# fx-erick/uncertainty-vit

Hardware: AMD Instinct MI355X
Metric: pretrain images/sec (ViT-B/16 224, bs=128/GPU) (higher is better)
Workload: dtype bf16

## Files before the change

### include/uvit.h

```cpp
#ifndef UVIT_H
#define UVIT_H
#include <stddef.h>
#include <stdint.h>

#ifdef __cplusplus
extern "C" {
#endif

#define UVIT_VERSION 100
#define UVIT_MAX_DEPTH 64

typedef struct uvit_engine uvit_engine;
typedef void* uvit_stream;

typedef struct uvit_config {
    int32_t img_size, patch_size, in_chans, embed_dim, depth, num_heads, mlp_hidden;
    int32_t use_shared_rel_pos_bias;
    int32_t use_abs_pos_emb;
    int32_t batch;
    float ln_eps;
    float attn_drop_rate;
    float drop_path_rate;
    int32_t bias_chunk;
    int32_t two_stream;
} uvit_config;

typedef struct uvit_layout_entry {
    char name[96];
    int64_t offset;
    int64_t numel;
    int32_t ndim;
    int32_t decay;
    int64_t shape[4];
} uvit_layout_entry;

typedef struct uvit_buffers {
    float* params;
    float* grads;
    float* adam_m;
    float* adam_v;
    float* ema;
    void* params_bf16;
    void* params_bf16_t;
    void* ema_bf16;
    const int32_t* rel_index;
    void* workspace;
    int64_t workspace_bytes;
} uvit_buffers;

typedef struct uvit_step_params {
    int32_t target_layers[UVIT_MAX_DEPTH];
    int32_t n_target_layers;
    int32_t target_layer_norm_last;
    int32_t post_target_layer_norm;
    int32_t l2_loss;
    float l1_beta;
    float loss_scale;
    float clip_grad;
    float lr, weight_decay, beta1, beta2, eps;
    int32_t opt_step;
    float ema_decay;
    int32_t do_ema;
    float grad_scale;
    uint32_t seed;
    uint32_t it;
    int32_t train_dropout;
    float lambda_pretraining;
    const float* sched_dev;
    int32_t sched_len, sched_index;
    int32_t layer_results_fc;
    float var_w0, var_margin0;
    int32_t target_batch_norm, target_instance_norm, post_target_instance_norm;
    int32_t n_rows_hint;
} uvit_step_params;

int uvit_version(void);
const char* uvit_source_hash(void);

int uvit_layout_count(const uvit_config* cfg);
int uvit_layout_get(const uvit_config* cfg, int index, uvit_layout_entry* out);
int64_t uvit_arena_numel(const uvit_config* cfg, int64_t* n_decay_out);
int64_t uvit_workspace_bytes(const uvit_config* cfg);

uvit_engine* uvit_engine_create(const uvit_config* cfg, const uvit_buffers* bufs, uvit_stream stream, int* err_out);
void uvit_engine_destroy(uvit_engine* e);

int uvit_engine_sync_shadows(uvit_engine* e, int which, uvit_stream stream);

int uvit_engine_forward_features(uvit_engine* e, int which, const float* images, const int64_t* mask, int batch,
                                 int train_dropout, uint32_t seed, uint32_t it, uvit_stream stream);
int uvit_engine_head(uvit_engine* e, int which, int all_tokens, float* out, int32_t* count_dev, uvit_stream stream);

void* uvit_engine_ws_ptr(uvit_engine* e, const char* name, int layer);
int uvit_engine_compact_rows(uvit_engine* e);

int uvit_step_begin(uvit_engine* e, const float* images, const int64_t* mask, const uvit_step_params* hp,
                    uvit_stream stream);
int uvit_step_backward_layer(uvit_engine* e, int layer, const uvit_step_params* hp, uvit_stream stream);
int uvit_step_wait_layer_grads(uvit_engine* e, int layer, uvit_stream stream);
int uvit_step_backward_embed(uvit_engine* e, uvit_stream stream);
int uvit_step_update(uvit_engine* e, const uvit_step_params* hp, uvit_stream stream);
int uvit_train_step(uvit_engine* e, const float* images, const int64_t* mask, const uvit_step_params* hp,
                    uvit_stream stream);
typedef struct uvit_tuning { int32_t nt_variant, tn_variant, tn_split_target, wgrad_group_chunks, nt_group, nt_persist; } uvit_tuning;
void uvit_tuning_default(uvit_tuning* out);
int uvit_engine_set_tuning(uvit_engine* e, const uvit_tuning* t);
int uvit_engine_set_streams(uvit_engine* e, int dual);
int uvit_engine_set_drop_path_rows(uvit_engine* e, int on);
int uvit_drop_path_kept_counts(int depth, float drop_path_rate, int draws_per_block, int batch, uint32_t seed, uint32_t it, int32_t* out);
int uvit_engine_profile(uvit_engine* e, int enable, int max_launches);
int uvit_engine_profile_read(uvit_engine* e, double* total_ms, int* launches, double* flops_per_launch);
int uvit_engine_profile_read_kind(uvit_engine* e, int kind, double* total_ms, int* launches, double* flops_per_launch,
                                  double* bytes_per_launch);
int uvit_engine_read_stats_async(uvit_engine* e, float* host_out2, uvit_stream stream);
int uvit_engine_read_stats(uvit_engine* e, float* host_out2, uvit_stream stream);

typedef struct uvit_gemm_epilogue {
    void* out; void* out2; const float* bias; const float* bias2; const float* gamma; const float* resid;
    const float* rowscale; const void* aux; const int64_t* mask; const float* mask_token;
    int32_t ldo, tokens, patches;
    int32_t row0;
} uvit_gemm_epilogue;
enum { UVIT_EPI_BF16 = 0, UVIT_EPI_QKV = 1, UVIT_EPI_GELU = 2, UVIT_EPI_RESID = 3, UVIT_EPI_F32 = 4,
       UVIT_EPI_PATCH = 5, UVIT_EPI_DGELU = 6, UVIT_EPI_QKV_ELU = 7,
       UVIT_EPI_GELU_DG = 8,
       UVIT_EPI_MULAUX = 9 };

int uvit_op_gemm_nt(int mode, const void* A_bf16, const void* W_bf16, int M, int N, int K, int lda, int ldw,
                    const uvit_gemm_epilogue* epi, uvit_stream stream);
int uvit_op_gemm_nt_tuned(int mode, const void* A_bf16, const void* W_bf16, int M, int N, int K, int lda, int ldw,
                          const uvit_gemm_epilogue* epi, const uvit_tuning* tune, int* tail_rows, uvit_stream stream);
int uvit_op_gemm_nt_sched(int mode, const void* A_bf16, const void* W_bf16, int M, int N, int K, int lda, int ldw,
                          const uvit_gemm_epilogue* epi, const uvit_tuning* tune, uint32_t* tile_counters, uvit_stream stream);
int uvit_op_gemm_tn(const void* Y_bf16, const void* X_bf16, int M, int N, int K, int ldy, int ldx, float* C, int ldc,
                    const uvit_tuning* tune, uvit_stream stream);
typedef struct uvit_wgrad_problem {
    const void* Y_bf16; const void* X_bf16; float* C; float* bias; float* bias2;
    int32_t bias_end, bias2_begin, M, N, K, ldy, ldx, ldc;
} uvit_wgrad_problem;
int uvit_op_wgrad_group(const uvit_wgrad_problem* problems, int count, const uvit_tuning* tune, uvit_stream stream);
int uvit_op_attn_fwd(const void* qkv, const float* biasP, void* out, float* lse, int B, int H, int N, int NP,
                     float scale, float p_drop, uint32_t seed, uint32_t layer, uvit_stream stream);
int64_t uvit_op_attn_bwd_ws_bytes(int B, int H, int N);
int uvit_op_attn_bwd(const void* qkv, const void* o_fwd, const void* d_o, const float* biasP, const float* lse,
                           float* delta, void* dqkv, float* dbias_slab, int accumulate_slab, void* ds_workspace, int B, int H,
                           int N, int NP, float scale, float p_drop, uint32_t seed, uint32_t layer, uvit_stream stream);
int uvit_op_attn_fwd_hd(const void* qkv, const float* biasP, void* out, float* lse, int B, int H, int N, int NP, int head_dim,
                        float scale, float p_drop, uint32_t seed, uint32_t layer, uvit_stream stream);
int uvit_op_attn_bwd_hd(const void* qkv, const void* o_fwd, const void* d_o, const float* biasP, const float* lse,
                        float* delta, void* dqkv, float* dbias_slab, int accumulate_slab, void* ds_workspace, int B, int H,
                        int N, int NP, int head_dim, float scale, float p_drop, uint32_t seed, uint32_t layer, uvit_stream stream);
int uvit_op_attn2_fwd(const void* qkv_m, const void* qkv_c, const float* biasP, void* out_m, void* out_c, float* lse, int B, int H,
                      int N, int NP, float scale, float p_drop, uint32_t seed, uint32_t layer, uvit_stream stream);
int64_t uvit_op_attn2_bwd_ws_bytes(int B, int H, int N);
int uvit_op_attn2_bwd(const void* qkv_m, const void* qkv_c, const void* o_m, const void* o_c, const void* d_m, const void* d_c,
                      const float* biasP, const float* lse, float* delta, void* dqkv_m, void* dqkv_c, float* dbias_slab,
                      int accumulate_slab, void* ds_workspace, int B, int H, int N, int NP, float scale, float p_drop, uint32_t seed,
                      uint32_t layer, uvit_stream stream);
int uvit_op_relpos_gather(const float* table, const int32_t* index, float* biasP, int H, int N, int NP, uvit_stream stream);
int uvit_op_relpos_scatter(const float* slab, int nslab, const int32_t* index, float* dtable, int H, int N, int NP,
                           uvit_stream stream);
int uvit_op_ln_fwd(const float* x, const float* w, const float* b, void* y_bf16, float* mean, float* rstd, int M, int C,
                   float eps, uvit_stream stream);
int uvit_op_ln_bwd(const void* dy_bf16, const float* x, const float* mean, const float* rstd, const float* w,
                   const float* dres, float* dx, float* dw, float* db, int M, int C, uvit_stream stream);
int uvit_op_ema(float* ema, const float* params, void* ema_bf16, int64_t n, float decay, uvit_stream stream);
int uvit_op_sumsq(const float* g, int64_t n, double* out, uvit_stream stream);
int uvit_op_adamw(float* p, const float* g, float* m, float* v, void* p_bf16, int64_t n, int64_t n_decay, float lr,
                  float wd, float b1, float b2, float eps, int step, const double* sumsq, float max_norm,
                  float grad_scale, float* gnorm_out, uvit_stream stream);
int uvit_op_smooth_l1(const float* out, const float* target, const int32_t* count_dev, float beta, int l2,
                      float loss_scale, float* loss, void* dout_bf16, int Mmax, int C, uvit_stream stream);
int uvit_op_wasserstein_loss(const float* out_m, const float* out_c, const float* tgt_m, const float* tgt_c,
                             const int32_t* count_dev, float lam, float loss_scale, float* scratch, float* loss,
                             void* dout_m_bf16, void* dout_c_bf16, int Mmax, int C, uvit_stream stream);
int uvit_op_target_accum(const float* x, const int32_t* rowidx, const int32_t* count, float* acc, int first, int Mmax,
                         int C, float eps, uvit_stream stream);
int uvit_op_variance_loss(const float* out, const int32_t* count_dev, float w, float margin, float loss_scale, float* scratch,
                          float* loss, float* std_loss0_out, void* dout_bf16, int Mmax, int C, uvit_stream stream);
int uvit_op_target_finalize(float* acc, const int32_t* count, int n_layers, int post_ln, int Mmax, int C, float eps,
                            uvit_stream stream);
int uvit_op_mask_compact(const int64_t* mask, int32_t* rowidx, int32_t* count, int B, int P, uvit_stream stream);
int uvit_op_synth_batch(float* images, int64_t* mask, int B, int chans, int img_size, int patches, int n_mask, uint32_t seed,
                        uint32_t it, uvit_stream stream);
int uvit_op_im2col(const float* img, void* cols_bf16, int B, int Cin, int img_size, int patch, uvit_stream stream);
int uvit_op_droppath(float* scales, const float* rates_dev, int depth, int B, uint32_t seed, uint32_t step,
                     uvit_stream stream);
int uvit_op_cast_bf16(const float* src, void* dst_bf16, int64_t n, uvit_stream stream);

#define UVIT_AUG_LANCZOS 1
#define UVIT_AUG_BILINEAR 2
#define UVIT_AUG_BICUBIC 3
#define UVIT_AUG_HAMMING 5
#define UVIT_AUG_BRIGHTNESS 0
#define UVIT_AUG_CONTRAST 1
#define UVIT_AUG_SATURATION 2
typedef struct uvit_augment_desc {
    int64_t offset;
    int32_t h, w;
    int32_t flip;
    int32_t crop_x, crop_y, crop_w, crop_h;
    int32_t resize_w, resize_h;
    int32_t win_x, win_y;
    int32_t filter;
    int32_t n_jitter;
    int32_t jitter_op[3];
    float jitter_factor[3];
    int32_t reserved;
} uvit_augment_desc;
int64_t uvit_op_augment_ws_bytes(const uvit_augment_desc* desc, int B, int S);
int uvit_op_augment_batch(const uint8_t* pixels, int64_t pixel_bytes, const uvit_augment_desc* desc, int B, int S, const float* mean,
                          const float* std, float* out, void* workspace, int64_t ws_bytes, uvit_stream stream);

#ifdef __cplusplus
}
#endif
#endif
```

### uncertainty-vit_amd/csrc/elementwise.hip

```cpp
#include "common.h"
#include "uvit_internal.h"
#include "rowwise.h"

__global__ void im2col_kernel(const float* __restrict__ img, bf16* __restrict__ cols, int B, int Cin, int S, int p) {
    const int g = S / p, P = g * g, K = Cin * p * p, kc_per_row = K / 8;
    const size_t total = (size_t)B * P * kc_per_row;
    for (size_t idx = blockIdx.x * (size_t)blockDim.x + threadIdx.x; idx < total; idx += (size_t)gridDim.x * blockDim.x) {
        const int kc = idx % kc_per_row;
        const size_t row = idx / kc_per_row;
        const int b = row / P, pp = row % P, py = pp / g, px = pp % g;
        const int k = kc * 8, c = k / (p * p), i = (k % (p * p)) / p, j = k % p;
        const float* src = img + (((size_t)b * Cin + c) * S + py * p + i) * S + px * p + j;
        const float4 a = *(const float4*)src, d = *(const float4*)(src + 4);
        bf16x8 o = {f2bf(a.x), f2bf(a.y), f2bf(a.z), f2bf(a.w), f2bf(d.x), f2bf(d.y), f2bf(d.z), f2bf(d.w)};
        *(bf16x8*)(cols + row * K + k) = o;
    }
}

__global__ __launch_bounds__(1024)
void mask_compact_kernel(const int64_t* __restrict__ mask, int* __restrict__ rowidx, int* __restrict__ count, int B, int P) {
    __shared__ int s_w[16];
    const int n = B * P, tid = threadIdx.x, lane = tid & 63, wave = tid >> 6;
    int base = 0;
    for (int sc = 0; sc < n; sc += 32 * 1024) {
        unsigned bits = 0;
#pragma unroll
        for (int k = 0; k < 32; ++k) {
            const int i = sc + k * 1024 + tid;
            if (i < n && mask[i] != 0) bits |= 1u << k;
        }
        for (int k = 0; k < 32 && sc + k * 1024 < n; ++k) {
            const bool keep = (bits >> k) & 1u;
            const unsigned long long bal = __ballot(keep);
            if (lane == 0) s_w[wave] = __popcll(bal);
            __syncthreads();
            int before = base, tot = 0;
#pragma unroll
            for (int q = 0; q < 16; ++q) { const int v = s_w[q]; tot += v; if (q < wave) before += v; }
            if (keep) {
                const int i = sc + k * 1024 + tid, b = i / P;
                rowidx[before + __popcll(bal & ((1ull << lane) - 1ull))] = b * (P + 1) + 1 + (i - b * P);
            }
            base += tot;
            __syncthreads();
        }
    }
    if (tid == 0) *count = base;
    for (int i = base + tid; i < n; i += 1024) rowidx[i] = 0;
}

__global__ void set_cls_kernel(float* __restrict__ x, const float* __restrict__ cls, int B, int N, int C) {
    const int i = blockIdx.x * blockDim.x + threadIdx.x;
    if (i < B * C) { const int b = i / C, c = i - b * C; x[(size_t)b * N * C + c] = cls[c]; }
}

__global__ void relpos_gather_kernel(const float* __restrict__ table, const int* __restrict__ index,
                                     float* __restrict__ biasP, int H, int N, int NP) {
    const size_t total = (size_t)H * NP * NP;
    for (size_t i = blockIdx.x * (size_t)blockDim.x + threadIdx.x; i < total; i += (size_t)gridDim.x * blockDim.x) {
        const int k = i % NP, q = (i / NP) % NP, h = i / ((size_t)NP * NP);
        float v = 0.f;
        if (k >= N) v = -1e30f;
        else if (q < N && table) v = table[(size_t)index[q * N + k] * H + h] * 1.4426950408889634f;
        biasP[i] = v;
    }
}

__global__ void relpos_scatter_kernel(const float* __restrict__ slab, int nslab, const int* __restrict__ index,
                                      float* __restrict__ dtable, int H, int N, int NP, int ntable) {
    extern __shared__ float tsum[];
    const int h = blockIdx.x;
    for (int i = threadIdx.x; i < ntable; i += blockDim.x) tsum[i] = 0.f;
    __syncthreads();
    const int total = N * N;
    for (int i = blockIdx.y * blockDim.x + threadIdx.x; i < total; i += gridDim.y * blockDim.x) {
        const int k = i / N, q = i - k * N;
        float s = 0.f;
        for (int sl = 0; sl < nslab; ++sl) s += slab[(((size_t)sl * H + h) * NP + k) * NP + q];
        atomicAdd(&tsum[index[q * N + k]], s);
    }
    __syncthreads();
    for (int i = threadIdx.x; i < ntable; i += blockDim.x)
        if (tsum[i] != 0.f) atomicAdd(dtable + (size_t)i * H + h, tsum[i]);
}

#define CP_ROWS 32

template <int NV, int WAVES = 4>
__device__ __forceinline__ void block_col_atomic(float4 (&acc)[NV], float* out, int nv, float (*red)[64 * 4]) {
    const int lane = threadIdx.x & 63, wave = threadIdx.x >> 6;
#pragma unroll
    for (int k = 0; k < NV; ++k) {
        if (64 * k < nv) {
            __syncthreads();
            ((float4*)red[wave])[lane] = acc[k];
            __syncthreads();
            if (wave == 0) {
                float4 s = ((float4*)red[0])[lane];
#pragma unroll
                for (int q = 1; q < WAVES; ++q) { const float4 a = ((float4*)red[q])[lane]; s.x += a.x; s.y += a.y; s.z += a.z; s.w += a.w; }
                const int i = lane + 64 * k;
                if (i < nv) { atomicAdd(out + 4 * i, s.x); atomicAdd(out + 4 * i + 1, s.y); atomicAdd(out + 4 * i + 2, s.z); atomicAdd(out + 4 * i + 3, s.w); }
            }
        }
    }
}

template <int NV>
__global__ __launch_bounds__(256)
void ls_bwd_kernel(const float* __restrict__ dx, const bf16* __restrict__ y, const float* __restrict__ gamma,
                   const float* __restrict__ rowscale, bf16* __restrict__ dy, float* __restrict__ dgamma,
                   float* __restrict__ dbias, int M, int C, int tokens, int nrep, size_t rep_stride,
                   const int* __restrict__ rowidx, const int* __restrict__ count) {
    __shared__ float red[4][64 * 4];
    dgamma += (size_t)(blockIdx.x % nrep) * rep_stride; dbias += (size_t)(blockIdx.x % nrep) * rep_stride;
    const int lane = threadIdx.x & 63, wave = threadIdx.x >> 6, nv = C >> 2;
    float4 ag[NV], ab[NV];
#pragma unroll
    for (int k = 0; k < NV; ++k) { ag[k] = make_float4(0.f, 0.f, 0.f, 0.f); ab[k] = ag[k]; }
    const int row_end = min((int)(blockIdx.x + 1) * CP_ROWS, M);
    const int n_valid = rowidx ? min(*count, M) : M;
    for (int row = blockIdx.x * CP_ROWS + wave; row < row_end; row += 4) {
        if (row >= n_valid) { store_zero_row<NV>(dy + (size_t)row * C, nv, lane); continue; }
        const int xr = rowidx ? rowidx[row] : row;
        const float dp = rowscale ? rowscale[xr / tokens] : 1.0f;
#pragma unroll
        for (int k = 0; k < NV; ++k) {
            const int i = lane + 64 * k;
            if (i < nv) {
                const float4 d = ((const float4*)(dx + (size_t)xr * C))[i];
                const float4 g = ((const float4*)gamma)[i];
                const bf16x4 yy = ((const bf16x4*)(y + (size_t)xr * C))[i];
                ls_apply(d, dp, yy, g, (bf16x4*)(dy + (size_t)row * C) + i, ag[k], ab[k]);
            }
        }
    }
    block_col_atomic(ag, dgamma, nv, red);
    block_col_atomic(ab, dbias, nv, red);
}

#define CS_ROWS 256
__global__ __launch_bounds__(256)
void colsum_kernel(const bf16* __restrict__ y, int ld, int col0, int ncols, int M, float* __restrict__ out, int nrep, size_t rep_stride) {
    __shared__ float red[4][64 * 8];
    out += (size_t)(blockIdx.y % nrep) * rep_stride;
    const int lane = threadIdx.x & 63, wave = threadIdx.x >> 6;
    const int c = blockIdx.x * 512 + lane * 8;
    float acc[8];
#pragma unroll
    for (int j = 0; j < 8; ++j) acc[j] = 0.f;
    const int row_end = min((int)(blockIdx.y + 1) * CS_ROWS, M);
    if (c < ncols) {
        const bf16* base = y + col0 + c;
        int row = blockIdx.y * CS_ROWS + wave;
        for (; row + 12 < row_end; row += 16) {
            const bf16x8 v0 = *(const bf16x8*)(base + (size_t)row * ld), v1 = *(const bf16x8*)(base + (size_t)(row + 4) * ld);
            const bf16x8 v2 = *(const bf16x8*)(base + (size_t)(row + 8) * ld), v3 = *(const bf16x8*)(base + (size_t)(row + 12) * ld);
#pragma unroll
            for (int j = 0; j < 8; ++j) acc[j] += (bf2f(v0[j]) + bf2f(v1[j])) + (bf2f(v2[j]) + bf2f(v3[j]));
        }
        for (; row < row_end; row += 4) {
            const bf16x8 v = *(const bf16x8*)(base + (size_t)row * ld);
#pragma unroll
            for (int j = 0; j < 8; ++j) acc[j] += bf2f(v[j]);
        }
    }
#pragma unroll
    for (int j = 0; j < 8; ++j) red[wave][lane * 8 + j] = acc[j];
    __syncthreads();
    for (int i = threadIdx.x; i < 512; i += 256) {
        const int cc = blockIdx.x * 512 + i;
        if (cc < ncols) atomicAdd(out + cc, red[0][i] + red[1][i] + red[2][i] + red[3][i]);
    }
}

__global__ __launch_bounds__(256)
void smooth_l1_kernel(const float* __restrict__ out, const float* __restrict__ target, const int* __restrict__ count,
                      float beta, int l2, float loss_scale, float* __restrict__ loss, bf16* __restrict__ dout,
                      int Mmax, int C) {
    __shared__ float red[4];
    const int n_valid = min(*count, Mmax);
    const size_t nv = (size_t)Mmax * C / 4, valid = (size_t)n_valid * C / 4;
    const float inv = loss_scale / ((float)n_valid * (float)C);
    float part = 0.f;
    for (size_t i = blockIdx.x * (size_t)blockDim.x + threadIdx.x; i < nv; i += (size_t)gridDim.x * blockDim.x) {
        bf16x4 g = bf16x4_zero();
        if (i < valid) {
            const float4 o = ((const float4*)out)[i], t = ((const float4*)target)[i];
            const float d[4] = {o.x - t.x, o.y - t.y, o.z - t.z, o.w - t.w};
#pragma unroll
            for (int j = 0; j < 4; ++j) {
                const float a = fabsf(d[j]);
                float l, gr;
                if (l2) { l = d[j] * d[j]; gr = 2.0f * d[j]; }
                else if (a < beta) { l = 0.5f * d[j] * d[j] / beta; gr = d[j] / beta; }
                else { l = a - 0.5f * beta; gr = d[j] > 0.f ? 1.0f : (d[j] < 0.f ? -1.0f : 0.f); }
                part += l;
                g[j] = f2bf(gr * inv);
            }
        }
        ((bf16x4*)dout)[i] = g;
    }
    part = wave_sum(part);
    if ((threadIdx.x & 63) == 0) red[threadIdx.x >> 6] = part;
    __syncthreads();
    if (threadIdx.x == 0) atomicAdd(loss, (red[0] + red[1] + red[2] + red[3]) * inv);
}

template <int NV, int TKB_WAVES>
__global__ __launch_bounds__(TKB_WAVES * 64)
void token_bwd_kernel(const float* __restrict__ dx, const int64_t* __restrict__ mask, bf16* __restrict__ dpatch,
                      float* __restrict__ dcls, float* __restrict__ dmask, int B, int P, int C, int rows_per_block) {
    __shared__ float red[TKB_WAVES][64 * 4];
    const int lane = threadIdx.x & 63, wave = threadIdx.x >> 6, nv = C >> 2, N = P + 1;
    float4 ac[NV], am[NV];
#pragma unroll
    for (int k = 0; k < NV; ++k) { ac[k] = make_float4(0.f, 0.f, 0.f, 0.f); am[k] = ac[k]; }
    const int M = B * N;
    const int row_end = min((int)(blockIdx.x + 1) * rows_per_block, M);
    for (int row = blockIdx.x * rows_per_block + wave; row < row_end; row += TKB_WAVES) {
        const int b = row / N, t = row - b * N;
        const bool is_cls = t == 0;
        const bool masked = !is_cls && mask[b * P + t - 1] != 0;
#pragma unroll
        for (int k = 0; k < NV; ++k) {
            const int i = lane + 64 * k;
            if (i < nv) {
                const float4 d = ((const float4*)(dx + (size_t)row * C))[i];
                if (is_cls) { ac[k].x += d.x; ac[k].y += d.y; ac[k].z += d.z; ac[k].w += d.w; }
                else {
                    if (masked) { am[k].x += d.x; am[k].y += d.y; am[k].z += d.z; am[k].w += d.w; }
                    const float m = masked ? 0.f : 1.f;
                    bf16x4 o = {f2bf(d.x * m), f2bf(d.y * m), f2bf(d.z * m), f2bf(d.w * m)};
                    ((bf16x4*)(dpatch + ((size_t)b * P + t - 1) * C))[i] = o;
                }
            }
        }
    }
    const int row0 = blockIdx.x * rows_per_block;
    if ((row0 + N - 1) / N * N < row_end) block_col_atomic<NV, TKB_WAVES>(ac, dcls, nv, red);
    block_col_atomic<NV, TKB_WAVES>(am, dmask, nv, red);
}

__global__ __launch_bounds__(256)
void transpose_batch_kernel(const TransposeDesc* __restrict__ descs, int ndesc) {
    __shared__ bf16 tile[64][66];
    int lo = 0, hi = ndesc - 1;
    const int t = blockIdx.x;
    while (lo < hi) { const int mid = (lo + hi + 1) >> 1; if (descs[mid].tile0 <= t) lo = mid; else hi = mid - 1; }
    const TransposeDesc d = descs[lo];
    const int local = t - d.tile0, tc = (d.cols + 63) / 64;
    const int tr0 = (local / tc) * 64, tc0 = (local % tc) * 64;
    if (tr0 >= d.rows) return;
    const bf16* src = (const bf16*)d.src; bf16* dst = (bf16*)d.dst;
    if (tr0 + 64 <= d.rows && tc0 + 64 <= d.cols && !(d.rows & 7) && !(d.cols & 7)) {
#pragma unroll
        for (int k = 0; k < 2; ++k) {
            const int idx = threadIdx.x + 256 * k, r = idx >> 3, c8 = (idx & 7) * 8;
            const bf16x8 v = *(const bf16x8*)(src + (size_t)(tr0 + r) * d.cols + tc0 + c8);
#pragma unroll
            for (int j = 0; j < 8; ++j) tile[r][c8 + j] = v[j];
        }
        __syncthreads();
#pragma unroll
        for (int k = 0; k < 2; ++k) {
            const int idx = threadIdx.x + 256 * k, oc = idx >> 3, r8 = (idx & 7) * 8;
            bf16x8 o;
#pragma unroll
            for (int j = 0; j < 8; ++j) o[j] = tile[r8 + j][oc];
            *(bf16x8*)(dst + (size_t)(tc0 + oc) * d.rows + tr0 + r8) = o;
        }
        return;
    }
    for (int i = threadIdx.x; i < 64 * 64; i += 256) {
        const int r = i >> 6, c = i & 63;
        tile[r][c] = (tr0 + r < d.rows && tc0 + c < d.cols) ? src[(size_t)(tr0 + r) * d.cols + tc0 + c] : f2bf(0.f);
    }
    __syncthreads();
    for (int i = threadIdx.x; i < 64 * 64; i += 256) {
        const int c = i >> 6, r = i & 63;
        if (tr0 + r < d.rows && tc0 + c < d.cols) dst[(size_t)(tc0 + c) * d.rows + tr0 + r] = tile[r][c];
    }
}

__global__ void droppath_kernel(float* __restrict__ scales, const float* __restrict__ rates, int depth, int nbr, int B,
                                uint32_t seed, uint32_t step) {
    const int i = blockIdx.x * blockDim.x + threadIdx.x;
    if (i >= depth * nbr * B) return;
    const int b = i % B, lb = i / B, layer = lb / nbr, br = lb - layer * nbr;
    const float r = rates[layer];
    float v = 1.0f;
    if (r > 0.f) {
        const uint32_t key = uvit_hash32(seed ^ ((step * (uint32_t)nbr * depth + (uint32_t)nbr * layer + br + 1u) * 0x9E3779B9u));
        v = uvit_hash32((uint32_t)b ^ key) >= uvit_drop_threshold(r) ? 1.0f / (1.0f - r) : 0.f;
    }
    scales[i] = v;
}

#define DP_MAX_LISTS 128
struct DpHostCounts { int k[DP_MAX_LISTS]; };
#define DPL_CHUNKS 8
__global__ __launch_bounds__(256)
void droppath_lists_kernel(const float* __restrict__ scales, int* __restrict__ pos, int* __restrict__ bmap, int* __restrict__ rows,
                           int* __restrict__ cnt, int B, int tokens, int rows_stride, DpHostCounts host) {
    extern __shared__ int s_m[];
    const int lb = blockIdx.x;
    const float* sc = scales + (size_t)lb * B;
    int* p = pos + (size_t)lb * B; int* m = bmap + (size_t)lb * B; int* r = rows + (size_t)lb * rows_stride;
    const bool pub = blockIdx.y == 0;
    __shared__ int s_w[4];
    const int lane = threadIdx.x & 63, wave = threadIdx.x >> 6;
    int base = 0;
    for (int b0 = 0; b0 < B; b0 += 256) {
        const int b = b0 + threadIdx.x;
        const bool keep = b < B && sc[b] != 0.f;
        const unsigned long long bal = __ballot(keep);
        if (lane == 0) s_w[wave] = __popcll(bal);
        __syncthreads();
        int before = base;
        for (int q = 0; q < wave; ++q) before += s_w[q];
        const int slot = before + __popcll(bal & ((1ull << lane) - 1ull));
        if (pub && b < B) p[b] = keep ? slot : -1;
        if (keep) { s_m[slot] = b; if (pub) m[slot] = b; }
        base += s_w[0] + s_w[1] + s_w[2] + s_w[3];
        __syncthreads();
    }
    if (pub) {
        for (int b = base + threadIdx.x; b < B; b += 256) m[b] = 0;
        if (threadIdx.x == 0) {
            cnt[lb] = base * tokens;
            cnt[gridDim.x + lb] = base != host.k[lb];
        }
    }
    const int n = base * tokens, npad = (n + 63) & ~63;
    const int per = (npad + DPL_CHUNKS - 1) / DPL_CHUNKS, lo = blockIdx.y * per, hi = min(lo + per, npad);
    for (int i = lo + threadIdx.x; i < hi; i += blockDim.x) {
        const int slot = i / tokens;
        r[i] = i < n ? s_m[slot] * tokens + (i - slot * tokens) : -1;
    }
}

static inline int grid_for(size_t n, int block, int cap = 256 * 8) {
    size_t g = (n + block - 1) / block;
    return (int)(g < 1 ? 1 : (g > (size_t)cap ? cap : g));
}

int uvit_im2col_launch(const float* img, void* cols, int B, int Cin, int S, int p, hipStream_t s) {
    if (B <= 0 || p % 8 || S % p || S % 4) return UVIT_ERR_SHAPE;
    const size_t total = (size_t)B * (S / p) * (S / p) * (Cin * p * p / 8);
    hipLaunchKernelGGL(im2col_kernel, dim3(grid_for(total, 256, 256 * 16)), dim3(256), 0, s, img, (bf16*)cols, B, Cin, S, p);
    return uvit_check_launch();
}
int uvit_mask_compact_launch(const int64_t* mask, int* rowidx, int* count, int B, int P, hipStream_t s) {
    hipLaunchKernelGGL(mask_compact_kernel, dim3(1), dim3(1024), 0, s, mask, rowidx, count, B, P);
    return uvit_check_launch();
}
int uvit_set_cls_launch(float* x, const float* cls, const float* pos, int B, int N, int C, hipStream_t s) {
    if (pos) return UVIT_ERR_ARG;
    hipLaunchKernelGGL(set_cls_kernel, dim3((B * C + 255) / 256), dim3(256), 0, s, x, cls, B, N, C);
    return uvit_check_launch();
}
int uvit_relpos_gather_launch(const float* table, const int* index, float* biasP, int H, int N, int NP, hipStream_t s) {
    hipLaunchKernelGGL(relpos_gather_kernel, dim3(grid_for((size_t)H * NP * NP, 256)), dim3(256), 0, s, table, index, biasP, H, N, NP);
    return uvit_check_launch();
}
int uvit_relpos_scatter_launch(const float* slab, int nslab, const int* index, float* dtable, int H, int N, int NP,
                               hipStream_t s) {
    const int g = (int)(sqrtf((float)(N - 1)) + 0.5f);
    const int ntable = (2 * g - 1) * (2 * g - 1) + 3;
    hipLaunchKernelGGL(relpos_scatter_kernel, dim3(H, 24), dim3(256), ntable * sizeof(float), s, slab, nslab, index, dtable, H, N, NP, ntable);
    return uvit_check_launch();
}
int uvit_ls_bwd_launch(const float* dx, const LsNext& ls, int M, int C, int nrep, size_t rep_stride, hipStream_t s,
                       const int* rowidx, const int* count) {
    if (C % 4 || C > ROW_MAXV * 256 || (rowidx && !count)) return UVIT_ERR_SHAPE;
    dispatch_nv(C, [&](auto nv) {
        hipLaunchKernelGGL(ls_bwd_kernel<decltype(nv)::value>, dim3((M + CP_ROWS - 1) / CP_ROWS), dim3(256), 0, s, dx, ls.y, ls.gamma, ls.rowscale,
                           ls.dy, ls.dgamma, ls.dbias, M, C, ls.tokens, nrep > 0 ? nrep : 1, rep_stride, rowidx, count);
    });
    return uvit_check_launch();
}
__global__ void rows_guard_kernel(const int* __restrict__ count, int limit, float* __restrict__ loss) {
    if (*count > limit) loss[0] = __builtin_nanf("");
}
int uvit_rows_guard_launch(const int* count, int limit, float* loss, hipStream_t s) {
    hipLaunchKernelGGL(rows_guard_kernel, dim3(1), dim3(1), 0, s, count, limit, loss);
    return uvit_check_launch();
}
int uvit_colsum_launch(const void* y, int ld, int col0, int ncols, int M, float* out, int nrep, size_t rep_stride, hipStream_t s) {
    if (ncols % 8 || col0 % 8 || ld % 8) return UVIT_ERR_SHAPE;
    hipLaunchKernelGGL(colsum_kernel, dim3((ncols + 511) / 512, (M + CS_ROWS - 1) / CS_ROWS), dim3(256), 0, s, (const bf16*)y, ld, col0, ncols, M, out, nrep > 0 ? nrep : 1, rep_stride);
    return uvit_check_launch();
}
int uvit_smooth_l1_launch(const float* out, const float* target, const int* count, float beta, int l2, float loss_scale,
                          float* loss, void* dout, int Mmax, int C, hipStream_t s) {
    if (C % 4) return UVIT_ERR_SHAPE;
    hipLaunchKernelGGL(smooth_l1_kernel, dim3(grid_for((size_t)Mmax * C / 4, 256, 512)), dim3(256), 0, s, out, target, count, beta, l2,
                       loss_scale, loss, (bf16*)dout, Mmax, C);
    return uvit_check_launch();
}
int uvit_token_bwd_launch(const float* dx, const int64_t* mask, void* dpatch, float* dcls, float* dmask_token, int B,
                          int P, int C, hipStream_t s) {
    if (C % 4 || C > ROW_MAXV * 256) return UVIT_ERR_SHAPE;
    const int M = B * (P + 1);
    int rpb = (M + 127) / 128;
    rpb = ((rpb + 15) / 16) * 16;
    if (rpb < 32) rpb = 32;
    dispatch_nv(C, [&](auto nv) {
        hipLaunchKernelGGL((token_bwd_kernel<decltype(nv)::value, 16>), dim3((M + rpb - 1) / rpb), dim3(16 * 64), 0, s, dx, mask, (bf16*)dpatch,
                           dcls, dmask_token, B, P, C, rpb);
    });
    return uvit_check_launch();
}
int uvit_transpose_batch_launch(const void* descs_dev, int ndesc, int total_tiles, hipStream_t s) {
    if (ndesc <= 0 || total_tiles <= 0) return UVIT_OK;
    hipLaunchKernelGGL(transpose_batch_kernel, dim3(total_tiles), dim3(256), 0, s, (const TransposeDesc*)descs_dev, ndesc);
    return uvit_check_launch();
}
int uvit_droppath_launch(float* scales, const float* rates_dev, int depth, int nbr, int B, uint32_t seed, uint32_t step, hipStream_t s) {
    hipLaunchKernelGGL(droppath_kernel, dim3((depth * nbr * B + 255) / 256), dim3(256), 0, s, scales, rates_dev, depth, nbr, B, seed, step);
    return uvit_check_launch();
}

__global__ void droppath_lists_guard_kernel(const int* __restrict__ flags, int n, float* __restrict__ loss) {
    int bad = 0;
    for (int i = 0; i < n; ++i) bad |= flags[i];
    if (bad) loss[0] = __builtin_nanf("");
}
int uvit_droppath_lists_guard_launch(const int* cnt, int nlists, float* loss, hipStream_t s) {
    hipLaunchKernelGGL(droppath_lists_guard_kernel, dim3(1), dim3(1), 0, s, cnt + nlists, nlists, loss);
    return uvit_check_launch();
}
int uvit_droppath_lists_launch(const float* scales, int* pos, int* bmap, int* rows, int* cnt, int nlists, int B, int tokens,
                               int rows_stride, const int* host_counts, hipStream_t s) {
    if (nlists < 1 || nlists > DP_MAX_LISTS || rows_stride < ((B * tokens + 63) & ~63)) return UVIT_ERR_ARG;
    DpHostCounts h;
    for (int i = 0; i < DP_MAX_LISTS; ++i) h.k[i] = i < nlists ? host_counts[i] : 0;
    hipLaunchKernelGGL(droppath_lists_kernel, dim3(nlists, DPL_CHUNKS), dim3(256), (size_t)B * sizeof(int), s, scales, pos, bmap, rows, cnt, B, tokens, rows_stride, h);
    return uvit_check_launch();
}

__global__ void poison_kernel(const float* __restrict__ loss, float* __restrict__ dst, int* __restrict__ sticky) {
    if ((__float_as_uint(*loss) & 0x7F800000u) == 0x7F800000u) { *dst = __int_as_float(0x7FC00000); if (sticky) *sticky = 1; }
}
int uvit_poison_if_nonfinite_launch(const float* loss, float* dst, int* sticky, hipStream_t s) {
    hipLaunchKernelGGL(poison_kernel, dim3(1), dim3(1), 0, s, loss, dst, sticky);
    return uvit_check_launch();
}

__device__ __forceinline__ float sig_(float x) { return 1.0f / (1.0f + __expf(-x)); }

__global__ __launch_bounds__(256)
void wl_pos_kernel(const float* __restrict__ om, const float* __restrict__ oc, const float* __restrict__ tm,
                   const float* __restrict__ tc, const int* __restrict__ count, float* __restrict__ scratch, int Mmax, int C) {
    const int lane = threadIdx.x & 63, row = blockIdx.x * 4 + (threadIdx.x >> 6);
    if (row >= min(*count, Mmax)) return;
    float acc = 0.f;
    for (int i = lane; i < C; i += 64) {
        const size_t o = (size_t)row * C + i;
        const float d = sig_(om[o]) - sig_(tm[o]);
        const float e = sqrtf(fmaxf(sig_(oc[o]), 1e-24f)) - sqrtf(fmaxf(sig_(tc[o]), 1e-24f));
        acc += d * d + e * e;
    }
    acc = wave_sum(acc);
    if (lane == 0) { scratch[16 + row] = acc; atomicMax((int*)scratch, __float_as_int(acc)); }
}

__global__ __launch_bounds__(256)
void wl_sum_kernel(const int* __restrict__ count, float* __restrict__ scratch, int Mmax) {
    const int n = min(*count, Mmax);
    const float m = scratch[0];
    float s1 = 0.f, s2 = 0.f;
    for (int r = blockIdx.x * blockDim.x + threadIdx.x; r < n; r += gridDim.x * blockDim.x) {
        const float pos = scratch[16 + r], u = pos / m;
        s1 += log1pf(__expf(u));
        s2 += sig_(u) * u;
        if (pos == m) atomicMin((int*)scratch + 3, r);
    }
    s1 = wave_sum(s1); s2 = wave_sum(s2);
    if ((threadIdx.x & 63) == 0) { atomicAdd(scratch + 1, s1); atomicAdd(scratch + 2, s2); }
}

__global__ __launch_bounds__(256)
void wl_grad_kernel(const float* __restrict__ om, const float* __restrict__ oc, const float* __restrict__ tm,
                    const float* __restrict__ tc, const int* __restrict__ count, const float* __restrict__ scratch,
                    float lam, float* __restrict__ loss, bf16* __restrict__ dout_m, bf16* __restrict__ dout_c, int Mmax, int C) {
    const int lane = threadIdx.x & 63, row = blockIdx.x * 4 + (threadIdx.x >> 6);
    const int n = min(*count, Mmax);
    const float F = 1.3132616875182228f;
    if (blockIdx.x == 0 && threadIdx.x == 0) atomicAdd(loss, lam * scratch[1] / F);
    if (row >= Mmax) return;
    if (row >= n) {
        for (int i = lane; i < C; i += 64) dout_c[(size_t)row * C + i] = f2bf(0.f);
        return;
    }
    const float m = scratch[0], u = scratch[16 + row] / m;
    float coef = sig_(u);
    if (row == ((const int*)scratch)[3]) coef -= scratch[2];
    coef *= lam / (F * m);
    for (int i = lane; i < C; i += 64) {
        const size_t o = (size_t)row * C + i;
        const float a = sig_(om[o]), c1 = sig_(oc[o]), c2 = sig_(tc[o]);
        const float gm = coef * 2.0f * (a - sig_(tm[o])) * a * (1.0f - a);
        const float s1 = sqrtf(fmaxf(c1, 1e-24f)), s2 = sqrtf(fmaxf(c2, 1e-24f));
        const float gc = coef * (s1 - s2) / s1 * c1 * (1.0f - c1);
        dout_m[o] = f2bf(bf2f(dout_m[o]) + gm);
        dout_c[o] = f2bf(gc);
    }
}

int uvit_wasserstein_loss_launch(const float* out_m, const float* out_c, const float* tgt_m, const float* tgt_c, const int* count,
                                 float lam, float loss_scale, float* scratch, float* loss, void* dout_m, void* dout_c,
                                 int Mmax, int C, hipStream_t s) {
    if (hipMemsetAsync(scratch, 0, 16 * sizeof(float), s) != hipSuccess) return UVIT_ERR_LAUNCH;
    const int big = 0x7FFFFFFF;
    (void)big;
    hipLaunchKernelGGL(wl_pos_kernel, dim3((Mmax + 3) / 4), dim3(256), 0, s, out_m, out_c, tgt_m, tgt_c, count, scratch, Mmax, C);
    if (hipMemsetD32Async((hipDeviceptr_t)((int*)scratch + 3), 0x7FFFFFFF, 1, s) != hipSuccess) return UVIT_ERR_LAUNCH;
    hipLaunchKernelGGL(wl_sum_kernel, dim3(64), dim3(256), 0, s, count, scratch, Mmax);
    hipLaunchKernelGGL(wl_grad_kernel, dim3((Mmax + 3) / 4), dim3(256), 0, s, out_m, out_c, tgt_m, tgt_c, count, scratch,
                       lam * loss_scale, loss, (bf16*)dout_m, (bf16*)dout_c, Mmax, C);
    return uvit_check_launch();
}

__global__ __launch_bounds__(256)
void synth_images_kernel(float* __restrict__ img, size_t n2, uint32_t key) {
    for (size_t i = blockIdx.x * (size_t)blockDim.x + threadIdx.x; i < n2; i += (size_t)gridDim.x * blockDim.x) {
        const uint32_t a = uvit_hash32((uint32_t)(2 * i) ^ key), b = uvit_hash32((uint32_t)(2 * i + 1) ^ key ^ (uint32_t)(i >> 31));
        const float u1 = ((float)(a >> 8) + 0.5f) * (1.0f / 16777216.0f);
        const float u2 = ((float)(b >> 8) + 0.5f) * (1.0f / 16777216.0f);
        const float r = sqrtf(-2.0f * __logf(u1));
        float sn, cs;
        __sincosf(6.283185307179586f * u2, &sn, &cs);
        ((float2*)img)[i] = make_float2(r * cs, r * sn);
    }
}

__global__ __launch_bounds__(256)
void synth_mask_kernel(int64_t* __restrict__ mask, int P, int n_mask, uint32_t key) {
    extern __shared__ uint32_t keys[];
    const int b = blockIdx.x;
    for (int i = threadIdx.x; i < P; i += blockDim.x) keys[i] = uvit_hash32((uint32_t)(b * P + i) ^ key);
    __syncthreads();
    for (int i = threadIdx.x; i < P; i += blockDim.x) {
        const uint32_t k = keys[i];
        int rank = 0;
        for (int j = 0; j < P; ++j) rank += (keys[j] < k) || (keys[j] == k && j < i);
        mask[(size_t)b * P + i] = rank < n_mask ? 1 : 0;
    }
}

int uvit_synth_batch_launch(float* images, int64_t* mask, int B, int chans, int img_size, int patches, int n_mask, uint32_t seed,
                            uint32_t it, hipStream_t s) {
    if (B < 1 || chans < 1 || img_size < 1 || patches < 1 || n_mask < 0 || n_mask > patches) return UVIT_ERR_SHAPE;
    const size_t n = (size_t)B * chans * img_size * img_size;
    if (n % 2) return UVIT_ERR_SHAPE;
    const uint32_t key = uvit_hash32(seed ^ (it * 0x9E3779B9u + 0x51ED270Bu));
    if (images) {
        size_t g = (n / 2 + 255) / 256;
        hipLaunchKernelGGL(synth_images_kernel, dim3((unsigned)(g > 4096 ? 4096 : g)), dim3(256), 0, s, images, n / 2, key);
    }
    if (mask) hipLaunchKernelGGL(synth_mask_kernel, dim3(B), dim3(256), patches * sizeof(uint32_t), s, mask, patches, n_mask, key ^ 0xA5A5A5A5u);
    return uvit_check_launch();
}

#define VL_ROWS 64
template <int PASS>
__global__ __launch_bounds__(256)
void varloss_colstat_kernel(const float* __restrict__ out, const int* __restrict__ count, float* __restrict__ scratch, int Mmax, int C) {
    const int n = min(*count, Mmax);
    const int c = blockIdx.x * 256 + threadIdx.x;
    if (c >= C) return;
    const int r0 = blockIdx.y * VL_ROWS, r1 = min(r0 + VL_ROWS, n);
    const float mean = PASS == 1 ? scratch[c] / (float)max(n, 1) : 0.f;
    float acc = 0.f;
    for (int r = r0; r < r1; ++r) {
        const float v = out[(size_t)r * C + c];
        acc += PASS == 0 ? v : (v - mean) * (v - mean);
    }
    if (r0 < r1) atomicAdd(scratch + PASS * C + c, acc);
}

__global__ __launch_bounds__(256)
void varloss_sum_kernel(const int* __restrict__ count, float* __restrict__ scratch, float w, float margin, float* __restrict__ loss,
                        float* __restrict__ std_out, int Mmax, int C) {
    __shared__ float red[4];
    const int n = min(*count, Mmax);
    float acc = 0.f;
    for (int c = threadIdx.x; c < C; c += 256) {
        const float z0 = sqrtf(scratch[C + c] / (float)max(n - 1, 1) + 1e-6f);
        acc += fmaxf(margin - z0, 0.f);
    }
    acc = wave_sum(acc);
    if ((threadIdx.x & 63) == 0) red[threadIdx.x >> 6] = acc;
    __syncthreads();
    if (threadIdx.x == 0) {
        const float s = (red[0] + red[1] + red[2] + red[3]) / (float)C;
        scratch[2 * C] = s;
        if (std_out) *std_out = s;
        atomicAdd(loss, w * s);
    }
}

__global__ __launch_bounds__(256)
void varloss_grad_kernel(const float* __restrict__ out, const int* __restrict__ count, const float* __restrict__ scratch, float w,
                         float margin, bf16* __restrict__ dout, int Mmax, int C) {
    const int n = min(*count, Mmax);
    const int c = blockIdx.x * 256 + threadIdx.x;
    if (c >= C || n < 2) return;
    const float mean = scratch[c] / (float)n;
    const float z0 = sqrtf(scratch[C + c] / (float)(n - 1) + 1e-6f);
    if (!(z0 < margin)) return;
    const float k = -w / ((float)C * (float)(n - 1) * z0);
    const int r0 = blockIdx.y * VL_ROWS, r1 = min(r0 + VL_ROWS, n);
    for (int r = r0; r < r1; ++r) {
        const size_t o = (size_t)r * C + c;
        dout[o] = f2bf(bf2f(dout[o]) + k * (out[o] - mean));
    }
}

int uvit_variance_loss_launch(const float* out, const int* count, float w, float margin, float loss_scale, float* scratch, float* loss,
                              float* std_loss0_out, void* dout, int Mmax, int C, hipStream_t s) {
    if (Mmax < 1 || C < 1) return UVIT_ERR_SHAPE;
    if (hipMemsetAsync(scratch, 0, (2 * (size_t)C + 16) * sizeof(float), s) != hipSuccess) return UVIT_ERR_LAUNCH;
    const dim3 grid((C + 255) / 256, (Mmax + VL_ROWS - 1) / VL_ROWS);
    hipLaunchKernelGGL(varloss_colstat_kernel<0>, grid, dim3(256), 0, s, out, count, scratch, Mmax, C);
    hipLaunchKernelGGL(varloss_colstat_kernel<1>, grid, dim3(256), 0, s, out, count, scratch, Mmax, C);
    hipLaunchKernelGGL(varloss_sum_kernel, dim3(1), dim3(256), 0, s, count, scratch, w * loss_scale, margin, loss, std_loss0_out, Mmax, C);
    hipLaunchKernelGGL(varloss_grad_kernel, grid, dim3(256), 0, s, out, count, scratch, w * loss_scale, margin, (bf16*)dout, Mmax, C);
    return uvit_check_launch();
}

__global__ __launch_bounds__(256)
void add_pos_kernel(float* __restrict__ x, const float* __restrict__ pos, size_t n4, size_t per_sample4) {
    for (size_t i = blockIdx.x * (size_t)blockDim.x + threadIdx.x; i < n4; i += (size_t)gridDim.x * blockDim.x) {
        float4 a = ((float4*)x)[i];
        const float4 p = ((const float4*)pos)[i % per_sample4];
        a.x += p.x; a.y += p.y; a.z += p.z; a.w += p.w;
        ((float4*)x)[i] = a;
    }
}
__global__ __launch_bounds__(256)
void pos_bwd_kernel(const float* __restrict__ dx, float* __restrict__ dpos, int B, size_t per_sample4) {
    const size_t i = blockIdx.x * (size_t)blockDim.x + threadIdx.x;
    if (i >= per_sample4) return;
    float4 acc = make_float4(0.f, 0.f, 0.f, 0.f);
    for (int b = 0; b < B; ++b) {
        const float4 d = ((const float4*)dx)[(size_t)b * per_sample4 + i];
        acc.x += d.x; acc.y += d.y; acc.z += d.z; acc.w += d.w;
    }
    ((float4*)dpos)[i] = acc;
}
int uvit_add_pos_launch(float* x, const float* pos, int B, int N, int C, hipStream_t s) {
    if (C % 4) return UVIT_ERR_SHAPE;
    const size_t per = (size_t)N * C / 4, n4 = per * B;
    hipLaunchKernelGGL(add_pos_kernel, dim3(grid_for(n4, 256)), dim3(256), 0, s, x, pos, n4, per);
    return uvit_check_launch();
}
int uvit_pos_bwd_launch(const float* dx, float* dpos, int B, int N, int C, hipStream_t s) {
    if (C % 4) return UVIT_ERR_SHAPE;
    const size_t per = (size_t)N * C / 4;
    hipLaunchKernelGGL(pos_bwd_kernel, dim3((unsigned)((per + 255) / 256)), dim3(256), 0, s, dx, dpos, B, per);
    return uvit_check_launch();
}
```

### uncertainty-vit_amd/csrc/engine.hip

```cpp
#include <hip/hip_runtime.h>
#include <math.h>
#include <stdio.h>
#include <stdlib.h>
#include <string.h>

#include <string>
#include <vector>

#include "../../include/uvit.h"
#include "common.h"
#include "uvit_internal.h"

#define CHECK(x) do { int _rc = (x); if (_rc) return _rc; } while (0)
#define NREP 32
#define RP(off) (e->grep + ((off) - e->lo.n_decay))
#define HIPCHECK(x) do { if ((x) != hipSuccess) return UVIT_ERR_LAUNCH; } while (0)
#define GEMM_NT(...) uvit_gemm_nt_launch(__VA_ARGS__, &e->tune)
#define GEMM_TN(...) uvit_gemm_tn_launch(__VA_ARGS__, &e->tune)
#define GEMM_TN_GROUP(...) uvit_gemm_tn_group_launch(__VA_ARGS__, &e->tune)

struct LayerOff { size_t n1w, n1b, qkvw, qb, vb, projw, projb, g1, n2w, n2b, fc1w, fc1b, fc2w, fc2b, g2;
                  size_t cqkvw, cqb, cvb, cprojw, cprojb; };
struct Layout {
    size_t cls, mask_tok, pew, peb, relt, normw, normb, lmw, lmb, pos;
    size_t ccls, cmask_tok, cpew, cpeb, clmw, clmb;
    LayerOff L[UVIT_MAX_DEPTH];
    size_t n_total, n_decay, n_live;
    std::vector<uvit_layout_entry> entries;
};

static size_t align64(size_t x) { return (x + 63) & ~(size_t)63; }

static int cfg_ok(const uvit_config* c) {
    if (!c) return UVIT_ERR_ARG;
    if (c->depth < 1 || c->depth > UVIT_MAX_DEPTH || c->num_heads < 1) return UVIT_ERR_SHAPE;
    if (c->embed_dim != c->num_heads * 64 && (c->two_stream || c->embed_dim != c->num_heads * 80)) return UVIT_ERR_SHAPE;
    if (c->embed_dim % 64 || c->mlp_hidden % 64 || c->patch_size % 8 || c->img_size % c->patch_size) return UVIT_ERR_SHAPE;
    if ((c->in_chans * c->patch_size * c->patch_size) % 64) return UVIT_ERR_SHAPE;
    const int g = c->img_size / c->patch_size;
    if (g * g + 1 > 208 || c->batch < 1) return UVIT_ERR_SHAPE;
    if (c->use_abs_pos_emb && c->two_stream) return UVIT_ERR_SHAPE;
    return UVIT_OK;
}

static void build_layout(const uvit_config* c, Layout& lo) {
    const int64_t C = c->embed_dim, Hd = c->mlp_hidden, g = c->img_size / c->patch_size;
    const int64_t Kpe = (int64_t)c->in_chans * c->patch_size * c->patch_size;
    size_t off = 0;
    auto add = [&](const std::string& name, std::vector<int64_t> shape, int decay) -> size_t {
        uvit_layout_entry e;
        memset(&e, 0, sizeof(e));
        snprintf(e.name, sizeof(e.name), "%s", name.c_str());
        e.offset = (int64_t)off; e.ndim = (int)shape.size(); e.decay = decay; e.numel = 1;
        for (size_t i = 0; i < shape.size(); ++i) { e.shape[i] = shape[i]; e.numel *= shape[i]; }
        lo.entries.push_back(e);
        const size_t at = off;
        off = align64(off + (size_t)e.numel);
        return at;
    };
    auto blk = [](int i, const char* s) { return "blocks." + std::to_string(i) + "." + s; };
    const bool two = c->two_stream != 0;
    lo.mask_tok = add("mask_token", {1, 1, C}, 1);
    if (two) lo.cmask_tok = add("cov_mask_token", {1, 1, C}, 1);
    if (two) lo.ccls = add("cov_cls_token", {1, 1, C}, 1);
    if (c->use_shared_rel_pos_bias) lo.relt = add("rel_pos_bias.relative_position_bias_table", {(2 * g - 1) * (2 * g - 1) + 3, c->num_heads}, 1);
    else lo.relt = (size_t)-1;
    lo.pew = add("patch_embed.proj.weight", {C, c->in_chans, c->patch_size, c->patch_size}, 1);
    if (two) lo.cpew = add("cov_patch_embed.proj.weight", {C, c->in_chans, c->patch_size, c->patch_size}, 1);
    (void)Kpe;
    for (int i = 0; i < c->depth; ++i) {
        lo.L[i].qkvw = add(blk(i, "attn.qkv.weight"), {3 * C, C}, 1);
        lo.L[i].projw = add(blk(i, "attn.proj.weight"), {C, C}, 1);
        if (two) lo.L[i].cprojw = add(blk(i, "attn.cov_proj.weight"), {C, C}, 1);
        lo.L[i].fc1w = add(blk(i, "mlp.fc1.weight"), {Hd, C}, 1);
        lo.L[i].fc2w = add(blk(i, "mlp.fc2.weight"), {C, Hd}, 1);
    }
    lo.lmw = add("lm_head.weight", {C, C}, 1);
    if (two) lo.clmw = add("cov_lm_head.weight", {C, C}, 1);
    lo.n_decay = off;
    lo.cls = add("cls_token", {1, 1, C}, 0);
    lo.pos = c->use_abs_pos_emb ? add("pos_embed", {1, g * g + 1, C}, 0) : (size_t)-1;
    lo.peb = add("patch_embed.proj.bias", {C}, 0);
    if (two) lo.cpeb = add("cov_patch_embed.proj.bias", {C}, 0);
    for (int i = 0; i < c->depth; ++i) {
        lo.L[i].g1 = add(blk(i, "gamma_1"), {C}, 0);
        lo.L[i].g2 = add(blk(i, "gamma_2"), {C}, 0);
        lo.L[i].n1w = add(blk(i, "norm1.weight"), {C}, 0);
        lo.L[i].n1b = add(blk(i, "norm1.bias"), {C}, 0);
        lo.L[i].qb = add(blk(i, "attn.q_bias"), {C}, 0);
        lo.L[i].vb = add(blk(i, "attn.v_bias"), {C}, 0);
        if (two) { lo.L[i].cqb = add(blk(i, "attn.cov_q_bias"), {C}, 0); lo.L[i].cvb = add(blk(i, "attn.cov_v_bias"), {C}, 0); }
        lo.L[i].projb = add(blk(i, "attn.proj.bias"), {C}, 0);
        if (two) lo.L[i].cprojb = add(blk(i, "attn.cov_proj.bias"), {C}, 0);
        lo.L[i].n2w = add(blk(i, "norm2.weight"), {C}, 0);
        lo.L[i].n2b = add(blk(i, "norm2.bias"), {C}, 0);
        lo.L[i].fc1b = add(blk(i, "mlp.fc1.bias"), {Hd}, 0);
        lo.L[i].fc2b = add(blk(i, "mlp.fc2.bias"), {C}, 0);
    }
    lo.normw = add("norm.weight", {C}, 0);
    lo.normb = add("norm.bias", {C}, 0);
    lo.lmb = add("lm_head.bias", {C}, 0);
    if (two) lo.clmb = add("cov_lm_head.bias", {C}, 0);
    lo.n_live = off;
    if (two)
        for (int i = 0; i < c->depth; ++i) lo.L[i].cqkvw = add(blk(i, "attn.cov_qkv.weight"), {3 * C, C}, 2);
    lo.n_total = off;
}

struct LayerActs {
    bf16 *ln1, *qkv, *attn, *projout, *ln2, *h, *a, *mlpout;
    float *mean1, *rstd1, *mean2, *rstd2, *lse;
};

struct uvit_engine {
    uvit_config cfg;
    uvit_buffers buf;
    Layout lo;
    int B, P, N, NP, C, Hd, H, Kpe, M, Mpad, BP, BPpad, chunk, nchunk;
    int head_dim;
    float attn_scale;
    int S;
    GemmTune tune;
    int cur_B;
    bf16* cols;
    float* X[UVIT_MAX_DEPTH + 1];
    float* XM[UVIT_MAX_DEPTH];
    LayerActs acts[UVIT_MAX_DEPTH];
    LayerActs tacts;
    float *tX[2], *tXM;
    int *rowidx, *count;
    bf16 *normed[2], *dout[2], *dnormed[2], *dpatch[2];
    float *meanF[2], *rstdF[2], *outputs[2], *targets[2];
    float *biasP_s, *biasP_t, *slabs, *delta;
    void* ds_ws[2] = {nullptr, nullptr};
    float *dXa, *dXb;
    bf16 *dY1[2], *dY2[2], *dH[2], *dLN, *dAttn, *dqkv[2];
    float *dp_scales, *dp_rates;
    int *dpl_pos = nullptr, *dpl_bmap = nullptr, *dpl_rows = nullptr, *dpl_cnt = nullptr;
    size_t dpl_stride = 0;
    int dpl_K[128] = {};
    bool dpl_enable = true;
    bool dpl_on = false;
    std::vector<float> dp_rates_host;
    float *loss, *gnorm; double* sumsq;
    float* wl_scratch;
    float *dense_v, *dense_acc; int *idrows, *idcount;
    float* var_scratch;
    int* poisoned;
    TransposeDesc* tdesc; int n_tdesc, n_ttiles;
    int64_t* mask_copy;
    unsigned* tile_cnt = nullptr;
    float* grep;
    size_t n_nd;
    bool slab_started;
    bool last_dropout; uint32_t last_seed, last_it;
    int bwd_next = -1;
    int compact_R = 0;
    bool dual = true;
    hipStream_t aux = nullptr, aux_eq = nullptr, aux_lo = nullptr;
    hipEvent_t ev_fork = nullptr, ev_teacher = nullptr, ev_x = nullptr;
    hipEvent_t ev_wdone[UVIT_MAX_DEPTH] = {};
    hipEvent_t ev_ds = nullptr;
    bool prof_on = false;
    std::vector<hipEvent_t> prof_ev;
    std::vector<int> prof_kind;
    std::vector<int> prof_rows;
    size_t prof_used = 0;
    size_t rows_all() const { return (size_t)(S - 1) * Mpad + M; }
    size_t rows_alloc() const { return (size_t)S * Mpad; }
};

struct Bump {
    char* base; size_t off, cap;
    template <typename T> T* take(size_t n) {
        off = (off + 255) & ~(size_t)255;
        T* p = base ? (T*)(base + off) : nullptr;
        off += n * sizeof(T);
        return p;
    }
};

static size_t roundup(size_t x, size_t m) { return (x + m - 1) / m * m; }
static std::vector<float> dp_rates_linspace(int depth, float rate);

static void plan_workspace(uvit_engine* e, Bump& b) {
    const uvit_config& c = e->cfg;
    const size_t Mp = e->rows_alloc(), C = e->C, Hd = e->Hd, BPp = e->BPpad;
    auto acts = [&](LayerActs& a) {
        a.ln1 = b.take<bf16>(Mp * C); a.qkv = b.take<bf16>(Mp * 3 * C); a.attn = b.take<bf16>(Mp * C);
        a.projout = b.take<bf16>(Mp * C); a.ln2 = b.take<bf16>(Mp * C); a.h = b.take<bf16>(Mp * Hd);
        a.a = b.take<bf16>(Mp * Hd); a.mlpout = b.take<bf16>(Mp * C);
        a.mean1 = b.take<float>(Mp); a.rstd1 = b.take<float>(Mp); a.mean2 = b.take<float>(Mp); a.rstd2 = b.take<float>(Mp);
        a.lse = b.take<float>((size_t)e->B * e->H * e->N);
    };
    e->cols = b.take<bf16>(BPp * e->Kpe);
    for (int i = 0; i <= c.depth; ++i) e->X[i] = b.take<float>(Mp * C);
    for (int i = 0; i < c.depth; ++i) { e->XM[i] = b.take<float>(Mp * C); acts(e->acts[i]); }
    acts(e->tacts);
    e->tX[0] = b.take<float>(Mp * C); e->tX[1] = b.take<float>(Mp * C); e->tXM = b.take<float>(Mp * C);
    e->rowidx = b.take<int>(e->BP + 64); e->count = b.take<int>(64);
    for (int st = 0; st < e->S; ++st) {
        e->normed[st] = b.take<bf16>(BPp * C); e->dout[st] = b.take<bf16>(BPp * C); e->dnormed[st] = b.take<bf16>(BPp * C);
        e->dpatch[st] = b.take<bf16>(BPp * C);
        e->meanF[st] = b.take<float>(BPp); e->rstdF[st] = b.take<float>(BPp);
        e->outputs[st] = b.take<float>(BPp * C); e->targets[st] = b.take<float>(BPp * C);
    }
    const size_t bias_n = (size_t)e->H * e->NP * e->NP;
    e->biasP_s = b.take<float>(bias_n); e->biasP_t = b.take<float>(bias_n);
    e->slabs = b.take<float>(bias_n);
    e->delta = b.take<float>((size_t)e->B * e->H * e->N);
    if (e->cfg.use_shared_rel_pos_bias)
        for (int k = 0; k < 2; ++k)
            e->ds_ws[k] = b.take<char>(e->S == 1 ? uvit_attn_bwd_fused_ws_bytes(e->B, e->H, e->N) : uvit_attn2_bwd_ws_bytes(e->B, e->H, e->N));
    e->dXa = b.take<float>(Mp * C); e->dXb = b.take<float>(Mp * C);
    for (int k = 0; k < 2; ++k) {
        e->dY1[k] = b.take<bf16>(Mp * C); e->dY2[k] = b.take<bf16>(Mp * C); e->dH[k] = b.take<bf16>(Mp * Hd);
        e->dqkv[k] = b.take<bf16>(Mp * 3 * C);
    }
    e->dLN = b.take<bf16>(Mp * C); e->dAttn = b.take<bf16>(Mp * C);
    e->dp_scales = b.take<float>((size_t)c.depth * 2 * e->S * e->B); e->dp_rates = b.take<float>(c.depth);
    if ((size_t)c.depth * 2 * e->S <= 128) {
        const size_t nl = (size_t)c.depth * 2 * e->S;
        e->dpl_stride = roundup((size_t)e->B * e->N, 64);
        e->dpl_pos = b.take<int>(nl * e->B); e->dpl_bmap = b.take<int>(nl * e->B);
        e->dpl_rows = b.take<int>(nl * e->dpl_stride); e->dpl_cnt = b.take<int>(2 * nl + 64);
    }
    e->loss = b.take<float>(64); e->gnorm = e->loss + 1; e->sumsq = (double*)(e->loss + 2);
    e->wl_scratch = b.take<float>(16 + BPp);
    e->poisoned = b.take<int>(64);
    e->var_scratch = b.take<float>(2 * C + 16);
    e->dense_v = b.take<float>(BPp * C); e->dense_acc = b.take<float>(BPp * C);
    e->idrows = b.take<int>(e->BP + 64); e->idcount = b.take<int>(64);
    e->tdesc = b.take<TransposeDesc>(7 * c.depth + 4);
    e->mask_copy = b.take<int64_t>(e->BP + 64);
    e->grep = b.take<float>((size_t)NREP * e->n_nd);
    e->tile_cnt = b.take<unsigned>(64);
}

static void fill_dims(uvit_engine* e) {
    const uvit_config& c = e->cfg;
    const int g = c.img_size / c.patch_size;
    e->B = c.batch; e->P = g * g; e->N = e->P + 1; e->NP = 208; e->C = c.embed_dim; e->Hd = c.mlp_hidden;
    e->H = c.num_heads; e->Kpe = c.in_chans * c.patch_size * c.patch_size;
    e->head_dim = c.embed_dim / c.num_heads;
    e->attn_scale = e->head_dim == 64 ? 0.125f : (float)(1.0 / std::sqrt((double)e->head_dim));
    e->S = c.two_stream ? 2 : 1;
    e->M = e->B * e->N; e->Mpad = (int)roundup(e->M, 128); e->BP = e->B * e->P; e->BPpad = (int)roundup(e->BP, 128);
    if (c.bias_chunk > 0) {
        e->chunk = c.bias_chunk;
    } else {
        int ncu = 256, dev = 0; hipDeviceProp_t prop;
        if (hipGetDevice(&dev) == hipSuccess && hipGetDeviceProperties(&prop, dev) == hipSuccess && prop.multiProcessorCount > 0)
            ncu = prop.multiProcessorCount;
        const int nhalf = (e->N + 15) / 16 > 7 ? 2 : 1;
        const int resident = 1;
        int max_chunks = (resident * ncu) / (e->H * nhalf);
        if (max_chunks < 1) max_chunks = 1;
        e->chunk = (e->B + max_chunks - 1) / max_chunks;
        if (e->chunk < 1) e->chunk = 1;
    }
    e->nchunk = (e->B + e->chunk - 1) / e->chunk;
    e->cur_B = e->B;
    Layout tmp_lo; build_layout(&e->cfg, tmp_lo);
    e->n_nd = tmp_lo.n_live - tmp_lo.n_decay;
}


extern "C" void uvit_engine_destroy(uvit_engine* e);
extern "C" int uvit_version(void) { return UVIT_VERSION; }
#ifndef UVIT_SRC_HASH
#define UVIT_SRC_HASH "unknown"
#endif
extern "C" const char* uvit_source_hash(void) { return UVIT_SRC_HASH; }

extern "C" int uvit_layout_count(const uvit_config* cfg) {
    if (cfg_ok(cfg)) return UVIT_ERR_SHAPE;
    Layout lo; build_layout(cfg, lo);
    return (int)lo.entries.size();
}
extern "C" int uvit_layout_get(const uvit_config* cfg, int index, uvit_layout_entry* out) {
    if (cfg_ok(cfg) || !out) return UVIT_ERR_SHAPE;
    Layout lo; build_layout(cfg, lo);
    if (index < 0 || index >= (int)lo.entries.size()) return UVIT_ERR_ARG;
    *out = lo.entries[index];
    return UVIT_OK;
}
extern "C" int64_t uvit_arena_numel(const uvit_config* cfg, int64_t* n_decay_out) {
    if (cfg_ok(cfg)) return UVIT_ERR_SHAPE;
    Layout lo; build_layout(cfg, lo);
    if (n_decay_out) *n_decay_out = (int64_t)lo.n_decay;
    return (int64_t)lo.n_total;
}
extern "C" int64_t uvit_workspace_bytes(const uvit_config* cfg) {
    if (cfg_ok(cfg)) return UVIT_ERR_SHAPE;
    uvit_engine tmp;
    tmp.cfg = *cfg;
    fill_dims(&tmp);
    Bump b{nullptr, 0, 0};
    plan_workspace(&tmp, b);
    return (int64_t)roundup(b.off, 4096) + 4096;
}

extern "C" uvit_engine* uvit_engine_create(const uvit_config* cfg, const uvit_buffers* bufs, uvit_stream stream, int* err_out) {
    auto fail = [&](int rc) -> uvit_engine* { if (err_out) *err_out = rc; return nullptr; };
    if (cfg_ok(cfg) || !bufs) return fail(UVIT_ERR_SHAPE);
    if (!bufs->params || !bufs->grads || !bufs->adam_m || !bufs->adam_v || !bufs->ema || !bufs->params_bf16 ||
        !bufs->params_bf16_t || !bufs->ema_bf16 || !bufs->workspace) return fail(UVIT_ERR_ARG);
    if (cfg->use_shared_rel_pos_bias && !bufs->rel_index) return fail(UVIT_ERR_ARG);
    if (bufs->workspace_bytes < uvit_workspace_bytes(cfg)) return fail(UVIT_ERR_WORKSPACE);
    uvit_engine* e = new uvit_engine();
    e->cfg = *cfg; e->buf = *bufs;
    fill_dims(e);
    build_layout(cfg, e->lo);
    Bump b{(char*)bufs->workspace, 0, (size_t)bufs->workspace_bytes};
    plan_workspace(e, b);
    hipStream_t s = (hipStream_t)stream;
    if (hipMemsetAsync(bufs->workspace, 0, b.off, s) != hipSuccess) { delete e; return fail(UVIT_ERR_LAUNCH); }
    std::vector<float> rates = dp_rates_linspace(cfg->depth, cfg->drop_path_rate);
    e->dp_rates_host = rates;
    if (const char* v = getenv("UVIT_DP_ROWS")) e->dpl_enable = v[0] != '0';
    std::vector<TransposeDesc> td;
    int tiles = 0;
    const char* src = (const char*)bufs->params_bf16; char* dst = (char*)bufs->params_bf16_t;
    auto addT = [&](size_t off, int rows, int cols) {
        TransposeDesc d; d.src = src + off * 2; d.dst = dst + off * 2; d.rows = rows; d.cols = cols; d.tile0 = tiles; d.pad = 0;
        tiles += ((rows + 63) / 64) * ((cols + 63) / 64);
        td.push_back(d);
    };
    for (int i = 0; i < cfg->depth; ++i) {
        addT(e->lo.L[i].qkvw, 3 * e->C, e->C); addT(e->lo.L[i].projw, e->C, e->C);
        addT(e->lo.L[i].fc1w, e->Hd, e->C); addT(e->lo.L[i].fc2w, e->C, e->Hd);
        if (e->S == 2) addT(e->lo.L[i].cprojw, e->C, e->C);
    }
    addT(e->lo.lmw, e->C, e->C);
    if (e->S == 2) addT(e->lo.clmw, e->C, e->C);
    e->n_tdesc = (int)td.size(); e->n_ttiles = tiles;
    {
        std::vector<int> idr(e->BP);
        for (int i = 0; i < e->BP; ++i) idr[i] = i;
        const int cnt = e->BP;
        if (hipMemcpyAsync(e->idrows, idr.data(), idr.size() * sizeof(int), hipMemcpyHostToDevice, s) != hipSuccess ||
            hipMemcpyAsync(e->idcount, &cnt, sizeof(int), hipMemcpyHostToDevice, s) != hipSuccess ||
            hipStreamSynchronize(s) != hipSuccess) { delete e; return fail(UVIT_ERR_LAUNCH); }
    }
    if (hipMemcpyAsync(e->dp_rates, rates.data(), rates.size() * sizeof(float), hipMemcpyHostToDevice, s) != hipSuccess ||
        hipMemcpyAsync(e->tdesc, td.data(), td.size() * sizeof(TransposeDesc), hipMemcpyHostToDevice, s) != hipSuccess ||
        hipStreamSynchronize(s) != hipSuccess) { delete e; return fail(UVIT_ERR_LAUNCH); }
    e->slab_started = false; e->last_dropout = false; e->last_seed = 0; e->last_it = 0;
    {
        const char* env = getenv("UVIT_SINGLE_STREAM");
        e->dual = !(env && env[0] == '1');
        int lo = 0, hi = 0; (void)hipDeviceGetStreamPriorityRange(&lo, &hi);
        bool ok = hipStreamCreateWithFlags(&e->aux_eq, hipStreamNonBlocking) == hipSuccess &&
                  hipStreamCreateWithPriority(&e->aux_lo, hipStreamNonBlocking, lo) == hipSuccess;
        e->aux = e->aux_eq;
        auto mk = [&](hipEvent_t* ev) { ok = ok && hipEventCreateWithFlags(ev, hipEventDisableTiming) == hipSuccess; };
        mk(&e->ev_fork); mk(&e->ev_teacher); mk(&e->ev_ds); mk(&e->ev_x);
        for (int i = 0; i < cfg->depth; ++i) mk(&e->ev_wdone[i]);
        if (!ok) { uvit_engine_destroy(e); return fail(UVIT_ERR_LAUNCH); }
    }
    if (err_out) *err_out = UVIT_OK;
    return e;
}

extern "C" void uvit_engine_destroy(uvit_engine* e) {
    if (!e) return;
    for (hipEvent_t ev : e->prof_ev) (void)hipEventDestroy(ev);
    if (e->aux_eq) { (void)hipStreamSynchronize(e->aux_eq); (void)hipStreamDestroy(e->aux_eq); }
    if (e->aux_lo) { (void)hipStreamSynchronize(e->aux_lo); (void)hipStreamDestroy(e->aux_lo); }
    if (e->ev_fork) (void)hipEventDestroy(e->ev_fork);
    if (e->ev_teacher) (void)hipEventDestroy(e->ev_teacher);
    if (e->ev_ds) (void)hipEventDestroy(e->ev_ds);
    if (e->ev_x) (void)hipEventDestroy(e->ev_x);
    for (int i = 0; i < UVIT_MAX_DEPTH; ++i) if (e->ev_wdone[i]) (void)hipEventDestroy(e->ev_wdone[i]);
    delete e;
}

static int tune_from_abi(const uvit_tuning* t, GemmTune& g) {
    if (!t) { g = GemmTune(); return UVIT_OK; }
    if ((t->nt_variant != 0 && t->nt_variant != 1 && t->nt_variant != 3 && t->nt_variant != 5 && t->nt_variant != 6 && t->nt_variant != 7) ||
        (t->tn_variant != 0 && t->tn_variant != 1 && t->tn_variant != 3) || t->tn_split_target < 0 || t->wgrad_group_chunks < 0 || t->nt_group < 0 || t->nt_group > 64 || (t->nt_persist != 0 && t->nt_persist != 1))
        return UVIT_ERR_ARG;
    g.nt_variant = t->nt_variant; g.tn_variant = t->tn_variant;
    g.tn_target = t->tn_split_target > 0 ? t->tn_split_target : 512; g.group_chunks = t->wgrad_group_chunks; g.nt_group = t->nt_group; g.nt_persist = t->nt_persist;
    return UVIT_OK;
}

extern "C" void uvit_tuning_default(uvit_tuning* out) {
    if (!out) return;
    const GemmTune d;
    out->nt_variant = d.nt_variant; out->tn_variant = d.tn_variant; out->tn_split_target = d.tn_target; out->wgrad_group_chunks = d.group_chunks; out->nt_group = d.nt_group; out->nt_persist = d.nt_persist;
}

extern "C" int uvit_engine_set_tuning(uvit_engine* e, const uvit_tuning* t) {
    if (!e) return UVIT_ERR_ARG;
    return tune_from_abi(t, e->tune);
}

extern "C" int uvit_engine_set_streams(uvit_engine* e, int dual) {
    if (!e || dual < 0 || dual > 2) return UVIT_ERR_ARG;
    hipStream_t next = dual == 2 ? e->aux_lo : e->aux_eq;
    if (next != e->aux && e->aux) HIPCHECK(hipStreamSynchronize(e->aux));
    e->aux = next;
    e->dual = dual != 0;
    return UVIT_OK;
}

extern "C" int uvit_engine_set_drop_path_rows(uvit_engine* e, int on) {
    if (!e) return UVIT_ERR_ARG;
    e->dpl_enable = on != 0;
    return UVIT_OK;
}

extern "C" int uvit_engine_profile(uvit_engine* e, int enable, int max_launches) {
    if (!e) return UVIT_ERR_ARG;
    if (enable && e->prof_ev.empty()) {
        e->prof_ev.resize((size_t)(max_launches > 0 ? max_launches : 4096) * 2);
        e->prof_kind.assign(e->prof_ev.size() / 2, -1);
        e->prof_rows.assign(e->prof_ev.size() / 2, 0);
        for (auto& ev : e->prof_ev) if (hipEventCreate(&ev) != hipSuccess) return UVIT_ERR_LAUNCH;
    }
    e->prof_on = enable != 0;
    if (enable) e->prof_used = 0;
    return UVIT_OK;
}

enum { UVIT_PROF_FC1_T = 0, UVIT_PROF_FC1_S = 1, UVIT_PROF_PROJ = 2, UVIT_PROF_FC2 = 3, UVIT_PROF_KINDS = 4 };

extern "C" int uvit_engine_profile_read_kind(uvit_engine* e, int kind, double* total_ms, int* launches, double* flops_per_launch,
                                             double* bytes_per_launch) {
    if (!e || !total_ms || !launches || kind >= UVIT_PROF_KINDS) return UVIT_ERR_ARG;
    double t = 0.0, rows = 0.0; int n = 0;
    for (size_t i = 0; i + 1 < e->prof_used; i += 2) {
        const int k = e->prof_kind[i / 2];
        if (kind < 0 ? (k != UVIT_PROF_FC1_T && k != UVIT_PROF_FC1_S) : k != kind) continue;
        float ms = 0.f;
        if (hipEventElapsedTime(&ms, e->prof_ev[i], e->prof_ev[i + 1]) != hipSuccess) return UVIT_ERR_LAUNCH;
        t += ms; ++n; rows += e->prof_rows[i / 2];
    }
    *total_ms = t; *launches = n;
    const double M1 = n ? rows / n : (double)e->cur_B * e->N, Mall = M1, C = e->C, Hd = e->Hd;
    double fl = 0.0, by = 0.0;
    if (kind < 0 || kind == UVIT_PROF_FC1_T || kind == UVIT_PROF_FC1_S) {
        fl = 2.0 * Mall * Hd * C;
        by = 2.0 * (Mall * C + Hd * C + Mall * Hd * (kind == UVIT_PROF_FC1_T ? 1.0 : kind == UVIT_PROF_FC1_S ? 2.0 : 1.5));
    } else if (kind == UVIT_PROF_PROJ) {
        fl = 2.0 * M1 * C * C;
        by = 2.0 * (M1 * C + C * C) + 8.0 * M1 * C;
    } else {
        fl = 2.0 * M1 * C * Hd;
        by = 2.0 * (M1 * Hd + C * Hd) + 8.0 * M1 * C;
    }
    if (flops_per_launch) *flops_per_launch = fl;
    if (bytes_per_launch) *bytes_per_launch = by;
    return UVIT_OK;
}
extern "C" int uvit_engine_profile_read(uvit_engine* e, double* total_ms, int* launches, double* flops_per_launch) {
    return uvit_engine_profile_read_kind(e, -1, total_ms, launches, flops_per_launch, nullptr);
}

extern "C" int uvit_engine_sync_shadows(uvit_engine* e, int which, uvit_stream stream) {
    if (!e) return UVIT_ERR_ARG;
    hipStream_t s = (hipStream_t)stream;
    if (which & 1) {
        CHECK(uvit_cast_bf16_launch(e->buf.params, e->buf.params_bf16, e->lo.n_total, s));
        CHECK(uvit_transpose_batch_launch(e->tdesc, e->n_tdesc, e->n_ttiles, s));
    }
    if (which & 2) CHECK(uvit_cast_bf16_launch(e->buf.ema, e->buf.ema_bf16, e->lo.n_total, s));
    return UVIT_OK;
}

struct Weights { const float* f; const bf16* b; };

static size_t off_projw(const LayerOff& o, int st) { return st ? o.cprojw : o.projw; }
static size_t off_projb(const LayerOff& o, int st) { return st ? o.cprojb : o.projb; }
static size_t off_qb(const LayerOff& o, int st) { return st ? o.cqb : o.qb; }
static size_t off_vb(const LayerOff& o, int st) { return st ? o.cvb : o.vb; }

static const float* dp_ptr(uvit_engine* e, bool on, int l, int st, int branch, int Bc) {
    if (!on) return nullptr;
    const int nbr = 2 * e->S, k = e->S == 2 ? 2 * st + branch : branch;
    return e->dp_scales + (size_t)(nbr * l + k) * Bc;
}

struct DpList { const int *pos, *bmap, *rows, *cnt; int K; };
static void dp_list_get(const uvit_engine* e, int l, int st, int branch, DpList& d) {
    const int lb = 2 * e->S * l + (e->S == 2 ? 2 * st + branch : branch);
    d.pos = e->dpl_pos + (size_t)lb * e->B; d.bmap = e->dpl_bmap + (size_t)lb * e->B;
    d.rows = e->dpl_rows + (size_t)lb * e->dpl_stride; d.cnt = e->dpl_cnt + lb; d.K = e->dpl_K[lb];
}
static void dp_kept_counts(const float* rates, int depth, int nbr, int B, uint32_t seed, uint32_t it, int* out) {
    for (int l = 0; l < depth; ++l)
        for (int br = 0; br < nbr; ++br) {
            const float r = rates[l];
            int K = B;
            if (r > 0.f) {
                const uint32_t key = uvit_hash32(seed ^ ((it * (uint32_t)nbr * depth + (uint32_t)nbr * l + br + 1u) * 0x9E3779B9u));
                const uint32_t thr = uvit_drop_threshold(r);
                K = 0;
                for (int b = 0; b < B; ++b) K += uvit_hash32((uint32_t)b ^ key) >= thr ? 1 : 0;
            }
            out[nbr * l + br] = K;
        }
}
static std::vector<float> dp_rates_linspace(int depth, float rate) {
    std::vector<float> rates(depth);
    for (int i = 0; i < depth; ++i) rates[i] = depth > 1 ? (float)((double)rate * i / (depth - 1)) : 0.f;
    return rates;
}
extern "C" int uvit_drop_path_kept_counts(int depth, float drop_path_rate, int draws_per_block, int B, uint32_t seed, uint32_t it,
                                          int32_t* out) {
    if (depth < 1 || depth > UVIT_MAX_DEPTH || (draws_per_block != 2 && draws_per_block != 4) || B < 1 || !out) return UVIT_ERR_ARG;
    const std::vector<float> rates = dp_rates_linspace(depth, drop_path_rate);
    dp_kept_counts(rates.data(), depth, draws_per_block, B, seed, it, out);
    return UVIT_OK;
}
static int dp_lists_begin(uvit_engine* e, uint32_t seed, uint32_t it, int Bc, hipStream_t s) {
    const int depth = e->cfg.depth, nbr = 2 * e->S;
    e->dpl_on = false;
    if (!e->dpl_pos) return UVIT_OK;
    dp_kept_counts(e->dp_rates_host.data(), depth, nbr, Bc, seed, it, e->dpl_K);
    bool any = false;
    for (int i = 0; i < nbr * depth; ++i) {
        const int K = e->dpl_K[i], br = i % nbr;
        any = any || (K > 0 && K < Bc && (e->S == 1 || (br & 1)));
    }
    e->dpl_on = any;
    if (!any) return UVIT_OK;
    return uvit_droppath_lists_launch(e->dp_scales, e->dpl_pos, e->dpl_bmap, e->dpl_rows, e->dpl_cnt, nbr * depth, Bc, e->N,
                                      (int)e->dpl_stride, e->dpl_K, s);
}

enum RowMode { ROWS_ALL, ROWS_LIST, ROWS_LIST2, ROWS_MASKED };
enum Pass { PASS_DENSE, PASS_TEACHER, PASS_STUDENT };
struct BranchRows {
    RowMode mode = ROWS_ALL;
    int K = 0;
    int n[2] = {0, 0};
    size_t off[2] = {0, 0};
    int rows = 0;
    int red = 0;
    DpList d[2] = {};
    const int* rowmap[2] = {nullptr, nullptr};
    const int* rowcnt[2] = {nullptr, nullptr};
};
static BranchRows branch_rows(const uvit_engine* e, int l, int branch, Pass pass, int Bc) {
    const int S = e->S;
    BranchRows r;
    r.K = Bc; r.n[0] = r.n[1] = Bc * e->N; r.off[1] = e->Mpad;
    if (pass != PASS_DENSE && branch == 1 && l == e->cfg.depth - 1 && e->compact_R > 0) {
        r.mode = ROWS_MASKED; r.n[0] = e->compact_R; r.rowmap[0] = e->rowidx; r.rowcnt[0] = e->count;
    } else if (pass == PASS_STUDENT && e->dpl_on && (S == 1 || branch == 1)) {
        DpList d[2] = {};
        bool none = false, some = false;
        for (int st = 0; st < S; ++st) {
            dp_list_get(e, l, st, branch, d[st]);
            none = none || d[st].K == 0; some = some || d[st].K < e->B;
        }
        if (!none && some) {
            r.mode = S == 1 ? ROWS_LIST : ROWS_LIST2;
            r.K = d[0].K;
            for (int st = 0; st < S; ++st) { r.d[st] = d[st]; r.n[st] = d[st].K * e->N; r.rowmap[st] = d[st].rows; r.rowcnt[st] = d[st].cnt; }
            r.off[1] = r.n[0];
        }
    }
    r.rows = (int)(r.off[S - 1] + r.n[S - 1]);
    r.red = (int)roundup(r.rows, 64);
    return r;
}

static int forward_layer(uvit_engine* e, const Weights& w, int l, const float* x_in, float* x_mid, float* x_out,
                         LayerActs& a, const float* biasP, bool dp_on, float pdrop, uint32_t seed, int Bc, Pass pass, hipStream_t s) {
    const LayerOff& o = e->lo.L[l];
    const int M = Bc * e->N, C = e->C, Hd = e->Hd, S = e->S;
    const size_t Mp = e->Mpad;
    const bool save = pass == PASS_STUDENT;
    const BranchRows at = branch_rows(e, l, 0, pass, Bc), ml = branch_rows(e, l, 1, pass, Bc);
    unsigned* const tcnt = e->tile_cnt + ((e->dual && s == e->aux) ? 16 : 0);
    LnFwd n1; n1.x = x_in; n1.w = w.f + o.n1w; n1.b = w.f + o.n1b; n1.y = a.ln1; n1.mean = a.mean1; n1.rstd = a.rstd1; n1.M = at.rows; n1.C = C;
    n1.eps = e->cfg.ln_eps;
    if (at.mode == ROWS_LIST) { n1.pos = at.d[0].pos; n1.xcopy = x_mid; n1.tokens = e->N; n1.M = M; }
    CHECK(uvit_ln_fwd_launch(n1, s));
    for (int st = 0; st < S; ++st) {
        GemmEpi q; q.out = a.qkv + at.off[st] * 3 * C; q.bias = w.f + off_qb(o, st); q.bias2 = w.f + off_vb(o, st); q.ldo = 3 * C;
        q.tile_counter = tcnt;
        CHECK(GEMM_NT(st ? EPI_QKV_ELU : EPI_QKV, a.ln1 + at.off[st] * C, w.b + o.qkvw, at.n[st], 3 * C, C, C, C, &q, s));
    }
    if (S == 1) {
        CHECK(uvit_attn_fwd_launch(a.qkv, biasP, a.attn, a.lse, at.K, e->H, e->N, e->NP, e->attn_scale, pdrop, seed, (uint32_t)l, s, at.d[0].bmap,
                                   e->head_dim));
    } else {
        CHECK(uvit_attn2_fwd_launch(a.qkv, a.qkv + Mp * 3 * C, biasP, a.attn, a.attn + Mp * C, a.lse, Bc, e->H, e->N, e->NP, 0.125f,
                                    pdrop, seed, (uint32_t)l, s));
    }
    auto prof_begin = [&](int kind, int rows) -> bool {
        if (!(e->prof_on && e->prof_used + 2 <= e->prof_ev.size())) return false;
        e->prof_kind[e->prof_used / 2] = kind; e->prof_rows[e->prof_used / 2] = rows;
        (void)hipEventRecord(e->prof_ev[e->prof_used], s);
        return true;
    };
    auto prof_end = [&](bool on) { if (on) { (void)hipEventRecord(e->prof_ev[e->prof_used + 1], s); e->prof_used += 2; } };
    for (int st = 0; st < S; ++st) {
        GemmEpi p; p.out = x_mid + st * Mp * C; p.out2 = save ? a.projout + st * Mp * C : nullptr; p.bias = w.f + off_projb(o, st);
        p.gamma = w.f + o.g1; p.resid = x_in + st * Mp * C; p.rowscale = dp_ptr(e, dp_on, l, st, 0, Bc); p.ldo = C; p.tokens = e->N;
        p.rowmap = at.rowmap[st]; p.rowcount = at.rowcnt[st];
        const bool pp = prof_begin(UVIT_PROF_PROJ, at.n[st]);
        CHECK(GEMM_NT(EPI_RESID, a.attn + at.off[st] * C, w.b + off_projw(o, st), at.n[st], C, C, C, C, &p, s));
        prof_end(pp);
    }
    LnFwd n2; n2.x = x_mid; n2.w = w.f + o.n2w; n2.b = w.f + o.n2b; n2.y = a.ln2; n2.mean = a.mean2; n2.rstd = a.rstd2; n2.M = ml.rows; n2.C = C;
    n2.eps = e->cfg.ln_eps;
    if (ml.mode == ROWS_LIST || ml.mode == ROWS_LIST2) {
        n2.tokens = e->N; n2.M = M;
        for (int st = 0; st < S; ++st) {
            n2.x = x_mid + st * Mp * C; n2.pos = ml.d[st].pos; n2.xcopy = x_out + st * Mp * C;
            n2.y = a.ln2 + ml.off[st] * C; n2.mean = a.mean2 + ml.off[st]; n2.rstd = a.rstd2 + ml.off[st];
            CHECK(uvit_ln_fwd_launch(n2, s));
        }
    } else {
        n2.rowidx = ml.rowmap[0]; n2.count = ml.rowcnt[0];
        CHECK(uvit_ln_fwd_launch(n2, s));
    }
    GemmEpi f1; f1.out = a.a; f1.out2 = save ? a.h : nullptr; f1.bias = w.f + o.fc1b; f1.ldo = Hd; f1.tile_counter = tcnt;
    const bool prof = prof_begin(save ? UVIT_PROF_FC1_S : UVIT_PROF_FC1_T, ml.rows);
    CHECK(GEMM_NT(save ? EPI_GELU_DG : EPI_GELU, a.ln2, w.b + o.fc1w, ml.rows, Hd, C, C, C, &f1, s));
    prof_end(prof);
    for (int st = 0; st < S; ++st) {
        GemmEpi f2; f2.out = x_out + st * Mp * C; f2.out2 = save ? a.mlpout + st * Mp * C : nullptr; f2.bias = w.f + o.fc2b;
        f2.gamma = w.f + o.g2; f2.resid = x_mid + st * Mp * C; f2.rowscale = dp_ptr(e, dp_on, l, st, 1, Bc); f2.ldo = C; f2.tokens = e->N;
        f2.rowmap = ml.rowmap[st]; f2.rowcount = ml.rowcnt[st];
        const bool pf2 = prof_begin(UVIT_PROF_FC2, ml.n[st]);
        CHECK(GEMM_NT(EPI_RESID, a.a + ml.off[st] * Hd, w.b + o.fc2w, ml.n[st], C, Hd, Hd, Hd, &f2, s));
        prof_end(pf2);
    }
    return UVIT_OK;
}

static int embed(uvit_engine* e, const Weights& w, const int64_t* mask, float* x0, int Bc, hipStream_t s) {
    for (int st = 0; st < e->S; ++st) {
        float* x = x0 + (size_t)st * e->Mpad * e->C;
        GemmEpi pe; pe.out = x; pe.bias = w.f + (st ? e->lo.cpeb : e->lo.peb); pe.mask = mask;
        pe.mask_token = w.f + (st ? e->lo.cmask_tok : e->lo.mask_tok); pe.ldo = e->C; pe.patches = e->P;
        CHECK(GEMM_NT(EPI_PATCH, e->cols, w.b + (st ? e->lo.cpew : e->lo.pew), Bc * e->P, e->C, e->Kpe, e->Kpe, e->Kpe, &pe, s));
        CHECK(uvit_set_cls_launch(x, w.f + (st ? e->lo.ccls : e->lo.cls), nullptr, Bc, e->N, e->C, s));
        if (e->cfg.use_abs_pos_emb) CHECK(uvit_add_pos_launch(x, w.f + e->lo.pos, Bc, e->N, e->C, s));
    }
    return UVIT_OK;
}

static int run_forward(uvit_engine* e, int which, const float* images, const int64_t* mask, int Bc, bool save_student,
                       bool dropout, uint32_t seed, uint32_t it, const uvit_step_params* hp_targets, bool cols_ready,
                       hipStream_t s) {
    if (Bc < 1 || Bc > e->B) return UVIT_ERR_SHAPE;
    const bool teacher = which == 1;
    Weights w{teacher ? e->buf.ema : e->buf.params, (const bf16*)(teacher ? e->buf.ema_bf16 : e->buf.params_bf16)};
    if (!cols_ready) CHECK(uvit_im2col_launch(images, e->cols, Bc, e->cfg.in_chans, e->cfg.img_size, e->cfg.patch_size, s));
    float* biasP = teacher ? e->biasP_t : e->biasP_s;
    CHECK(uvit_relpos_gather_launch(e->cfg.use_shared_rel_pos_bias ? w.f + e->lo.relt : nullptr, e->buf.rel_index, biasP,
                                    e->H, e->N, e->NP, s));
    const bool dp_on = dropout && !teacher && e->cfg.drop_path_rate > 0.f;
    const float pdrop = (dropout && !teacher) ? e->cfg.attn_drop_rate : 0.f;
    if (dp_on) CHECK(uvit_droppath_launch(e->dp_scales, e->dp_rates, e->cfg.depth, 2 * e->S, Bc, seed, it, s));
    if (!teacher) {
        e->dpl_on = false;
        if (dp_on && save_student && e->dpl_enable && Bc == e->B) CHECK(dp_lists_begin(e, seed, it, Bc, s));
    }
    const uint32_t aseed = uvit_hash32(seed ^ (it * 0x85EBCA6Bu + 0x1234567u));
    if (!teacher) { e->last_dropout = dropout; e->last_seed = aseed; e->last_it = it; }
    const bool use_saved = !teacher || !hp_targets;
    float* x0 = use_saved ? e->X[0] : e->tX[0];
    CHECK(embed(e, w, mask, x0, Bc, s));
    int n_t = 0;
    for (int l = 0; l < e->cfg.depth; ++l) {
        if (use_saved) {
            CHECK(forward_layer(e, w, l, e->X[l], e->XM[l], e->X[l + 1], e->acts[l], biasP, dp_on, pdrop, aseed, Bc,
                                save_student && !teacher ? PASS_STUDENT : PASS_DENSE, s));
        } else {
            float* xin = e->tX[l & 1]; float* xout = e->tX[(l + 1) & 1];
            const bool dense = hp_targets->target_batch_norm || hp_targets->target_instance_norm ||
                               hp_targets->post_target_instance_norm || !hp_targets->target_layer_norm_last;
            CHECK(forward_layer(e, w, l, xin, e->tXM, xout, e->tacts, biasP, false, 0.f, 0, Bc, dense ? PASS_DENSE : PASS_TEACHER, s));
            if (dense && Bc != e->B) return UVIT_ERR_ARG;
            for (int k = 0; k < hp_targets->n_target_layers; ++k) {
                if (hp_targets->target_layers[k] != l) continue;
                const float* sub = hp_targets->layer_results_fc ? e->tXM : nullptr;
                for (int st = dense ? 1 : 0; st < e->S; ++st)
                    CHECK(uvit_target_accum_launch(xout + (size_t)st * e->Mpad * e->C, e->rowidx, e->count, e->targets[st], n_t == 0,
                                                   Bc * e->P, e->C, 1e-5f, s, sub ? sub + (size_t)st * e->Mpad * e->C : nullptr,
                                                   hp_targets->target_layer_norm_last ? 1 : 0));
                if (dense) {
                    CHECK(uvit_gather_patch_rows_launch(xout, sub, e->dense_v, Bc, e->P, e->C, s));
                    if (hp_targets->target_batch_norm) CHECK(uvit_colnorm_launch(e->dense_v, 1, Bc * e->P, e->C, 1e-5f, s));
                    if (hp_targets->target_instance_norm) CHECK(uvit_colnorm_launch(e->dense_v, Bc, e->P, e->C, 1e-5f, s));
                    if (hp_targets->target_layer_norm_last)
                        CHECK(uvit_target_accum_launch(e->dense_v, e->idrows, e->idcount, e->dense_acc, n_t == 0, Bc * e->P, e->C, 1e-5f, s));
                    else CHECK(uvit_axpy_rows_launch(e->dense_acc, e->dense_v, n_t == 0, (size_t)Bc * e->P * e->C, s));
                }
                ++n_t;
            }
        }
    }
    if (teacher && hp_targets) {
        if (n_t != hp_targets->n_target_layers) return UVIT_ERR_ARG;
        const bool dense = hp_targets->target_batch_norm || hp_targets->target_instance_norm ||
                           hp_targets->post_target_instance_norm || !hp_targets->target_layer_norm_last;
        for (int st = dense ? 1 : 0; st < e->S; ++st)
            CHECK(uvit_target_finalize_launch(e->targets[st], e->count, n_t, hp_targets->post_target_layer_norm, Bc * e->P, e->C, 1e-5f, s));
        if (dense) {
            const bool pin = hp_targets->post_target_instance_norm != 0;
            CHECK(uvit_target_finalize_launch(e->dense_acc, e->idcount, n_t, hp_targets->post_target_layer_norm && !pin, Bc * e->P, e->C, 1e-5f, s));
            if (pin) {
                CHECK(uvit_colnorm_launch(e->dense_acc, Bc, e->P, e->C, 1e-5f, s));
                if (hp_targets->post_target_layer_norm)
                    CHECK(uvit_target_finalize_launch(e->dense_acc, e->idcount, 1, 1, Bc * e->P, e->C, 1e-5f, s));
            }
            CHECK(uvit_gather_masked_rows_launch(e->dense_acc, e->rowidx, e->count, e->targets[0], Bc * e->P, e->P, e->C, s));
        }
    }
    e->cur_B = Bc;
    return UVIT_OK;
}

extern "C" int uvit_engine_forward_features(uvit_engine* e, int which, const float* images, const int64_t* mask, int batch,
                                            int train_dropout, uint32_t seed, uint32_t it, uvit_stream stream) {
    if (!e || !images || (which != 0 && which != 1)) return UVIT_ERR_ARG;
    hipStream_t s = (hipStream_t)stream;
    if (mask) CHECK(uvit_mask_compact_launch(mask, e->rowidx, e->count, batch, e->P, s));
    return run_forward(e, which, images, mask, batch, false, train_dropout != 0, seed, it, nullptr, false, s);
}

static int head_forward(uvit_engine* e, const Weights& w, int Bc, int st, bool all_tokens, float* out, hipStream_t s, int rows = 0) {
    const int BP = rows > 0 ? rows : Bc * e->P;
    const float* x = e->X[e->cfg.depth] + (size_t)st * e->Mpad * e->C;
    const size_t lmw = st ? e->lo.clmw : e->lo.lmw, lmb = st ? e->lo.clmb : e->lo.lmb;
    LnFwd fn; fn.x = x; fn.w = w.f + e->lo.normw; fn.b = w.f + e->lo.normb; fn.C = e->C; fn.eps = e->cfg.ln_eps;
    if (all_tokens) {
        fn.y = e->acts[0].ln1; fn.mean = e->acts[0].mean1; fn.rstd = e->acts[0].rstd1; fn.M = Bc * e->N;
        CHECK(uvit_ln_fwd_launch(fn, s));
        for (int b = 0; b < Bc; ++b) {
            GemmEpi h; h.out = out + (size_t)b * e->P * e->C; h.bias = w.f + lmb; h.ldo = e->C;
            CHECK(GEMM_NT(EPI_F32, e->acts[0].ln1 + ((size_t)b * e->N + 1) * e->C, w.b + lmw, e->P, e->C, e->C,
                                      e->C, e->C, &h, s));
        }
        return UVIT_OK;
    }
    fn.rowidx = e->rowidx; fn.count = e->count; fn.y = e->normed[st]; fn.mean = e->meanF[st]; fn.rstd = e->rstdF[st]; fn.M = BP;
    CHECK(uvit_ln_fwd_launch(fn, s));
    GemmEpi h; h.out = out; h.bias = w.f + lmb; h.ldo = e->C;
    CHECK(GEMM_NT(EPI_F32, e->normed[st], w.b + lmw, BP, e->C, e->C, e->C, e->C, &h, s));
    return UVIT_OK;
}

extern "C" int uvit_engine_head(uvit_engine* e, int which, int all_tokens, float* out, int32_t* count_dev, uvit_stream stream) {
    if (!e || !out) return UVIT_ERR_ARG;
    hipStream_t s = (hipStream_t)stream;
    const bool teacher = (which & 1) != 0;
    const int st = (which >> 1) & 1;
    if (st >= e->S) return UVIT_ERR_ARG;
    Weights w{teacher ? e->buf.ema : e->buf.params, (const bf16*)(teacher ? e->buf.ema_bf16 : e->buf.params_bf16)};
    CHECK(head_forward(e, w, e->cur_B, st, all_tokens != 0, out, s));
    if (count_dev && !all_tokens) HIPCHECK(hipMemcpyAsync(count_dev, e->count, sizeof(int), hipMemcpyDeviceToDevice, s));
    return UVIT_OK;
}

extern "C" int uvit_engine_compact_rows(uvit_engine* e) { return e ? e->compact_R : 0; }

extern "C" void* uvit_engine_ws_ptr(uvit_engine* e, const char* name, int layer) {
    if (!e || !name) return nullptr;
    const std::string n(name);
    const size_t cov = (size_t)e->Mpad * e->C;
    if (n == "x" && layer >= 0 && layer <= e->cfg.depth) return e->X[layer];
    if (n == "xm" && layer >= 0 && layer < e->cfg.depth) return e->XM[layer];
    if (n == "x_cov" && e->S == 2 && layer >= 0 && layer <= e->cfg.depth) return e->X[layer] + cov;
    if (n == "xm_cov" && e->S == 2 && layer >= 0 && layer < e->cfg.depth) return e->XM[layer] + cov;
    if (n == "loss") return e->loss;
    if (n == "grad_norm") return e->gnorm;
    if (n == "targets") return e->targets[0];
    if (n == "outputs") return e->outputs[0];
    if (n == "targets_cov" && e->S == 2) return e->targets[1];
    if (n == "outputs_cov" && e->S == 2) return e->outputs[1];
    if (n == "count") return e->count;
    if (n == "dx") return e->dXa;
    return nullptr;
}

static int wgrad(uvit_engine* e, const TnProb* p, int n, hipStream_t s) {
    if (uvit_gemm_tn_group_ok(p, n, &e->tune)) return GEMM_TN_GROUP(p, n, s);
    for (int i = 0; i < n; ++i) {
        const TnProb& q = p[i];
        const int r0 = q.s1_row ? q.s1_row : q.M;
        const bf16* y1 = (const bf16*)q.Y + (size_t)r0 * q.ldy;
        if (q.bias) CHECK(uvit_colsum_launch(q.Y, q.ldy, 0, q.bias_end, r0, q.bias, NREP, e->n_nd, s));
        if (q.bias2) CHECK(uvit_colsum_launch(q.Y, q.ldy, q.bias2_begin, q.Nn - q.bias2_begin, r0, q.bias2, NREP, e->n_nd, s));
        if (q.s1_row && q.bias_s1) CHECK(uvit_colsum_launch(y1, q.ldy, 0, q.bias_end, q.M - r0, q.bias_s1, NREP, e->n_nd, s));
        if (q.s1_row && q.bias2_s1) CHECK(uvit_colsum_launch(y1, q.ldy, q.bias2_begin, q.Nn - q.bias2_begin, q.M - r0, q.bias2_s1, NREP, e->n_nd, s));
        CHECK(GEMM_TN(q.Y, q.X, q.M, q.Nn, q.Kk, q.ldy, q.ldx, q.C, q.ldc, 1, s));
    }
    return UVIT_OK;
}

extern "C" int uvit_step_begin(uvit_engine* e, const float* images, const int64_t* mask, const uvit_step_params* hp,
                               uvit_stream stream) {
    if (!e || !images || !mask || !hp || hp->n_target_layers < 1 || hp->n_target_layers > UVIT_MAX_DEPTH) return UVIT_ERR_ARG;
    hipStream_t s = (hipStream_t)stream;
    const int Bc = e->B, BP = e->BP, C = e->C;
    Layout& lo = e->lo;
    hipStream_t ts = e->dual ? e->aux : s;
    if (e->dual) { HIPCHECK(hipEventRecord(e->ev_fork, s)); HIPCHECK(hipStreamWaitEvent(ts, e->ev_fork, 0)); }
    CHECK(uvit_zero_launch(e->buf.grads, lo.n_live * sizeof(float), ts));
    CHECK(uvit_zero_launch(e->grep, (size_t)NREP * e->n_nd * sizeof(float), ts));
    CHECK(uvit_zero_launch(e->loss, 64 * sizeof(float), ts));
    CHECK(uvit_zero_launch(e->dXa, e->rows_alloc() * C * sizeof(float), ts));
    e->slab_started = false; e->bwd_next = e->cfg.depth - 1;
    e->compact_R = 0;
    if (e->S == 1 && hp->n_rows_hint > 0) {
        const int R = (int)roundup((size_t)(hp->n_rows_hint < BP ? hp->n_rows_hint : BP), 64);
        if (R >= 512 && R < e->M) {
            e->compact_R = R;
            CHECK(uvit_zero_launch(e->dXb, e->rows_alloc() * C * sizeof(float), ts));
            CHECK(uvit_zero_launch(e->dY2[(e->cfg.depth - 1) & 1], e->rows_alloc() * C * sizeof(bf16), ts));
        }
    }
    HIPCHECK(hipMemcpyAsync(e->mask_copy, mask, (size_t)BP * sizeof(int64_t), hipMemcpyDeviceToDevice, s));
    CHECK(uvit_mask_compact_launch(mask, e->rowidx, e->count, Bc, e->P, s));
    CHECK(uvit_im2col_launch(images, e->cols, Bc, e->cfg.in_chans, e->cfg.img_size, e->cfg.patch_size, s));
    if (e->dual) { HIPCHECK(hipEventRecord(e->ev_fork, s)); HIPCHECK(hipStreamWaitEvent(ts, e->ev_fork, 0)); }
    CHECK(run_forward(e, 1, images, nullptr, Bc, false, false, 0, 0, hp, true, ts));
    if (e->dual) HIPCHECK(hipEventRecord(e->ev_teacher, ts));
    CHECK(run_forward(e, 0, images, mask, Bc, true, hp->train_dropout != 0, hp->seed, hp->it, nullptr, true, s));
    Weights w{e->buf.params, (const bf16*)e->buf.params_bf16};
    const int Rh = e->compact_R > 0 ? e->compact_R : BP;
    for (int st = 0; st < e->S; ++st) CHECK(head_forward(e, w, Bc, st, false, e->outputs[st], s, e->compact_R));
    if (e->dual) HIPCHECK(hipStreamWaitEvent(s, e->ev_teacher, 0));
    const float ls = hp->loss_scale == -1.0f ? 1.0f : hp->loss_scale;
    CHECK(uvit_smooth_l1_launch(e->outputs[0], e->targets[0], e->count, hp->l1_beta, hp->l2_loss, ls, e->loss, e->dout[0], BP, C, s));
    if (hp->var_w0 > 0.f)
        CHECK(uvit_variance_loss_launch(e->outputs[0], e->count, hp->var_w0, hp->var_margin0, ls, e->var_scratch, e->loss, e->loss + 4,
                                        e->dout[0], BP, C, s));
    if (e->compact_R > 0) CHECK(uvit_rows_guard_launch(e->count, e->compact_R, e->loss, s));
    if (e->dpl_on) CHECK(uvit_droppath_lists_guard_launch(e->dpl_cnt, 2 * e->S * e->cfg.depth, e->loss, s));
    if (e->S == 2)
        CHECK(uvit_wasserstein_loss_launch(e->outputs[0], e->outputs[1], e->targets[0], e->targets[1], e->count, hp->lambda_pretraining,
                                           ls, e->wl_scratch, e->loss, e->dout[0], e->dout[1], BP, C, s));
    float* g = e->buf.grads;
    const bf16* wt = (const bf16*)e->buf.params_bf16_t;
    for (int st = 0; st < e->S; ++st) {
        const size_t lmw = st ? lo.clmw : lo.lmw, lmb = st ? lo.clmb : lo.lmb;
        TnProb hw; hw.Y = e->dout[st]; hw.X = e->normed[st]; hw.C = g + lmw; hw.M = e->compact_R > 0 ? e->compact_R : e->BPpad; hw.Nn = C; hw.Kk = C;
        hw.ldy = C; hw.ldx = C; hw.ldc = C; hw.bias = RP(lmb); hw.bias_end = C;
        CHECK(wgrad(e, &hw, 1, s));
        GemmEpi d; d.out = e->dnormed[st]; d.ldo = C;
        CHECK(GEMM_NT(EPI_BF16, e->dout[st], wt + lmw, Rh, C, C, C, C, &d, s));
        LnBwd fn; fn.dy = e->dnormed[st]; fn.x = e->X[e->cfg.depth] + (size_t)st * e->Mpad * C; fn.rowidx = e->rowidx; fn.count = e->count;
        fn.mean = e->meanF[st]; fn.rstd = e->rstdF[st]; fn.w = e->buf.params + lo.normw; fn.dx = e->dXa + (size_t)st * e->Mpad * C;
        fn.dw = RP(lo.normw); fn.db = RP(lo.normb); fn.M = Rh; fn.C = C; fn.nrep = NREP; fn.rep_stride = e->n_nd;
        CHECK(uvit_ln_bwd_launch(fn, s));
    }
    return UVIT_OK;
}

extern "C" int uvit_step_backward_layer(uvit_engine* e, int l, const uvit_step_params* hp, uvit_stream stream) {
    if (!e || l < 0 || l >= e->cfg.depth || l != e->bwd_next) return UVIT_ERR_ARG;
    (void)hp;
    e->bwd_next = l - 1;
    hipStream_t s = (hipStream_t)stream;
    const LayerOff& o = e->lo.L[l];
    LayerActs& a = e->acts[l];
    const int M = e->M, C = e->C, Hd = e->Hd, S = e->S;
    const size_t Mp = e->Mpad;
    float* g = e->buf.grads;
    const float* pf = e->buf.params;
    const bf16* wt = (const bf16*)e->buf.params_bf16_t;
    const bool dp_on = e->last_dropout && e->cfg.drop_path_rate > 0.f;
    const float pdrop = e->last_dropout ? e->cfg.attn_drop_rate : 0.f;
    const int par = l & 1;
    hipStream_t ws = e->dual ? e->aux : s;
    if (e->dual && l + 2 < e->cfg.depth) HIPCHECK(hipStreamWaitEvent(s, e->ev_wdone[l + 2], 0));
    bf16 *dY1 = e->dY1[par], *dY2 = e->dY2[par], *dH = e->dH[par], *dqkv = e->dqkv[par];
    const BranchRows at = branch_rows(e, l, 0, PASS_STUDENT, e->B), ml = branch_rows(e, l, 1, PASS_STUDENT, e->B);
    const BranchRows nx = l > 0 ? branch_rows(e, l - 1, 1, PASS_STUDENT, e->B) : BranchRows{};
    const int Mmlp = ml.mode == ROWS_ALL ? ml.rows : ml.red;
    if (S == 2 && ml.mode == ROWS_ALL && Mp > (size_t)M) CHECK(uvit_zero_launch(dY1 + (size_t)M * C, (Mp - M) * C * sizeof(bf16), s));
    TnProb wg[UVIT_TN_GROUP_MAX];
    int nwg = 0;
    {
        TnProb& f2 = wg[nwg++]; f2.Y = dY1; f2.X = a.a; f2.C = g + o.fc2w; f2.M = ml.red; f2.Nn = C; f2.Kk = Hd; f2.ldy = C; f2.ldx = Hd; f2.ldc = Hd;
        TnProb& f1 = wg[nwg++]; f1.Y = dH; f1.X = a.ln2; f1.C = g + o.fc1w; f1.M = ml.red; f1.Nn = Hd; f1.Kk = C; f1.ldy = Hd; f1.ldx = C; f1.ldc = C;
        f1.bias = RP(o.fc1b); f1.bias_end = Hd;
        for (int st = 0; st < S; ++st) {
            TnProb& pj = wg[nwg++]; pj.Y = dY2 + at.off[st] * C; pj.X = a.attn + at.off[st] * C; pj.C = g + off_projw(o, st);
            pj.M = (int)roundup(at.n[st], 64); pj.Nn = C; pj.Kk = C; pj.ldy = C; pj.ldx = C; pj.ldc = C;
        }
        TnProb& qk = wg[nwg++]; qk.Y = dqkv; qk.X = a.ln1; qk.C = g + o.qkvw; qk.M = at.red; qk.Nn = 3 * C; qk.Kk = C; qk.ldy = 3 * C; qk.ldx = C; qk.ldc = C;
        qk.bias = RP(off_qb(o, 0)); qk.bias_end = C; qk.bias2 = RP(off_vb(o, 0)); qk.bias2_begin = 2 * C;
        if (S == 2) { qk.bias_s1 = RP(off_qb(o, 1)); qk.bias2_s1 = RP(off_vb(o, 1)); qk.s1_row = (int)Mp; }
    }
    auto mlp_rider = [&](int layer, int st, const BranchRows& br, bf16* dY) {
        const LayerOff& L = e->lo.L[layer];
        LsNext n; n.y = e->acts[layer].mlpout + st * Mp * C; n.gamma = pf + L.g2; n.rowscale = dp_ptr(e, dp_on, layer, st, 1, e->B);
        n.dy = dY + br.off[st] * C; n.dgamma = RP(L.g2); n.dbias = RP(L.fc2b); n.tokens = e->N;
        return n;
    };
    if (l == e->cfg.depth - 1)
        for (int st = 0; st < S; ++st)
            CHECK(uvit_ls_bwd_launch(e->dXa + st * Mp * C, mlp_rider(l, st, ml, dY1), (ml.mode == ROWS_ALL || st + 1 < S) ? ml.n[st] : ml.red - (int)ml.off[st],
                                     C, NREP, e->n_nd, s, ml.rowmap[st], ml.rowcnt[st]));
    GemmEpi d1; d1.out = dH; d1.aux = a.h; d1.ldo = Hd;
    CHECK(GEMM_NT(EPI_MULAUX, dY1, wt + o.fc2w, Mmlp, Hd, C, C, C, &d1, s));
    GemmEpi d2; d2.out = e->dLN; d2.ldo = C;
    CHECK(GEMM_NT(EPI_BF16, dH, wt + o.fc1w, Mmlp, C, Hd, Hd, Hd, &d2, s));
    const bool ln2_samples = ml.mode != ROWS_MASKED && (ml.mode != ROWS_ALL || at.mode == ROWS_LIST);
    for (int st = 0; st < S; ++st) {
        const size_t eo = st * Mp * C;
        LnBwd b; b.dy = e->dLN + ml.off[st] * C; b.x = e->XM[l] + eo; b.mean = a.mean2 + ml.off[st]; b.rstd = a.rstd2 + ml.off[st]; b.w = pf + o.n2w;
        b.dres = e->dXa + eo; b.dx = e->dXb + eo; b.dw = RP(o.n2w); b.db = RP(o.n2b); b.C = C; b.nrep = NREP; b.rep_stride = e->n_nd;
        LsNext& n = b.next;
        n.y = a.projout + eo; n.gamma = pf + o.g1; n.rowscale = dp_ptr(e, dp_on, l, st, 0, e->B); n.dy = dY2 + at.off[st] * C;
        n.dgamma = RP(o.g1); n.dbias = RP(off_projb(o, st)); n.tokens = e->N; n.pos = at.d[st].pos;
        if (ln2_samples) { b.M = M; b.pos = ml.d[st].pos; n.cnt = at.d[st].cnt; if (at.mode == ROWS_LIST) { n.pad2 = dqkv; n.pad2_cols = 3 * C; } }
        else { b.M = ml.n[st]; b.rowidx = ml.rowmap[st]; b.count = ml.rowcnt[st]; }
        CHECK(uvit_ln_bwd_launch(b, s));
    }
    for (int st = 0; st < S; ++st) {
        GemmEpi d3; d3.out = e->dAttn + at.off[st] * C; d3.ldo = C;
        CHECK(GEMM_NT(EPI_BF16, dY2 + at.off[st] * C, wt + off_projw(o, st), at.n[st], C, C, C, C, &d3, s));
    }
    const float* biasP = e->biasP_s;
    float* slabs = e->cfg.use_shared_rel_pos_bias ? e->slabs : nullptr;
    {
        void* dsw = slabs ? e->ds_ws[par] : nullptr;
        if (S == 1) {
            if (at.mode == ROWS_LIST && ml.mode == ROWS_MASKED && at.red > at.rows)
                CHECK(uvit_zero_launch(dqkv + (size_t)at.rows * 3 * C, (size_t)(at.red - at.rows) * 3 * C * sizeof(bf16), s));
            CHECK(uvit_attn_bwd_fused_launch(a.qkv, a.attn, e->dAttn, biasP, a.lse, e->delta, dqkv, dsw, dsw != nullptr, at.K, e->H,
                                             e->N, e->NP, e->attn_scale, pdrop, e->last_seed, (uint32_t)l, s, at.d[0].bmap, e->head_dim));
        } else {
            CHECK(uvit_attn2_bwd_launch(a.qkv, a.qkv + Mp * 3 * C, a.attn, a.attn + Mp * C, e->dAttn, e->dAttn + Mp * C, biasP, a.lse,
                                        e->delta, dqkv, dqkv + Mp * 3 * C, dsw, dsw != nullptr, e->B, e->H, e->N, e->NP, 0.125f, pdrop,
                                        e->last_seed, (uint32_t)l, s));
        }
        if (dsw) {
            if (e->dual) { HIPCHECK(hipEventRecord(e->ev_ds, s)); HIPCHECK(hipStreamWaitEvent(ws, e->ev_ds, 0)); }
            if (S == 1) CHECK(uvit_attn_dbias_reduce_launch(dsw, slabs, e->slab_started ? 1 : 0, at.K, e->H, e->N, e->NP, ws));
            else CHECK(uvit_attn2_dbias_reduce_launch(dsw, slabs, e->slab_started ? 1 : 0, e->B, e->H, e->N, e->NP, ws));
        }
    }
    e->slab_started = true;
    if (e->dual) { HIPCHECK(hipEventRecord(e->ev_x, s)); HIPCHECK(hipStreamWaitEvent(ws, e->ev_x, 0)); }
    CHECK(wgrad(e, wg, nwg, ws));
    if (e->dual) HIPCHECK(hipEventRecord(e->ev_wdone[l], ws));
    GemmEpi d4; d4.out = e->dLN; d4.ldo = C;
    CHECK(GEMM_NT(EPI_BF16, dqkv, wt + o.qkvw, at.rows, C, 3 * C, 3 * C, 3 * C, &d4, s));
    if (l > 0 && e->dual && l + 1 < e->cfg.depth) HIPCHECK(hipStreamWaitEvent(s, e->ev_wdone[l + 1], 0));
    const bool ln1_samples = at.mode == ROWS_LIST || nx.mode != ROWS_ALL;
    for (int st = 0; st < (l > 0 ? S : 1); ++st) {
        const size_t ro = st * Mp, eo = ro * C;
        LnBwd b; b.dy = e->dLN + eo; b.x = e->X[l] + eo; b.mean = a.mean1 + ro; b.rstd = a.rstd1 + ro; b.w = pf + o.n1w; b.dres = e->dXb + eo;
        b.dx = e->dXa + eo; b.dw = RP(o.n1w); b.db = RP(o.n1b); b.M = l > 0 ? M : (int)e->rows_all(); b.C = C; b.nrep = NREP;
        b.rep_stride = e->n_nd;
        if (ln1_samples) { b.pos = at.d[st].pos; b.next.tokens = e->N; }
        if (l > 0) {
            b.next = mlp_rider(l - 1, st, nx, e->dY1[(l - 1) & 1]);
            b.next.pos = nx.d[st].pos;
            if (st + 1 == S && nx.d[st].cnt) { b.next.cnt = nx.d[st].cnt; b.next.pad_base = (int)nx.off[st]; }
        }
        CHECK(uvit_ln_bwd_launch(b, s));
    }
    return UVIT_OK;
}

extern "C" int uvit_step_backward_embed(uvit_engine* e, uvit_stream stream) {
    if (!e) return UVIT_ERR_ARG;
    hipStream_t s = (hipStream_t)stream;
    Layout& lo = e->lo;
    float* g = e->buf.grads;
    const int C = e->C, BP = e->BP;
    TnProb pe[2];
    for (int st = 0; st < e->S; ++st) {
        CHECK(uvit_token_bwd_launch(e->dXa + (size_t)st * e->Mpad * C, e->mask_copy, e->dpatch[st], g + (st ? lo.ccls : lo.cls),
                                    g + (st ? lo.cmask_tok : lo.mask_tok), e->B, e->P, C, s));
        TnProb& q = pe[st]; q.Y = e->dpatch[st]; q.X = e->cols; q.C = g + (st ? lo.cpew : lo.pew); q.M = (int)roundup(BP, 64); q.Nn = C; q.Kk = e->Kpe;
        q.ldy = C; q.ldx = e->Kpe; q.ldc = e->Kpe; q.bias = RP(st ? lo.cpeb : lo.peb); q.bias_end = C;
    }
    CHECK(wgrad(e, pe, e->S, s));
    if (e->cfg.use_abs_pos_emb) CHECK(uvit_pos_bwd_launch(e->dXa, g + lo.pos, e->B, e->N, C, s));
    if (e->dual) HIPCHECK(hipStreamWaitEvent(s, e->ev_wdone[0], 0));
    if (e->cfg.use_shared_rel_pos_bias && e->slab_started)
        CHECK(uvit_relpos_scatter_launch(e->slabs, 1, e->buf.rel_index, g + lo.relt, e->H, e->N, e->NP, s));
    CHECK(uvit_reduce_replicas_launch(e->grep, g + lo.n_decay, e->n_nd, NREP, e->n_nd, s));
    CHECK(uvit_poison_if_nonfinite_launch(e->loss, g + lo.n_decay, e->poisoned, s));
    return UVIT_OK;
}


extern "C" int uvit_step_wait_layer_grads(uvit_engine* e, int layer, uvit_stream stream) {
    if (!e || layer < 0 || layer >= e->cfg.depth) return UVIT_ERR_ARG;
    if (e->dual) HIPCHECK(hipStreamWaitEvent((hipStream_t)stream, e->ev_wdone[layer], 0));
    return UVIT_OK;
}

extern "C" int uvit_step_update(uvit_engine* e, const uvit_step_params* hp, uvit_stream stream) {
    if (!e || !hp) return UVIT_ERR_ARG;
    if (hp->sched_dev && (hp->sched_len < 1 || hp->sched_index < 0 || hp->sched_index >= hp->sched_len)) return UVIT_ERR_ARG;
    hipStream_t s = (hipStream_t)stream;
    Layout& lo = e->lo;
    HIPCHECK(hipMemsetAsync(e->sumsq, 0, sizeof(double), s));
    CHECK(uvit_sumsq_launch(e->buf.grads, lo.n_live, e->sumsq, s));
    const float gs = hp->grad_scale > 0.f ? hp->grad_scale : 1.0f;
    CHECK(uvit_adamw_launch(e->buf.params, e->buf.grads, e->buf.adam_m, e->buf.adam_v, e->buf.params_bf16, lo.n_live, lo.n_decay,
                            hp->lr, hp->weight_decay, hp->beta1, hp->beta2, hp->eps, hp->opt_step, e->sumsq, hp->clip_grad, gs,
                            e->gnorm, s, e->loss, (hp->do_ema || hp->sched_dev) ? e->buf.ema : nullptr, e->buf.ema_bf16, hp->ema_decay, e->poisoned,
                            hp->sched_dev, hp->sched_len, hp->sched_index));
    CHECK(uvit_transpose_batch_launch(e->tdesc, e->n_tdesc, e->n_ttiles, s));
    return UVIT_OK;
}

extern "C" int uvit_train_step(uvit_engine* e, const float* images, const int64_t* mask, const uvit_step_params* hp,
                               uvit_stream stream) {
    CHECK(uvit_step_begin(e, images, mask, hp, stream));
    for (int l = e->cfg.depth - 1; l >= 0; --l) CHECK(uvit_step_backward_layer(e, l, hp, stream));
    CHECK(uvit_step_backward_embed(e, stream));
    return uvit_step_update(e, hp, stream);
}

extern "C" int uvit_engine_read_stats_async(uvit_engine* e, float* host_out2, uvit_stream stream) {
    if (!e || !host_out2) return UVIT_ERR_ARG;
    HIPCHECK(hipMemcpyAsync(host_out2, e->loss, 8 * sizeof(float), hipMemcpyDeviceToHost, (hipStream_t)stream));
    return UVIT_OK;
}

extern "C" int uvit_engine_read_stats(uvit_engine* e, float* host_out2, uvit_stream stream) {
    if (!e || !host_out2) return UVIT_ERR_ARG;
    hipStream_t s = (hipStream_t)stream;
    HIPCHECK(hipMemcpyAsync(host_out2, e->loss, 2 * sizeof(float), hipMemcpyDeviceToHost, s));
    HIPCHECK(hipStreamSynchronize(s));
    return UVIT_OK;
}

#define S(x) ((hipStream_t)(x))
static GemmEpi epi_from_abi(const uvit_gemm_epilogue* ep) {
    GemmEpi g; g.out = ep->out; g.out2 = ep->out2; g.bias = ep->bias; g.bias2 = ep->bias2; g.gamma = ep->gamma;
    g.resid = ep->resid; g.rowscale = ep->rowscale; g.aux = ep->aux; g.mask = ep->mask; g.mask_token = ep->mask_token;
    g.ldo = ep->ldo; g.tokens = ep->tokens > 0 ? ep->tokens : 1; g.patches = ep->patches > 0 ? ep->patches : 1;
    g.row0 = ep->row0;
    return g;
}
extern "C" int uvit_op_gemm_nt_tuned(int mode, const void* A, const void* W, int M, int N, int K, int lda, int ldw,
                                     const uvit_gemm_epilogue* ep, const uvit_tuning* tune, int* tail_rows, uvit_stream st) {
    if (!A || !W || !ep || !ep->out) return UVIT_ERR_ARG;
    GemmTune tu;
    const int trc = tune_from_abi(tune, tu);
    if (trc) return trc;
    GemmEpi g = epi_from_abi(ep);
    return uvit_gemm_nt_launch(mode, A, W, M, N, K, lda, ldw, &g, S(st), &tu, tail_rows);
}
extern "C" int uvit_op_gemm_nt(int mode, const void* A, const void* W, int M, int N, int K, int lda, int ldw,
                               const uvit_gemm_epilogue* ep, uvit_stream st) {
    return uvit_op_gemm_nt_tuned(mode, A, W, M, N, K, lda, ldw, ep, nullptr, nullptr, st);
}
extern "C" int uvit_op_gemm_nt_sched(int mode, const void* A, const void* W, int M, int N, int K, int lda, int ldw,
                                     const uvit_gemm_epilogue* ep, const uvit_tuning* tune, uint32_t* tile_counters, uvit_stream st) {
    if (!ep || !A || !W || !ep->out) return UVIT_ERR_ARG;
    GemmTune tu;
    const int trc = tune_from_abi(tune, tu);
    if (trc) return trc;
    GemmEpi g = epi_from_abi(ep);
    g.tile_counter = tile_counters;
    return uvit_gemm_nt_launch(mode, A, W, M, N, K, lda, ldw, &g, S(st), &tu, nullptr);
}
extern "C" int uvit_op_wgrad_group(const uvit_wgrad_problem* problems, int count, const uvit_tuning* tune, uvit_stream st) {
    if (!problems || count < 1 || count > UVIT_TN_GROUP_MAX) return UVIT_ERR_ARG;
    GemmTune tu;
    const int trc = tune_from_abi(tune, tu);
    if (trc) return trc;
    TnProb pr[UVIT_TN_GROUP_MAX];
    for (int i = 0; i < count; ++i) {
        const uvit_wgrad_problem& q = problems[i];
        if (!q.Y_bf16 || !q.X_bf16 || !q.C) return UVIT_ERR_ARG;
        pr[i].Y = q.Y_bf16; pr[i].X = q.X_bf16; pr[i].C = q.C; pr[i].bias = q.bias; pr[i].bias2 = q.bias2;
        pr[i].bias_end = q.bias_end; pr[i].bias2_begin = q.bias2_begin;
        pr[i].M = q.M; pr[i].Nn = q.N; pr[i].Kk = q.K; pr[i].ldy = q.ldy; pr[i].ldx = q.ldx; pr[i].ldc = q.ldc;
    }
    return uvit_gemm_tn_group_launch(pr, count, S(st), &tu);
}

extern "C" int uvit_op_gemm_tn(const void* Y, const void* X, int M, int N, int K, int ldy, int ldx, float* C, int ldc,
                               const uvit_tuning* tune, uvit_stream st) {
    if (!Y || !X || !C) return UVIT_ERR_ARG;
    GemmTune tu;
    const int trc = tune_from_abi(tune, tu);
    if (trc) return trc;
    if (hipMemsetAsync(C, 0, (size_t)N * ldc * sizeof(float), S(st)) != hipSuccess) return UVIT_ERR_LAUNCH;
    return uvit_gemm_tn_launch(Y, X, M, N, K, ldy, ldx, C, ldc, 1, S(st), &tu);
}
extern "C" int uvit_op_attn_fwd(const void* qkv, const float* biasP, void* out, float* lse, int B, int H, int N, int NP,
                                float scale, float p_drop, uint32_t seed, uint32_t layer, uvit_stream st) {
    if (!qkv || !out || !lse) return UVIT_ERR_ARG;
    return uvit_attn_fwd_launch(qkv, biasP, out, lse, B, H, N, NP, scale, p_drop, seed, layer, S(st));
}
extern "C" int64_t uvit_op_attn_bwd_ws_bytes(int B, int H, int N) {
    if (B < 1 || H < 1 || N < 1 || N > 208) return UVIT_ERR_SHAPE;
    return (int64_t)uvit_attn_bwd_fused_ws_bytes(B, H, N);
}
extern "C" int uvit_op_attn_bwd(const void* qkv, const void* o_fwd, const void* d_o, const float* biasP, const float* lse,
                                      float* delta, void* dqkv, float* slab, int acc, void* ds_ws, int B, int H, int N, int NP,
                                      float scale, float p_drop, uint32_t seed, uint32_t layer, uvit_stream st) {
    if (!qkv || !o_fwd || !d_o || !lse || !delta || !dqkv || (slab && !ds_ws)) return UVIT_ERR_ARG;
    CHECK(uvit_attn_bwd_fused_launch(qkv, o_fwd, d_o, biasP, lse, delta, dqkv, ds_ws, slab != nullptr, B, H, N, NP, scale, p_drop, seed, layer, S(st)));
    if (slab) CHECK(uvit_attn_dbias_reduce_launch(ds_ws, slab, acc, B, H, N, NP, S(st)));
    return UVIT_OK;
}
extern "C" int uvit_op_attn_fwd_hd(const void* qkv, const float* biasP, void* out, float* lse, int B, int H, int N, int NP, int head_dim,
                                   float scale, float p_drop, uint32_t seed, uint32_t layer, uvit_stream st) {
    if (!qkv || !out || !lse) return UVIT_ERR_ARG;
    if (head_dim != 64 && head_dim != 80) return UVIT_ERR_SHAPE;
    return uvit_attn_fwd_launch(qkv, biasP, out, lse, B, H, N, NP, scale, p_drop, seed, layer, S(st), nullptr, head_dim);
}
extern "C" int uvit_op_attn_bwd_hd(const void* qkv, const void* o_fwd, const void* d_o, const float* biasP, const float* lse,
                                   float* delta, void* dqkv, float* slab, int acc, void* ds_ws, int B, int H, int N, int NP, int head_dim,
                                   float scale, float p_drop, uint32_t seed, uint32_t layer, uvit_stream st) {
    if (!qkv || !o_fwd || !d_o || !lse || !delta || !dqkv || (slab && !ds_ws)) return UVIT_ERR_ARG;
    if (head_dim != 64 && head_dim != 80) return UVIT_ERR_SHAPE;
    CHECK(uvit_attn_bwd_fused_launch(qkv, o_fwd, d_o, biasP, lse, delta, dqkv, ds_ws, slab != nullptr, B, H, N, NP, scale, p_drop, seed, layer,
                                     S(st), nullptr, head_dim));
    if (slab) CHECK(uvit_attn_dbias_reduce_launch(ds_ws, slab, acc, B, H, N, NP, S(st)));
    return UVIT_OK;
}
extern "C" int uvit_op_attn2_fwd(const void* qkv_m, const void* qkv_c, const float* biasP, void* out_m, void* out_c, float* lse, int B,
                                 int H, int N, int NP, float scale, float p_drop, uint32_t seed, uint32_t layer, uvit_stream st) {
    if (!qkv_m || !qkv_c || !out_m || !out_c || !lse) return UVIT_ERR_ARG;
    return uvit_attn2_fwd_launch(qkv_m, qkv_c, biasP, out_m, out_c, lse, B, H, N, NP, scale, p_drop, seed, layer, S(st));
}
extern "C" int64_t uvit_op_attn2_bwd_ws_bytes(int B, int H, int N) {
    if (B <= 0 || H <= 0 || N <= 0) return UVIT_ERR_SHAPE;
    return (int64_t)uvit_attn2_bwd_ws_bytes(B, H, N);
}
extern "C" int uvit_op_attn2_bwd(const void* qkv_m, const void* qkv_c, const void* o_m, const void* o_c, const void* d_m, const void* d_c,
                                 const float* biasP, const float* lse, float* delta, void* dqkv_m, void* dqkv_c, float* slab, int acc,
                                 void* ds_ws, int B, int H, int N, int NP, float scale, float p_drop, uint32_t seed, uint32_t layer,
                                 uvit_stream st) {
    if (!qkv_m || !qkv_c || !o_m || !o_c || !d_m || !d_c || !lse || !delta || !dqkv_m || !dqkv_c || (slab && !ds_ws)) return UVIT_ERR_ARG;
    CHECK(uvit_attn2_bwd_launch(qkv_m, qkv_c, o_m, o_c, d_m, d_c, biasP, lse, delta, dqkv_m, dqkv_c, ds_ws, slab != nullptr, B, H, N, NP,
                                scale, p_drop, seed, layer, S(st)));
    if (slab) CHECK(uvit_attn2_dbias_reduce_launch(ds_ws, slab, acc, B, H, N, NP, S(st)));
    return UVIT_OK;
}
extern "C" int uvit_op_relpos_gather(const float* t, const int32_t* idx, float* biasP, int H, int N, int NP, uvit_stream st) {
    return uvit_relpos_gather_launch(t, idx, biasP, H, N, NP, S(st));
}
extern "C" int uvit_op_relpos_scatter(const float* slab, int nslab, const int32_t* idx, float* dt, int H, int N, int NP, uvit_stream st) {
    return uvit_relpos_scatter_launch(slab, nslab, idx, dt, H, N, NP, S(st));
}
extern "C" int uvit_op_ln_fwd(const float* x, const float* w, const float* b, void* y, float* mean, float* rstd, int M, int C,
                              float eps, uvit_stream st) {
    LnFwd p; p.x = x; p.w = w; p.b = b; p.y = (bf16*)y; p.mean = mean; p.rstd = rstd; p.M = M; p.C = C; p.eps = eps;
    return uvit_ln_fwd_launch(p, S(st));
}
extern "C" int uvit_op_ln_bwd(const void* dy, const float* x, const float* mean, const float* rstd, const float* w,
                              const float* dres, float* dx, float* dw, float* db, int M, int C, uvit_stream st) {
    LnBwd p; p.dy = (const bf16*)dy; p.x = x; p.mean = mean; p.rstd = rstd; p.w = w; p.dres = dres; p.dx = dx; p.dw = dw; p.db = db; p.M = M; p.C = C;
    return uvit_ln_bwd_launch(p, S(st));
}
extern "C" int uvit_op_ema(float* ema, const float* p, void* eb, int64_t n, float d, uvit_stream st) {
    return uvit_ema_launch(ema, p, eb, (size_t)n, d, S(st));
}
extern "C" int uvit_op_sumsq(const float* g, int64_t n, double* out, uvit_stream st) { return uvit_sumsq_launch(g, (size_t)n, out, S(st)); }
extern "C" int uvit_op_adamw(float* p, const float* g, float* m, float* v, void* pb, int64_t n, int64_t nd, float lr, float wd,
                             float b1, float b2, float eps, int step, const double* sumsq, float max_norm, float gs,
                             float* gn, uvit_stream st) {
    return uvit_adamw_launch(p, g, m, v, pb, (size_t)n, (size_t)nd, lr, wd, b1, b2, eps, step, sumsq, max_norm, gs, gn, S(st));
}
extern "C" int uvit_op_smooth_l1(const float* out, const float* target, const int32_t* count, float beta, int l2, float ls,
                                 float* loss, void* dout, int Mmax, int C, uvit_stream st) {
    return uvit_smooth_l1_launch(out, target, count, beta, l2, ls, loss, dout, Mmax, C, S(st));
}
extern "C" int uvit_op_wasserstein_loss(const float* om, const float* oc, const float* tm, const float* tc, const int32_t* count, float lam,
                                        float ls, float* scratch, float* loss, void* dm, void* dc, int Mmax, int C, uvit_stream st) {
    if (!om || !oc || !tm || !tc || !count || !scratch || !loss || !dm || !dc || Mmax < 1 || C < 1) return UVIT_ERR_ARG;
    return uvit_wasserstein_loss_launch(om, oc, tm, tc, count, lam, ls, scratch, loss, dm, dc, Mmax, C, S(st));
}
extern "C" int uvit_op_variance_loss(const float* out, const int32_t* count, float w, float margin, float ls, float* scratch, float* loss,
                                     float* std_out, void* dout, int Mmax, int C, uvit_stream st) {
    if (!out || !count || !scratch || !loss || !dout) return UVIT_ERR_ARG;
    return uvit_variance_loss_launch(out, count, w, margin, ls, scratch, loss, std_out, dout, Mmax, C, S(st));
}
extern "C" int uvit_op_target_accum(const float* x, const int32_t* rowidx, const int32_t* count, float* acc, int first, int Mmax,
                                    int C, float eps, uvit_stream st) {
    return uvit_target_accum_launch(x, rowidx, count, acc, first, Mmax, C, eps, S(st));
}
extern "C" int uvit_op_target_finalize(float* acc, const int32_t* count, int nl, int post_ln, int Mmax, int C, float eps, uvit_stream st) {
    return uvit_target_finalize_launch(acc, count, nl, post_ln, Mmax, C, eps, S(st));
}
extern "C" int uvit_op_mask_compact(const int64_t* mask, int32_t* rowidx, int32_t* count, int B, int P, uvit_stream st) {
    return uvit_mask_compact_launch(mask, rowidx, count, B, P, S(st));
}
extern "C" int uvit_op_synth_batch(float* images, int64_t* mask, int B, int chans, int img_size, int patches, int n_mask, uint32_t seed,
                                   uint32_t it, uvit_stream st) {
    if (!images && !mask) return UVIT_ERR_ARG;
    return uvit_synth_batch_launch(images, mask, B, chans, img_size, patches, n_mask, seed, it, S(st));
}
extern "C" int uvit_op_im2col(const float* img, void* cols, int B, int Cin, int S_, int p, uvit_stream st) {
    return uvit_im2col_launch(img, cols, B, Cin, S_, p, S(st));
}
extern "C" int uvit_op_droppath(float* sc, const float* rates, int depth, int B, uint32_t seed, uint32_t step, uvit_stream st) {
    return uvit_droppath_launch(sc, rates, depth, 2, B, seed, step, S(st));
}
extern "C" int uvit_op_cast_bf16(const float* src, void* dst, int64_t n, uvit_stream st) { return uvit_cast_bf16_launch(src, dst, (size_t)n, S(st)); }
```

### uncertainty-vit_amd/csrc/norm.hip

```cpp
#include "common.h"
#include "uvit_internal.h"
#include "rowwise.h"

#define LN_WAVES 4

enum LnWalk { WALK_ROWS, WALK_SAMPLES };

template <int NV, LnWalk WALK>
__global__ __launch_bounds__(LN_WAVES * 64)
void ln_fwd_kernel(const float* __restrict__ x, const int* __restrict__ rowidx, const int* __restrict__ count,
                   const int* __restrict__ pos, const float* __restrict__ w, const float* __restrict__ b, bf16* __restrict__ y,
                   float* __restrict__ mean_o, float* __restrict__ rstd_o, float* __restrict__ xcopy, int M, int C, float eps, int tokens) {
    const int lane = threadIdx.x & 63;
    const int row = blockIdx.x * LN_WAVES + (threadIdx.x >> 6);
    if (row >= M) return;
    const int nv = C >> 2;
    int src = row;
    size_t dst = row;
    if constexpr (WALK == WALK_ROWS) {
        if (row >= (count ? *count : M)) { store_zero_row<NV>(y + (size_t)row * C, nv, lane); return; }
        if (rowidx) src = rowidx[row];
    }
    RowVec<NV> r;
    load_row(r, x + (size_t)src * C, C, lane);
    if constexpr (WALK == WALK_SAMPLES) {
        const int smp = row / tokens, slot = pos[smp];
        if (slot < 0) {
#pragma unroll
            for (int k = 0; k < NV; ++k) if (lane + 64 * k < nv) ((float4*)(xcopy + (size_t)row * C))[lane + 64 * k] = r.v[k];
            return;
        }
        dst = (size_t)slot * tokens + (row - smp * tokens);
    }
    float mean, rstd;
    row_stats(r, C, lane, eps, mean, rstd);
    if (lane == 0 && (WALK == WALK_SAMPLES || mean_o)) { mean_o[dst] = mean; rstd_o[dst] = rstd; }
    normalize_store(r, mean, rstd, w, b, y + dst * C, nv, lane);
}

#define LNB_WAVES 8

template <int NV, bool LS>
struct LnbRow {
    float4 x[NV], dres[NV];
    bf16x4 dy[NV], y[LS ? NV : 1];
    float mean, rstd, dp;
    int xr;
    int ar;
    int yr;
};

template <int NV, LnWalk WALK, bool LS>
__device__ __forceinline__ void lnb_load(LnbRow<NV, LS>& r, int row, const bf16* dy, const float* x, const int* map,
                                         const float* mean_i, const float* rstd_i, const float* dres, const LsNext& ls,
                                         int C, int nv, int lane) {
    const int tokens = ls.tokens;
    r.dp = 1.0f;
    if constexpr (WALK == WALK_ROWS) {
        const int xr = map ? map[row] : row;
        r.xr = xr; r.ar = row; r.yr = xr;
        r.mean = mean_i[row]; r.rstd = rstd_i[row];
        if constexpr (LS) {
            if (ls.rowscale) r.dp = ls.rowscale[xr / tokens];
            if (ls.pos) { const int smp = xr / tokens, sl = ls.pos[smp]; r.yr = sl < 0 ? -1 : sl * tokens + (xr - smp * tokens); }
        }
    } else {
        const int smp = row / tokens, t = row - smp * tokens;
        const int sa = map ? map[smp] : smp, sb = LS ? (ls.pos ? ls.pos[smp] : smp) : -1;
        r.xr = row;
        r.ar = sa < 0 ? -1 : sa * tokens + t;
        r.yr = sb < 0 ? -1 : sb * tokens + t;
        r.mean = 0.f; r.rstd = 0.f;
        if (r.ar >= 0) { r.mean = mean_i[r.ar]; r.rstd = rstd_i[r.ar]; }
        if (r.yr >= 0 && ls.rowscale) r.dp = ls.rowscale[smp];
    }
#pragma unroll
    for (int k = 0; k < NV; ++k) {
        const int i = lane + 64 * k;
        if (i < nv) {
            if (WALK == WALK_ROWS || r.ar >= 0) {
                r.x[k] = ((const float4*)(x + (size_t)r.xr * C))[i];
                r.dy[k] = ((const bf16x4*)(dy + (size_t)r.ar * C))[i];
            }
            r.dres[k] = WALK == WALK_SAMPLES || dres ? ((const float4*)(dres + (size_t)r.xr * C))[i] : make_float4(0.f, 0.f, 0.f, 0.f);
            if constexpr (LS) if (WALK == WALK_ROWS || r.yr >= 0) r.y[k] = ((const bf16x4*)(ls.y + (size_t)r.xr * C))[i];
        }
    }
}

template <int NV>
__device__ __forceinline__ void lnb_pad_fill(const LsNext& ls, int C, int nv, int lane, int wave) {
    const int n = *ls.cnt, npad = ((ls.pad_base + n + 63) & ~63) - ls.pad_base;
    for (int r = n + wave; r < npad; r += LNB_WAVES) {
        store_zero_row<NV>(ls.dy + (size_t)r * C, nv, lane);
        if (ls.pad2) for (int c = lane * 4; c < ls.pad2_cols; c += 256) *(bf16x4*)(ls.pad2 + (size_t)r * ls.pad2_cols + c) = bf16x4_zero();
    }
}

template <int NV, LnWalk WALK, bool LS>
__global__ __launch_bounds__(LNB_WAVES * 64)
void ln_bwd_kernel(const bf16* __restrict__ dy, const float* __restrict__ x, const int* __restrict__ map ,
                   const int* __restrict__ count, const float* __restrict__ mean_i, const float* __restrict__ rstd_i,
                   const float* __restrict__ w, const float* __restrict__ dres, float* __restrict__ dx,
                   float* __restrict__ dw, float* __restrict__ db, int M, int C, int nrep, size_t rep_stride, LsNext ls,
                   int rows_per_block) {
    __shared__ float red[LNB_WAVES][64 * 4];
    const int lane = threadIdx.x & 63, wave = threadIdx.x >> 6;
    const int nv = C >> 2;
    int n_valid = M;
    if constexpr (WALK == WALK_ROWS) { if (count) n_valid = min(*count, M); }
    if constexpr (WALK == WALK_SAMPLES && LS) { if (ls.cnt && blockIdx.x == gridDim.x - 1) lnb_pad_fill<NV>(ls, C, nv, lane, wave); }
    float4 ww[NV], gm[LS ? NV : 1];
    RowVec<NV> aw, ab;
    RowVec<LS ? NV : 1> ag, ay;
#pragma unroll
    for (int k = 0; k < NV; ++k) {
        aw.v[k] = make_float4(0.f, 0.f, 0.f, 0.f); ab.v[k] = aw.v[k];
        ww[k] = lane + 64 * k < nv ? ((const float4*)w)[lane + 64 * k] : aw.v[k];
    }
#pragma unroll
    for (int k = 0; k < (LS ? NV : 1); ++k) {
        ag.v[k] = make_float4(0.f, 0.f, 0.f, 0.f); ay.v[k] = ag.v[k]; gm[k] = ag.v[k];
        if constexpr (LS) { if (lane + 64 * k < nv) gm[k] = ((const float4*)ls.gamma)[lane + 64 * k]; }
    }
    const int row_end = min((int)(blockIdx.x + 1) * rows_per_block, n_valid);
    int row = blockIdx.x * rows_per_block + wave;
    LnbRow<NV, LS> cur, nxt;
    if (row < row_end) lnb_load<NV, WALK, LS>(cur, row, dy, x, map, mean_i, rstd_i, dres, ls, C, nv, lane);
    for (; row < row_end; row += LNB_WAVES) {
        const bool more = row + LNB_WAVES < row_end;
        if (more) lnb_load<NV, WALK, LS>(nxt, row + LNB_WAVES, dy, x, map, mean_i, rstd_i, dres, ls, C, nv, lane);
        const bool own = WALK == WALK_ROWS || cur.ar >= 0;
        const float mean = cur.mean, rstd = cur.rstd;
        float4 g[NV], h[NV];
        float s1 = 0.f, s2 = 0.f;
        if (own) {
#pragma unroll
            for (int k = 0; k < NV; ++k) {
                if (lane + 64 * k < nv) {
                    const float d0 = bf2f(cur.dy[k][0]), d1 = bf2f(cur.dy[k][1]), d2 = bf2f(cur.dy[k][2]), d3 = bf2f(cur.dy[k][3]);
                    h[k] = normalize4(cur.x[k], mean, rstd);
                    aw.v[k].x += d0 * h[k].x; aw.v[k].y += d1 * h[k].y; aw.v[k].z += d2 * h[k].z; aw.v[k].w += d3 * h[k].w;
                    ab.v[k].x += d0; ab.v[k].y += d1; ab.v[k].z += d2; ab.v[k].w += d3;
                    g[k] = make_float4(d0 * ww[k].x, d1 * ww[k].y, d2 * ww[k].z, d3 * ww[k].w);
                    s1 += g[k].x + g[k].y + g[k].z + g[k].w;
                    s2 += g[k].x * h[k].x + g[k].y * h[k].y + g[k].z * h[k].z + g[k].w * h[k].w;
                } else {
                    g[k] = make_float4(0.f, 0.f, 0.f, 0.f); h[k] = g[k];
                }
            }
            s1 = wave_sum(s1) / C;
            s2 = wave_sum(s2) / C;
        }
#pragma unroll
        for (int k = 0; k < NV; ++k) {
            const int i = lane + 64 * k;
            if (i < nv) {
                float4 o = cur.dres[k];
                if (own) o = make_float4(o.x + rstd * (g[k].x - s1 - h[k].x * s2), o.y + rstd * (g[k].y - s1 - h[k].y * s2),
                                         o.z + rstd * (g[k].z - s1 - h[k].z * s2), o.w + rstd * (g[k].w - s1 - h[k].w * s2));
                ((float4*)(dx + (size_t)cur.xr * C))[i] = o;
                if constexpr (LS) if (cur.yr >= 0)
                    ls_apply(o, cur.dp, cur.y[k], gm[k], (bf16x4*)(ls.dy + (size_t)cur.yr * C) + i, ag.v[k], ay.v[k]);
            }
        }
        if (more) cur = nxt;
    }
    const size_t rep = (size_t)(blockIdx.x % nrep) * rep_stride;
    auto fold = [&](const float4& part, float* dst, int k) {
        __syncthreads();
        ((float4*)red[wave])[lane] = part;
        __syncthreads();
        if (lane < 32) {
            const int col = wave * 32 + lane;
            float sum = 0.f;
#pragma unroll
            for (int q = 0; q < LNB_WAVES; ++q) sum += red[q][col];
            const int c = 256 * k + col;
            if (c < C) atomicAdd(dst + rep + c, sum);
        }
    };
#pragma unroll
    for (int k = 0; k < NV; ++k) {
        if (64 * k < nv) {
            fold(aw.v[k], dw, k);
            fold(ab.v[k], db, k);
            if constexpr (LS) { fold(ag.v[k], ls.dgamma, k); fold(ay.v[k], ls.dbias, k); }
        }
    }
}

template <int NV>
__global__ __launch_bounds__(LN_WAVES * 64)
void target_accum_kernel(const float* __restrict__ x, const float* __restrict__ sub, const int* __restrict__ rowidx,
                         const int* __restrict__ count, float* __restrict__ acc, int first, int Mmax, int C, float eps, int ln) {
    const int lane = threadIdx.x & 63;
    const int row = blockIdx.x * LN_WAVES + (threadIdx.x >> 6);
    if (row >= Mmax) return;
    const int nv = C >> 2;
    float4* dst = (float4*)(acc + (size_t)row * C);
    if (row >= *count) {
        if (first)
#pragma unroll
            for (int k = 0; k < NV; ++k) if (lane + 64 * k < nv) dst[lane + 64 * k] = make_float4(0.f, 0.f, 0.f, 0.f);
        return;
    }
    RowVec<NV> r;
    load_row(r, x + (size_t)rowidx[row] * C, C, lane);
    if (sub) {
        RowVec<NV> q;
        load_row(q, sub + (size_t)rowidx[row] * C, C, lane);
#pragma unroll
        for (int k = 0; k < NV; ++k) { r.v[k].x -= q.v[k].x; r.v[k].y -= q.v[k].y; r.v[k].z -= q.v[k].z; r.v[k].w -= q.v[k].w; }
    }
    float mean = 0.f, rstd = 1.f;
    if (ln) row_stats(r, C, lane, eps, mean, rstd);
    normalize_store(r, mean, rstd, (float*)dst, !first, nv, lane);
}

template <int NV>
__global__ __launch_bounds__(LN_WAVES * 64)
void target_finalize_kernel(float* __restrict__ acc, const int* __restrict__ count, float inv_layers, int post_ln,
                            int Mmax, int C, float eps) {
    const int lane = threadIdx.x & 63;
    const int row = blockIdx.x * LN_WAVES + (threadIdx.x >> 6);
    if (row >= Mmax || row >= *count) return;
    const int nv = C >> 2;
    RowVec<NV> r;
    load_row(r, acc + (size_t)row * C, C, lane);
#pragma unroll
    for (int k = 0; k < NV; ++k) { r.v[k].x *= inv_layers; r.v[k].y *= inv_layers; r.v[k].z *= inv_layers; r.v[k].w *= inv_layers; }
    float mean = 0.f, rstd = 1.f;
    if (post_ln) row_stats(r, C, lane, eps, mean, rstd);
    normalize_store(r, mean, rstd, acc + (size_t)row * C, false, nv, lane);
}

#define LNB_BLOCKS_PER_CU 1
static int lnb_rows(int M, int resident_blocks_per_cu) {
    static int ncu = 0;
    if (!ncu) {
        int dev = 0; hipDeviceProp_t prop;
        ncu = (hipGetDevice(&dev) == hipSuccess && hipGetDeviceProperties(&prop, dev) == hipSuccess && prop.multiProcessorCount > 0)
                  ? prop.multiProcessorCount : 256;
    }
    const int target = ncu * resident_blocks_per_cu;
    int rows = (M + target - 1) / target;
    rows = ((rows + LNB_WAVES - 1) / LNB_WAVES) * LNB_WAVES;
    return rows < LNB_WAVES ? LNB_WAVES : rows;
}

static int ln_shape_ok(int M, int C) { return (M > 0 && C > 0 && (C % 4) == 0 && C <= ROW_MAXV * 256) ? UVIT_OK : UVIT_ERR_SHAPE; }
static dim3 ln_grid(int M) { return dim3((M + LN_WAVES - 1) / LN_WAVES); }

int uvit_ln_fwd_launch(const LnFwd& p, hipStream_t s) {
    const bool samples = p.pos || p.xcopy;
    if (ln_shape_ok(p.M, p.C) || (samples && (p.rowidx || p.count))) return UVIT_ERR_SHAPE;
    if (samples && (p.tokens <= 0 || (p.M % p.tokens) || !p.pos || !p.xcopy || !p.mean || !p.rstd)) return UVIT_ERR_SHAPE;
    dispatch_nv(p.C, [&](auto nv) {
        constexpr int NV = decltype(nv)::value;
        hipLaunchKernelGGL((samples ? ln_fwd_kernel<NV, WALK_SAMPLES> : ln_fwd_kernel<NV, WALK_ROWS>), ln_grid(p.M), dim3(LN_WAVES * 64), 0, s,
                           p.x, p.rowidx, p.count, p.pos, p.w, p.b, p.y, p.mean, p.rstd, p.xcopy, p.M, p.C, p.eps, p.tokens);
    });
    return uvit_check_launch();
}
int uvit_ln_bwd_launch(const LnBwd& p, hipStream_t s) {
    const LsNext& n = p.next;
    const bool ls = n.dy != nullptr, samples = p.pos || n.cnt || (n.pos && !p.rowidx);
    if (ln_shape_ok(p.M, p.C) || (p.rowidx && !p.count) || (samples && (p.rowidx || p.count))) return UVIT_ERR_SHAPE;
    if ((ls || samples) && n.tokens <= 0) return UVIT_ERR_SHAPE;
    if (samples && ((p.M % n.tokens) || !p.dres)) return UVIT_ERR_SHAPE;
    if (((n.pos || n.cnt) && !ls) || n.pad_base < 0 || (n.pad2 && (!n.cnt || n.pad2_cols <= 0 || (n.pad2_cols % 4)))) return UVIT_ERR_SHAPE;
    const int rpb = lnb_rows(p.M, LNB_BLOCKS_PER_CU);
    dispatch_nv(p.C, [&](auto nv) {
        constexpr int NV = decltype(nv)::value;
        auto kernel = samples ? (ls ? ln_bwd_kernel<NV, WALK_SAMPLES, true> : ln_bwd_kernel<NV, WALK_SAMPLES, false>)
                              : (ls ? ln_bwd_kernel<NV, WALK_ROWS, true> : ln_bwd_kernel<NV, WALK_ROWS, false>);
        hipLaunchKernelGGL(kernel, dim3((p.M + rpb - 1) / rpb), dim3(LNB_WAVES * 64), 0, s, p.dy, p.x, samples ? p.pos : p.rowidx, p.count,
                           p.mean, p.rstd, p.w, p.dres, p.dx, p.dw, p.db, p.M, p.C, p.nrep > 0 ? p.nrep : 1, p.rep_stride, n, rpb);
    });
    return uvit_check_launch();
}
int uvit_target_accum_launch(const float* x, const int* rowidx, const int* count, float* acc, int first, int Mmax,
                             int C, float eps, hipStream_t s, const float* sub, int ln) {
    if (ln_shape_ok(Mmax, C)) return UVIT_ERR_SHAPE;
    dispatch_nv(C, [&](auto nv) {
        hipLaunchKernelGGL(target_accum_kernel<decltype(nv)::value>, ln_grid(Mmax), dim3(LN_WAVES * 64), 0, s, x, sub, rowidx, count, acc, first,
                           Mmax, C, eps, ln);
    });
    return uvit_check_launch();
}
int uvit_target_finalize_launch(float* acc, const int* count, int n_layers, int post_ln, int Mmax, int C, float eps,
                                hipStream_t s) {
    if (ln_shape_ok(Mmax, C) || n_layers <= 0) return UVIT_ERR_SHAPE;
    dispatch_nv(C, [&](auto nv) {
        hipLaunchKernelGGL(target_finalize_kernel<decltype(nv)::value>, ln_grid(Mmax), dim3(LN_WAVES * 64), 0, s, acc, count, 1.0f / n_layers,
                           post_ln, Mmax, C, eps);
    });
    return uvit_check_launch();
}

__global__ __launch_bounds__(256)
void reduce_replicas_kernel(const float* __restrict__ rep, float* __restrict__ out, size_t n4, int nrep, size_t stride4) {
    for (size_t i = blockIdx.x * (size_t)blockDim.x + threadIdx.x; i < n4; i += (size_t)gridDim.x * blockDim.x) {
        float4 a = ((const float4*)out)[i];
        for (int r = 0; r < nrep; ++r) {
            const float4 b = ((const float4*)rep)[(size_t)r * stride4 + i];
            a.x += b.x; a.y += b.y; a.z += b.z; a.w += b.w;
        }
        ((float4*)out)[i] = a;
    }
}
int uvit_reduce_replicas_launch(const float* rep, float* out, size_t n, int nrep, size_t stride, hipStream_t s) {
    if (n % 4 || stride % 4) return UVIT_ERR_SHAPE;
    size_t g = (n / 4 + 255) / 256;
    hipLaunchKernelGGL(reduce_replicas_kernel, dim3((unsigned)(g > 1024 ? 1024 : g)), dim3(256), 0, s, rep, out, n / 4, nrep, stride / 4);
    return uvit_check_launch();
}

__global__ __launch_bounds__(256)
void gather_patch_rows_kernel(const float* __restrict__ x, const float* __restrict__ sub, float* __restrict__ v, int B, int P, int C4) {
    const size_t total = (size_t)B * P * C4;
    for (size_t i = blockIdx.x * (size_t)blockDim.x + threadIdx.x; i < total; i += (size_t)gridDim.x * blockDim.x) {
        const size_t row = i / C4; const int c = (int)(i - row * C4);
        const int b = (int)(row / P), p_ = (int)(row - (size_t)b * P);
        const size_t src = ((size_t)b * (P + 1) + 1 + p_) * C4 + c;
        float4 a = ((const float4*)x)[src];
        if (sub) { const float4 q = ((const float4*)sub)[src]; a.x -= q.x; a.y -= q.y; a.z -= q.z; a.w -= q.w; }
        ((float4*)v)[i] = a;
    }
}

__global__ __launch_bounds__(256)
void colnorm_kernel(float* __restrict__ v, int rows, int C, float eps) {
    __shared__ double red[2][4][64];
    __shared__ float stat[2][64];
    const int ch = blockIdx.x * 64 + (threadIdx.x & 63), ph = threadIdx.x >> 6;
    float* base = v + (size_t)blockIdx.y * rows * C;
    double s1 = 0.0, s2 = 0.0;
    if (ch < C)
        for (int r = ph; r < rows; r += 4) { const double a = base[(size_t)r * C + ch]; s1 += a; s2 += a * a; }
    red[0][ph][threadIdx.x & 63] = s1; red[1][ph][threadIdx.x & 63] = s2;
    __syncthreads();
    if (ph == 0) {
        const int l = threadIdx.x;
        const double a = red[0][0][l] + red[0][1][l] + red[0][2][l] + red[0][3][l];
        const double q = red[1][0][l] + red[1][1][l] + red[1][2][l] + red[1][3][l];
        const double mean = a / rows, var = q / rows - mean * mean;
        stat[0][l] = (float)mean; stat[1][l] = (float)(1.0 / sqrt((var > 0.0 ? var : 0.0) + (double)eps));
    }
    __syncthreads();
    if (ch < C) {
        const float mean = stat[0][threadIdx.x & 63], rstd = stat[1][threadIdx.x & 63];
        for (int r = ph; r < rows; r += 4) { float* q = base + (size_t)r * C + ch; *q = (*q - mean) * rstd; }
    }
}

__global__ __launch_bounds__(256)
void axpy_rows_kernel(float* __restrict__ acc, const float* __restrict__ v, int first, size_t n4) {
    for (size_t i = blockIdx.x * (size_t)blockDim.x + threadIdx.x; i < n4; i += (size_t)gridDim.x * blockDim.x) {
        float4 a = ((const float4*)v)[i];
        if (!first) { const float4 b = ((const float4*)acc)[i]; a.x += b.x; a.y += b.y; a.z += b.z; a.w += b.w; }
        ((float4*)acc)[i] = a;
    }
}

__global__ __launch_bounds__(256)
void gather_masked_rows_kernel(const float* __restrict__ dense, const int* __restrict__ rowidx, const int* __restrict__ count,
                               float* __restrict__ out, int Mmax, int P, int C4) {
    const int n = min(*count, Mmax);
    const size_t total = (size_t)n * C4;
    for (size_t i = blockIdx.x * (size_t)blockDim.x + threadIdx.x; i < total; i += (size_t)gridDim.x * blockDim.x) {
        const size_t r = i / C4; const int c = (int)(i - r * C4);
        const int tok = rowidx[r], b = tok / (P + 1), p_ = tok - b * (P + 1) - 1;
        ((float4*)out)[i] = ((const float4*)dense)[((size_t)b * P + p_) * C4 + c];
    }
}

static unsigned dense_grid(size_t n) { size_t g = (n + 255) / 256; return (unsigned)(g < 1 ? 1 : (g > 4096 ? 4096 : g)); }

int uvit_gather_patch_rows_launch(const float* x, const float* sub, float* v, int B, int P, int C, hipStream_t s) {
    if (C % 4) return UVIT_ERR_SHAPE;
    hipLaunchKernelGGL(gather_patch_rows_kernel, dim3(dense_grid((size_t)B * P * (C / 4))), dim3(256), 0, s, x, sub, v, B, P, C / 4);
    return uvit_check_launch();
}
int uvit_colnorm_launch(float* v, int groups, int rows, int C, float eps, hipStream_t s) {
    if (groups < 1 || rows < 1) return UVIT_ERR_SHAPE;
    hipLaunchKernelGGL(colnorm_kernel, dim3((C + 63) / 64, groups), dim3(256), 0, s, v, rows, C, eps);
    return uvit_check_launch();
}
int uvit_axpy_rows_launch(float* acc, const float* v, int first, size_t n, hipStream_t s) {
    if (n % 4) return UVIT_ERR_SHAPE;
    hipLaunchKernelGGL(axpy_rows_kernel, dim3(dense_grid(n / 4)), dim3(256), 0, s, acc, v, first, n / 4);
    return uvit_check_launch();
}
int uvit_gather_masked_rows_launch(const float* dense, const int* rowidx, const int* count, float* out, int Mmax, int P, int C,
                                   hipStream_t s) {
    if (C % 4) return UVIT_ERR_SHAPE;
    hipLaunchKernelGGL(gather_masked_rows_kernel, dim3(dense_grid((size_t)Mmax * (C / 4))), dim3(256), 0, s, dense, rowidx, count, out,
                       Mmax, P, C / 4);
    return uvit_check_launch();
}
```

### uncertainty-vit_amd/csrc/rowwise.h

```cpp
#pragma once
#include <type_traits>
#include "common.h"

#define ROW_MAXV 8

template <class F>
static inline void dispatch_nv(int C, F&& f) {
    const int nv = (C + 255) / 256;
    if (nv <= 1) f(std::integral_constant<int, 1>{}); else if (nv == 2) f(std::integral_constant<int, 2>{});
    else if (nv == 3) f(std::integral_constant<int, 3>{}); else if (nv == 4) f(std::integral_constant<int, 4>{});
    else if (nv == 5) f(std::integral_constant<int, 5>{}); else f(std::integral_constant<int, ROW_MAXV>{});
}

template <int NV> struct RowVec { float4 v[NV]; };

template <int NV>
__device__ __forceinline__ void load_row(RowVec<NV>& r, const float* x, int C, int lane) {
    const int nv = C >> 2;
#pragma unroll
    for (int k = 0; k < NV; ++k) {
        const int i = lane + 64 * k;
        r.v[k] = i < nv ? ((const float4*)x)[i] : make_float4(0.f, 0.f, 0.f, 0.f);
    }
}

template <int NV>
__device__ __forceinline__ void row_stats(const RowVec<NV>& r, int C, int lane, float eps, float& mean, float& rstd) {
    const int nv = C >> 2;
    float s = 0.f;
#pragma unroll
    for (int k = 0; k < NV; ++k) s += r.v[k].x + r.v[k].y + r.v[k].z + r.v[k].w;
    mean = wave_sum(s) / C;
    float q = 0.f;
#pragma unroll
    for (int k = 0; k < NV; ++k) {
        if (lane + 64 * k < nv) {
            const float a = r.v[k].x - mean, b = r.v[k].y - mean, c = r.v[k].z - mean, d = r.v[k].w - mean;
            q += a * a + b * b + c * c + d * d;
        }
    }
    rstd = rsqrtf(wave_sum(q) / C + eps);
}

__device__ __forceinline__ float4 normalize4(const float4& v, float mean, float rstd) {
    return make_float4((v.x - mean) * rstd, (v.y - mean) * rstd, (v.z - mean) * rstd, (v.w - mean) * rstd);
}

template <int NV>
__device__ __forceinline__ void normalize_store(const RowVec<NV>& r, float mean, float rstd, const float* w, const float* b, bf16* y,
                                                int nv, int lane) {
#pragma unroll
    for (int k = 0; k < NV; ++k) {
        const int i = lane + 64 * k;
        if (i < nv) {
            const float4 h = normalize4(r.v[k], mean, rstd), ww = ((const float4*)w)[i], bb = ((const float4*)b)[i];
            ((bf16x4*)y)[i] = bf16x4{f2bf(h.x * ww.x + bb.x), f2bf(h.y * ww.y + bb.y), f2bf(h.z * ww.z + bb.z), f2bf(h.w * ww.w + bb.w)};
        }
    }
}
template <int NV>
__device__ __forceinline__ void normalize_store(const RowVec<NV>& r, float mean, float rstd, float* dst, bool accumulate, int nv, int lane) {
#pragma unroll
    for (int k = 0; k < NV; ++k) {
        const int i = lane + 64 * k;
        if (i < nv) {
            float4 o = normalize4(r.v[k], mean, rstd);
            if (accumulate) { const float4 a = ((const float4*)dst)[i]; o.x += a.x; o.y += a.y; o.z += a.z; o.w += a.w; }
            ((float4*)dst)[i] = o;
        }
    }
}

__device__ __forceinline__ bf16x4 bf16x4_zero() { return bf16x4{f2bf(0.f), f2bf(0.f), f2bf(0.f), f2bf(0.f)}; }

template <int NV>
__device__ __forceinline__ void store_zero_row(bf16* y, int nv, int lane) {
#pragma unroll
    for (int k = 0; k < NV; ++k)
        if (lane + 64 * k < nv) ((bf16x4*)y)[lane + 64 * k] = bf16x4_zero();
}

__device__ __forceinline__ void ls_apply(const float4& d, float dp, const bf16x4& y, const float4& gamma, bf16x4* dy, float4& ag, float4& ab) {
    const float e0 = d.x * dp, e1 = d.y * dp, e2 = d.z * dp, e3 = d.w * dp;
    ag.x += e0 * bf2f(y[0]); ag.y += e1 * bf2f(y[1]); ag.z += e2 * bf2f(y[2]); ag.w += e3 * bf2f(y[3]);
    const bf16x4 o = {f2bf(e0 * gamma.x), f2bf(e1 * gamma.y), f2bf(e2 * gamma.z), f2bf(e3 * gamma.w)};
    *dy = o;
    ab.x += bf2f(o[0]); ab.y += bf2f(o[1]); ab.z += bf2f(o[2]); ab.w += bf2f(o[3]);
}
```

### uncertainty-vit_amd/csrc/uvit_internal.h

```cpp
#pragma once
#include <hip/hip_runtime.h>
#include <stdint.h>
#include "common.h"

enum { EPI_BF16 = 0, EPI_QKV = 1, EPI_GELU = 2, EPI_RESID = 3, EPI_F32 = 4, EPI_PATCH = 5, EPI_DGELU = 6, EPI_QKV_ELU = 7,
       EPI_GELU_DG = 8,
       EPI_MULAUX = 9 };

struct GemmEpi {
    void* out = nullptr;
    void* out2 = nullptr;
    const float* bias = nullptr;
    const float* bias2 = nullptr;
    const float* gamma = nullptr;
    const float* resid = nullptr;
    const float* rowscale = nullptr;
    const void* aux = nullptr;
    const int64_t* mask = nullptr;
    const float* mask_token = nullptr;
    int ldo = 0;
    int tokens = 1;
    int patches = 1;
    int row0 = 0;
    int ngroup = 0;
    const int* rowmap = nullptr;
    const int* rowcount = nullptr;
    unsigned* tile_counter = nullptr;
};

struct GemmTune {
    int nt_variant = 3;
    int tn_variant = 3;
    int tn_target = 512;
    int group_chunks = 0;
    int nt_group = 0;
    int nt_persist = 1;
};
int uvit_gemm_nt_launch(int mode, const void* A, const void* W, int M, int N, int K, int lda, int ldw,
                        const GemmEpi* epi, hipStream_t s, const GemmTune* tune = nullptr, int* tail_rows_out = nullptr);
int uvit_gemm_tn_launch(const void* Y, const void* X, int M, int Nn, int Kk, int ldy, int ldx, float* C,
                        int ldc, int allow_split, hipStream_t s, const GemmTune* tune = nullptr);

#define UVIT_TN_GROUP_MAX 6
struct TnProb {
    const void* Y = nullptr;
    const void* X = nullptr;
    float* C = nullptr;
    float* bias = nullptr;
    float* bias2 = nullptr;
    int bias_end = 0, bias2_begin = 0;
    float* bias_s1 = nullptr; float* bias2_s1 = nullptr; int s1_row = 0;
    int M = 0, Nn = 0, Kk = 0, ldy = 0, ldx = 0, ldc = 0;
    int nm = 0, tiles_n = 0, tiles_k = 0, chunk_steps = 0, chunks = 0;
};
struct TnGroup { TnProb p[UVIT_TN_GROUP_MAX]; int nprob = 0; int max_chunks = 0; };
bool uvit_gemm_tn_group_ok(const TnProb* probs, int n, const GemmTune* tune = nullptr);
int uvit_gemm_tn_group_launch(const TnProb* probs, int n, hipStream_t s, const GemmTune* tune = nullptr);

int uvit_attn_fwd_launch(const void* qkv, const float* biasP, void* out, float* lse, int B, int H, int N, int NP,
                         float scale, float p_drop, uint32_t seed, uint32_t layer, hipStream_t s, const int* bmap = nullptr,
                         int head_dim = 64);
size_t uvit_attn_bwd_fused_ws_bytes(int B, int H, int N);
int uvit_attn_bwd_fused_launch(const void* qkv, const void* o_fwd, const void* d_o, const float* biasP, const float* lse,
                               float* delta, void* dqkv, void* ds_ws, int want_ds, int B, int H, int N, int NP, float scale,
                               float p_drop, uint32_t seed, uint32_t layer, hipStream_t s, const int* bmap = nullptr,
                               int head_dim = 64);
int uvit_attn_dbias_reduce_launch(const void* ds_ws, float* dbias_slab, int accumulate, int B, int H, int N, int NP, hipStream_t s);

int uvit_attn2_fwd_launch(const void* qkv_m, const void* qkv_c, const float* biasP, void* out_m, void* out_c, float* lse,
                          int B, int H, int N, int NP, float scale, float p_drop, uint32_t seed, uint32_t layer, hipStream_t s);
size_t uvit_attn2_bwd_ws_bytes(int B, int H, int N);
int uvit_attn2_bwd_launch(const void* qkv_m, const void* qkv_c, const void* o_m, const void* o_c, const void* d_m, const void* d_c,
                          const float* biasP, const float* lse, float* delta, void* dqkv_m, void* dqkv_c, void* ds_ws, int want_ds,
                          int B, int H, int N, int NP, float scale, float p_drop, uint32_t seed, uint32_t layer, hipStream_t s);
int uvit_attn2_dbias_reduce_launch(const void* ds_ws, float* dbias_slab, int accumulate, int B, int H, int N, int NP, hipStream_t s);

struct LnFwd {
    const float* x = nullptr;
    const float* w = nullptr;
    const float* b = nullptr;
    bf16* y = nullptr;
    float* mean = nullptr;
    float* rstd = nullptr;
    int M = 0, C = 0;
    float eps = 0.f;
    const int* rowidx = nullptr;
    const int* count = nullptr;
    const int* pos = nullptr;
    float* xcopy = nullptr;
    int tokens = 0;
};
int uvit_ln_fwd_launch(const LnFwd& p, hipStream_t s);

struct LsNext {
    const bf16* y = nullptr;
    const float* gamma = nullptr;
    const float* rowscale = nullptr;
    bf16* dy = nullptr;
    float* dgamma = nullptr;
    float* dbias = nullptr;
    int tokens = 0;
    const int* pos = nullptr;
    const int* cnt = nullptr;
    int pad_base = 0;
    bf16* pad2 = nullptr;
    int pad2_cols = 0;
};
struct LnBwd {
    const bf16* dy = nullptr;
    const float* x = nullptr;
    const float* mean = nullptr;
    const float* rstd = nullptr;
    const float* w = nullptr;
    const float* dres = nullptr;
    float* dx = nullptr;
    float* dw = nullptr;
    float* db = nullptr;
    int M = 0, C = 0;
    int nrep = 1;
    size_t rep_stride = 0;
    const int* rowidx = nullptr;
    const int* count = nullptr;
    const int* pos = nullptr;
    LsNext next;
};
int uvit_ln_bwd_launch(const LnBwd& p, hipStream_t s);
int uvit_reduce_replicas_launch(const float* rep, float* out, size_t n, int nrep, size_t stride, hipStream_t s);
int uvit_target_accum_launch(const float* x, const int* rowidx, const int* count, float* acc, int first, int Mmax,
                             int C, float eps, hipStream_t s, const float* sub = nullptr,
                             int ln = 1);
int uvit_variance_loss_launch(const float* out, const int* count, float w, float margin, float loss_scale, float* scratch,
                              float* loss, float* std_loss0_out, void* dout_bf16, int Mmax, int C, hipStream_t s);
int uvit_gather_patch_rows_launch(const float* x, const float* sub, float* v, int B, int P, int C, hipStream_t s);
int uvit_colnorm_launch(float* v, int groups, int rows, int C, float eps, hipStream_t s);
int uvit_axpy_rows_launch(float* acc, const float* v, int first, size_t n, hipStream_t s);
int uvit_gather_masked_rows_launch(const float* dense, const int* rowidx, const int* count, float* out, int Mmax, int P, int C,
                                   hipStream_t s);
int uvit_target_finalize_launch(float* acc, const int* count, int n_layers, int post_ln, int Mmax, int C, float eps,
                                hipStream_t s);

int uvit_im2col_launch(const float* img, void* cols_bf16, int B, int Cin, int img_size, int patch, hipStream_t s);
int uvit_mask_compact_launch(const int64_t* mask, int* rowidx, int* count, int B, int P, hipStream_t s);
int uvit_set_cls_launch(float* x, const float* cls, const float* pos, int B, int N, int C, hipStream_t s);
int uvit_relpos_gather_launch(const float* table, const int* index, float* biasP, int H, int N, int NP, hipStream_t s);
int uvit_relpos_scatter_launch(const float* slab, int nslab, const int* index, float* dtable, int H, int N, int NP,
                               hipStream_t s);
int uvit_ls_bwd_launch(const float* dx, const LsNext& ls, int M, int C, int nrep, size_t rep_stride, hipStream_t s,
                       const int* rowidx = nullptr, const int* count = nullptr);
int uvit_rows_guard_launch(const int* count, int limit, float* loss, hipStream_t s);
int uvit_colsum_launch(const void* y_bf16, int ld, int col0, int ncols, int M, float* out, int nrep, size_t rep_stride,
                       hipStream_t s);
int uvit_smooth_l1_launch(const float* out, const float* target, const int* count, float beta, int l2, float loss_scale,
                          float* loss, void* dout_bf16, int Mmax, int C, hipStream_t s);
int uvit_token_bwd_launch(const float* dx, const int64_t* mask, void* dpatch_bf16, float* dcls, float* dmask_token,
                          int B, int P, int C, hipStream_t s);
int uvit_transpose_batch_launch(const void* descs_dev, int ndesc, int max_tiles, hipStream_t s);
int uvit_droppath_launch(float* scales, const float* rates_dev, int depth, int nbr, int B, uint32_t seed, uint32_t step,
                         hipStream_t s);
int uvit_droppath_lists_launch(const float* scales, int* pos, int* bmap, int* rows, int* cnt, int nlists, int B, int tokens,
                               int rows_stride, const int* host_counts, hipStream_t s);
int uvit_droppath_lists_guard_launch(const int* cnt, int nlists, float* loss, hipStream_t s);
int uvit_add_pos_launch(float* x, const float* pos, int B, int N, int C, hipStream_t s);
int uvit_pos_bwd_launch(const float* dx, float* dpos, int B, int N, int C, hipStream_t s);
int uvit_synth_batch_launch(float* images, int64_t* mask, int B, int chans, int img_size, int patches, int n_mask, uint32_t seed,
                            uint32_t it, hipStream_t s);
int uvit_poison_if_nonfinite_launch(const float* loss, float* dst, int* sticky, hipStream_t s);
int uvit_wasserstein_loss_launch(const float* out_m, const float* out_c, const float* tgt_m, const float* tgt_c, const int* count,
                                 float lam, float loss_scale, float* scratch, float* loss, void* dout_m_bf16, void* dout_c_bf16,
                                 int Mmax, int C, hipStream_t s);

int uvit_ema_launch(float* ema, const float* p, void* ema_bf16, size_t n, float decay, hipStream_t s, const float* guard_loss = nullptr,
                    const double* guard_sumsq = nullptr);
int uvit_sumsq_launch(const float* g, size_t n, double* out, hipStream_t s);
int uvit_adamw_launch(float* p, const float* g, float* m, float* v, void* p_bf16, size_t n, size_t n_decay, float lr,
                      float wd, float b1, float b2, float eps, int step, const double* sumsq, float max_norm,
                      float grad_scale, float* gnorm_out, hipStream_t s, const float* guard_loss = nullptr,
                      float* ema = nullptr, void* ema_bf16 = nullptr, float ema_decay = 0.f,
                      int* sticky_poison = nullptr,
                      const float* sched_dev = nullptr, int sched_len = 0, int sched_idx = 0);
int uvit_zero_launch(void* dst, size_t bytes, hipStream_t s);
int uvit_cast_bf16_launch(const float* src, void* dst_bf16, size_t n, hipStream_t s);

struct TransposeDesc { const void* src; void* dst; int rows; int cols; int tile0; int pad; };
```

### uncertainty-vit_amd/native.py

```python
import ctypes as C
import os
import subprocess

import torch

_HERE = os.path.dirname(os.path.abspath(__file__))
LIB_PATH = os.path.join(_HERE, "libuvit.so")
MAX_DEPTH = 64


class UvitError(RuntimeError):
    pass


_ERR = {-1: "bad argument", -2: "unsupported shape", -3: "HIP launch/runtime error", -4: "workspace too small"}


def check(rc, what=""):
    if rc != 0:
        raise UvitError(f"libuvit: {what} failed: {_ERR.get(rc, rc)} ({rc})")


class Config(C.Structure):
    _fields_ = [(n, C.c_int32) for n in ("img_size", "patch_size", "in_chans", "embed_dim", "depth", "num_heads",
                                          "mlp_hidden", "use_shared_rel_pos_bias", "use_abs_pos_emb", "batch")] + \
               [("ln_eps", C.c_float), ("attn_drop_rate", C.c_float), ("drop_path_rate", C.c_float),
                ("bias_chunk", C.c_int32), ("two_stream", C.c_int32)]


class LayoutEntry(C.Structure):
    _fields_ = [("name", C.c_char * 96), ("offset", C.c_int64), ("numel", C.c_int64), ("ndim", C.c_int32),
                ("decay", C.c_int32), ("shape", C.c_int64 * 4)]


class Buffers(C.Structure):
    _fields_ = [(n, C.c_void_p) for n in ("params", "grads", "adam_m", "adam_v", "ema", "params_bf16",
                                           "params_bf16_t", "ema_bf16", "rel_index", "workspace")] + \
               [("workspace_bytes", C.c_int64)]


class StepParams(C.Structure):
    _fields_ = [("target_layers", C.c_int32 * MAX_DEPTH), ("n_target_layers", C.c_int32),
                ("target_layer_norm_last", C.c_int32), ("post_target_layer_norm", C.c_int32), ("l2_loss", C.c_int32),
                ("l1_beta", C.c_float), ("loss_scale", C.c_float), ("clip_grad", C.c_float), ("lr", C.c_float),
                ("weight_decay", C.c_float), ("beta1", C.c_float), ("beta2", C.c_float), ("eps", C.c_float),
                ("opt_step", C.c_int32), ("ema_decay", C.c_float), ("do_ema", C.c_int32), ("grad_scale", C.c_float),
                ("seed", C.c_uint32), ("it", C.c_uint32), ("train_dropout", C.c_int32), ("lambda_pretraining", C.c_float),
                ("sched_dev", C.c_void_p), ("sched_len", C.c_int32), ("sched_index", C.c_int32),
                ("layer_results_fc", C.c_int32), ("var_w0", C.c_float), ("var_margin0", C.c_float),
                ("target_batch_norm", C.c_int32), ("target_instance_norm", C.c_int32), ("post_target_instance_norm", C.c_int32),
                ("n_rows_hint", C.c_int32)]


class WgradProblem(C.Structure):
    _fields_ = [("Y", C.c_void_p), ("X", C.c_void_p), ("C", C.c_void_p), ("bias", C.c_void_p), ("bias2", C.c_void_p),
                ("bias_end", C.c_int32), ("bias2_begin", C.c_int32), ("M", C.c_int32), ("N", C.c_int32), ("K", C.c_int32),
                ("ldy", C.c_int32), ("ldx", C.c_int32), ("ldc", C.c_int32)]


class GemmEpilogue(C.Structure):
    _fields_ = [(n, C.c_void_p) for n in ("out", "out2", "bias", "bias2", "gamma", "resid", "rowscale", "aux", "mask",
                                           "mask_token")] + [("ldo", C.c_int32), ("tokens", C.c_int32), ("patches", C.c_int32),
                                                             ("row0", C.c_int32)]


class Tuning(C.Structure):
    _fields_ = [("nt_variant", C.c_int32), ("tn_variant", C.c_int32), ("tn_split_target", C.c_int32),
                ("wgrad_group_chunks", C.c_int32), ("nt_group", C.c_int32), ("nt_persist", C.c_int32)]

    @classmethod
    def default(cls, **over):
        t = cls()
        lib().uvit_tuning_default(C.byref(t))
        for k, v in over.items():
            setattr(t, k, v)
        return t


class AugmentDesc(C.Structure):
    _fields_ = [("offset", C.c_int64)] + \
               [(n, C.c_int32) for n in ("h", "w", "flip", "crop_x", "crop_y", "crop_w", "crop_h", "resize_w", "resize_h", "win_x",
                                          "win_y", "filter", "n_jitter")] + \
               [("jitter_op", C.c_int32 * 3), ("jitter_factor", C.c_float * 3), ("reserved", C.c_int32)]


_vp, _i, _i64, _f, _u32 = C.c_void_p, C.c_int, C.c_int64, C.c_float, C.c_uint32
_PROTOTYPES = {
    "uvit_version": (_i, []),
    "uvit_source_hash": (C.c_char_p, []),
    "uvit_layout_count": (_i, [_vp]),
    "uvit_layout_get": (_i, [_vp, _i, _vp]),
    "uvit_arena_numel": (_i64, [_vp, _vp]),
    "uvit_workspace_bytes": (_i64, [_vp]),
    "uvit_engine_create": (_vp, [_vp, _vp, _vp, _vp]),
    "uvit_engine_destroy": (None, [_vp]),
    "uvit_engine_sync_shadows": (_i, [_vp, _i, _vp]),
    "uvit_engine_forward_features": (_i, [_vp, _i, _vp, _vp, _i, _i, _u32, _u32, _vp]),
    "uvit_engine_head": (_i, [_vp, _i, _i, _vp, _vp, _vp]),
    "uvit_engine_ws_ptr": (_vp, [_vp, C.c_char_p, _i]),
    "uvit_engine_compact_rows": (_i, [_vp]),
    "uvit_step_begin": (_i, [_vp, _vp, _vp, _vp, _vp]),
    "uvit_step_backward_layer": (_i, [_vp, _i, _vp, _vp]),
    "uvit_step_backward_embed": (_i, [_vp, _vp]),
    "uvit_step_wait_layer_grads": (_i, [_vp, _i, _vp]),
    "uvit_step_update": (_i, [_vp, _vp, _vp]),
    "uvit_train_step": (_i, [_vp, _vp, _vp, _vp, _vp]),
    "uvit_engine_read_stats": (_i, [_vp, _vp, _vp]),
    "uvit_engine_read_stats_async": (_i, [_vp, _vp, _vp]),
    "uvit_tuning_default": (None, [_vp]),
    "uvit_engine_set_tuning": (_i, [_vp, _vp]),
    "uvit_op_wgrad_group": (_i, [_vp, _i, _vp, _vp]),
    "uvit_engine_set_streams": (_i, [_vp, _i]),
    "uvit_engine_set_drop_path_rows": (_i, [_vp, _i]),
    "uvit_drop_path_kept_counts": (_i, [_i, _f, _i, _i, _u32, _u32, _vp]),
    "uvit_engine_profile": (_i, [_vp, _i, _i]),
    "uvit_engine_profile_read": (_i, [_vp, _vp, _vp, _vp]),
    "uvit_engine_profile_read_kind": (_i, [_vp, _i, _vp, _vp, _vp, _vp]),
    "uvit_op_gemm_nt": (_i, [_i, _vp, _vp, _i, _i, _i, _i, _i, _vp, _vp]),
    "uvit_op_gemm_nt_tuned": (_i, [_i, _vp, _vp, _i, _i, _i, _i, _i, _vp, _vp, _vp, _vp]),
    "uvit_op_gemm_nt_sched": (_i, [_i, _vp, _vp, _i, _i, _i, _i, _i, _vp, _vp, _vp, _vp]),
    "uvit_op_gemm_tn": (_i, [_vp, _vp, _i, _i, _i, _i, _i, _vp, _i, _vp, _vp]),
    "uvit_op_wasserstein_loss": (_i, [_vp, _vp, _vp, _vp, _vp, _f, _f, _vp, _vp, _vp, _vp, _i, _i, _vp]),
    "uvit_op_attn_fwd": (_i, [_vp, _vp, _vp, _vp, _i, _i, _i, _i, _f, _f, _u32, _u32, _vp]),
    "uvit_op_attn_bwd_ws_bytes": (_i64, [_i, _i, _i]),
    "uvit_op_attn_bwd": (_i, [_vp, _vp, _vp, _vp, _vp, _vp, _vp, _vp, _i, _vp, _i, _i, _i, _i, _f, _f, _u32, _u32, _vp]),
    "uvit_op_attn_fwd_hd": (_i, [_vp, _vp, _vp, _vp, _i, _i, _i, _i, _i, _f, _f, _u32, _u32, _vp]),
    "uvit_op_attn_bwd_hd": (_i, [_vp, _vp, _vp, _vp, _vp, _vp, _vp, _vp, _i, _vp, _i, _i, _i, _i, _i, _f, _f, _u32, _u32, _vp]),
    "uvit_op_attn2_fwd": (_i, [_vp, _vp, _vp, _vp, _vp, _vp, _i, _i, _i, _i, _f, _f, _u32, _u32, _vp]),
    "uvit_op_attn2_bwd_ws_bytes": (_i64, [_i, _i, _i]),
    "uvit_op_attn2_bwd": (_i, [_vp] * 12 + [_i, _vp, _i, _i, _i, _i, _f, _f, _u32, _u32, _vp]),
    "uvit_op_relpos_gather": (_i, [_vp, _vp, _vp, _i, _i, _i, _vp]),
    "uvit_op_relpos_scatter": (_i, [_vp, _i, _vp, _vp, _i, _i, _i, _vp]),
    "uvit_op_ln_fwd": (_i, [_vp, _vp, _vp, _vp, _vp, _vp, _i, _i, _f, _vp]),
    "uvit_op_ln_bwd": (_i, [_vp, _vp, _vp, _vp, _vp, _vp, _vp, _vp, _vp, _i, _i, _vp]),
    "uvit_op_ema": (_i, [_vp, _vp, _vp, _i64, _f, _vp]),
    "uvit_op_sumsq": (_i, [_vp, _i64, _vp, _vp]),
    "uvit_op_adamw": (_i, [_vp, _vp, _vp, _vp, _vp, _i64, _i64, _f, _f, _f, _f, _f, _i, _vp, _f, _f, _vp, _vp]),
    "uvit_op_smooth_l1": (_i, [_vp, _vp, _vp, _f, _i, _f, _vp, _vp, _i, _i, _vp]),
    "uvit_op_target_accum": (_i, [_vp, _vp, _vp, _vp, _i, _i, _i, _f, _vp]),
    "uvit_op_variance_loss": (_i, [_vp, _vp, _f, _f, _f, _vp, _vp, _vp, _vp, _i, _i, _vp]),
    "uvit_op_target_finalize": (_i, [_vp, _vp, _i, _i, _i, _i, _f, _vp]),
    "uvit_op_mask_compact": (_i, [_vp, _vp, _vp, _i, _i, _vp]),
    "uvit_op_im2col": (_i, [_vp, _vp, _i, _i, _i, _i, _vp]),
    "uvit_op_synth_batch": (_i, [_vp, _vp, _i, _i, _i, _i, _i, _u32, _u32, _vp]),
    "uvit_op_droppath": (_i, [_vp, _vp, _i, _i, _u32, _u32, _vp]),
    "uvit_op_cast_bf16": (_i, [_vp, _vp, _i64, _vp]),
    "uvit_op_augment_ws_bytes": (_i64, [_vp, _i, _i]),
    "uvit_op_augment_batch": (_i, [_vp, _i64, _vp, _i, _i, _vp, _vp, _vp, _vp, _i64, _vp]),
}
SYMBOLS = list(_PROTOTYPES)

_lib = None


def source_hash():
    import hashlib
    src = os.path.join(_HERE, "csrc")
    h = hashlib.sha256()
    for f in sorted(n for n in os.listdir(src) if n.endswith((".hip", ".h"))):
        with open(os.path.join(src, f), "rb") as fh:
            h.update(fh.read())
    with open(os.path.join(_HERE, "..", "include", "uvit.h"), "rb") as fh:
        h.update(fh.read())
    return h.hexdigest()[:16]


def build(force=False):
    if os.path.exists(LIB_PATH) and not force:
        try:
            with open(LIB_PATH + ".hash") as fh:
                if fh.read().strip() == source_hash():
                    return LIB_PATH
        except OSError:
            pass
    subprocess.run(["bash", os.path.join(_HERE, "csrc", "build.sh"), LIB_PATH], check=True)
    return LIB_PATH


def lib():
    global _lib
    if _lib is not None:
        return _lib
    if not os.path.exists(LIB_PATH):
        raise UvitError(f"{LIB_PATH} is missing: run `python -c 'import __graft_entry__ as g; g.build()'` "
                        "(hipcc --offload-arch=gfx950). There is no CPU fallback.")
    alt = os.environ.get("UVIT_LIB_AB")
    L = C.CDLL(os.path.abspath(alt) if alt else LIB_PATH)
    for name, (res, args) in _PROTOTYPES.items():
        f = getattr(L, name)
        f.restype, f.argtypes = res, args
    if L.uvit_version() != 100:
        raise UvitError("libuvit version mismatch")
    built, want = L.uvit_source_hash().decode(), source_hash()
    if built != want and not alt:
        raise UvitError(f"{LIB_PATH} is stale: built from sources {built}, on disk {want}. "
                        "Run `python -c 'import __graft_entry__ as g; g.build()'`.")
    _lib = L
    return L


def augment_ws_bytes(desc, size):
    n = lib().uvit_op_augment_ws_bytes(C.c_void_p(desc.data_ptr()), desc.numel() // C.sizeof(AugmentDesc), int(size))
    if n < 0:
        check(n, "uvit_op_augment_ws_bytes")
    return n


def augment_batch(pixels, desc, size, mean, std, out, workspace, stream):
    B = desc.numel() // C.sizeof(AugmentDesc)
    if out.shape != (B, 3, size, size) or out.dtype != torch.float32 or not out.is_contiguous():
        raise UvitError(f"augment output must be a contiguous float32 ({B}, 3, {size}, {size}) tensor")
    m, sd = (C.c_float * 3)(*mean), (C.c_float * 3)(*std)
    check(lib().uvit_op_augment_batch(ptr(pixels), pixels.numel(), C.c_void_p(desc.data_ptr()), B, int(size), m, sd, ptr(out),
                                      ptr(workspace), workspace.numel(), stream), "uvit_op_augment_batch")


def ptr(t):
    return C.c_void_p(0 if t is None else t.data_ptr())


def cur_stream():
    return C.c_void_p(torch.cuda.current_stream().cuda_stream)


def f32(x):
    return C.c_float(float(x))
```

Measured before the change: 5521.

## Derive layer-scale dgamma from weight gradients instead of saving projection outputs

The layer-scale gamma gradient is now computed algebraically from the proj/fc2 weight and bias gradients (dgamma_c = (sum_k W_ck dW_ck + b_c db_c)/gamma_c) in a new per-channel kernel on the wgrad stream. This lets the forward pass stop writing the projout and mlpout activation buffers, and the backward LN/layer-scale kernels stop reading them. It saves activation memory and bandwidth in exchange for a small extra reduction over the weights. The result becomes undefined when gamma is zero, which is flagged by writing NaN into the loss, and it depends on bf16 weights matching those used in the forward pass.

```diff
diff --git a/include/uvit.h b/include/uvit.h
--- a/include/uvit.h
+++ b/include/uvit.h
@@ -164,6 +164,8 @@
                    float eps, uvit_stream stream);
 int uvit_op_ln_bwd(const void* dy_bf16, const float* x, const float* mean, const float* rstd, const float* w,
                    const float* dres, float* dx, float* dw, float* db, int M, int C, uvit_stream stream);
+int uvit_op_ls_dgamma_from_wgrad(const void* W_bf16, const float* dW, const float* b, const float* db, const float* gamma,
+                                 float* dgamma, int C, int K, float* loss, uvit_stream stream);
 int uvit_op_ema(float* ema, const float* params, void* ema_bf16, int64_t n, float decay, uvit_stream stream);
 int uvit_op_sumsq(const float* g, int64_t n, double* out, uvit_stream stream);
 int uvit_op_adamw(float* p, const float* g, float* m, float* v, void* p_bf16, int64_t n, int64_t n_decay, float lr,
diff --git a/uncertainty-vit_amd/csrc/elementwise.hip b/uncertainty-vit_amd/csrc/elementwise.hip
--- a/uncertainty-vit_amd/csrc/elementwise.hip
+++ b/uncertainty-vit_amd/csrc/elementwise.hip
@@ -108,16 +108,16 @@
 
 template <int NV>
 __global__ __launch_bounds__(256)
-void ls_bwd_kernel(const float* __restrict__ dx, const bf16* __restrict__ y, const float* __restrict__ gamma,
-                   const float* __restrict__ rowscale, bf16* __restrict__ dy, float* __restrict__ dgamma,
+void ls_bwd_kernel(const float* __restrict__ dx, const float* __restrict__ gamma,
+                   const float* __restrict__ rowscale, bf16* __restrict__ dy,
                    float* __restrict__ dbias, int M, int C, int tokens, int nrep, size_t rep_stride,
                    const int* __restrict__ rowidx, const int* __restrict__ count) {
     __shared__ float red[4][64 * 4];
-    dgamma += (size_t)(blockIdx.x % nrep) * rep_stride; dbias += (size_t)(blockIdx.x % nrep) * rep_stride;
+    dbias += (size_t)(blockIdx.x % nrep) * rep_stride;
     const int lane = threadIdx.x & 63, wave = threadIdx.x >> 6, nv = C >> 2;
-    float4 ag[NV], ab[NV];
-#pragma unroll
-    for (int k = 0; k < NV; ++k) { ag[k] = make_float4(0.f, 0.f, 0.f, 0.f); ab[k] = ag[k]; }
+    float4 ab[NV];
+#pragma unroll
+    for (int k = 0; k < NV; ++k) ab[k] = make_float4(0.f, 0.f, 0.f, 0.f);
     const int row_end = min((int)(blockIdx.x + 1) * CP_ROWS, M);
     const int n_valid = rowidx ? min(*count, M) : M;
     for (int row = blockIdx.x * CP_ROWS + wave; row < row_end; row += 4) {
@@ -130,13 +130,44 @@
             if (i < nv) {
                 const float4 d = ((const float4*)(dx + (size_t)xr * C))[i];
                 const float4 g = ((const float4*)gamma)[i];
-                const bf16x4 yy = ((const bf16x4*)(y + (size_t)xr * C))[i];
-                ls_apply(d, dp, yy, g, (bf16x4*)(dy + (size_t)row * C) + i, ag[k], ab[k]);
+                ls_apply(d, dp, g, (bf16x4*)(dy + (size_t)row * C) + i, ab[k]);
             }
         }
     }
-    block_col_atomic(ag, dgamma, nv, red);
     block_col_atomic(ab, dbias, nv, red);
+}
+
+struct LsDgArgs { LsDgVec v[LSDG_MAX_VEC]; };
+__global__ __launch_bounds__(256)
+void ls_dgamma_from_wgrad_kernel(LsDgArgs a, int nrep, size_t rep_stride, float* __restrict__ loss) {
+    __shared__ float red[4];
+    const LsDgVec& v = a.v[blockIdx.y];
+    const int c = blockIdx.x, lane = threadIdx.x & 63, wave = threadIdx.x >> 6;
+    float acc = 0.f, bdb = 0.f;
+    for (int t = 0; t < v.nterm; ++t) {
+        const LsDgTerm& q = v.t[t];
+        const bf16* w = q.W + (size_t)c * q.K;
+        const float* d = q.dW + (size_t)c * q.K;
+        for (int k = threadIdx.x * 8; k < q.K; k += 256 * 8) {
+            const bf16x8 wv = *(const bf16x8*)(w + k);
+            const float4 d0 = *(const float4*)(d + k), d1 = *(const float4*)(d + k + 4);
+            acc += bf2f(wv[0]) * d0.x + bf2f(wv[1]) * d0.y + bf2f(wv[2]) * d0.z + bf2f(wv[3]) * d0.w;
+            acc += bf2f(wv[4]) * d1.x + bf2f(wv[5]) * d1.y + bf2f(wv[6]) * d1.z + bf2f(wv[7]) * d1.w;
+        }
+        if (wave == 0) {
+            float r = 0.f;
+            for (int i = lane; i < nrep; i += 64) r += q.db[(size_t)i * rep_stride + c];
+            bdb += q.b[c] * wave_sum(r);
+        }
+    }
+    acc = wave_sum(acc);
+    if (lane == 0) red[wave] = acc;
+    __syncthreads();
+    if (threadIdx.x == 0) {
+        const float g = v.gamma[c], sum = ((red[0] + red[1]) + (red[2] + red[3])) + bdb;
+        if (g == 0.f) loss[0] = __builtin_nanf("");
+        else v.dgamma[c] += sum / g;
+    }
 }
 
 #define CS_ROWS 256
@@ -375,9 +406,24 @@
                        const int* rowidx, const int* count) {
     if (C % 4 || C > ROW_MAXV * 256 || (rowidx && !count)) return UVIT_ERR_SHAPE;
     dispatch_nv(C, [&](auto nv) {
-        hipLaunchKernelGGL(ls_bwd_kernel<decltype(nv)::value>, dim3((M + CP_ROWS - 1) / CP_ROWS), dim3(256), 0, s, dx, ls.y, ls.gamma, ls.rowscale,
-                           ls.dy, ls.dgamma, ls.dbias, M, C, ls.tokens, nrep > 0 ? nrep : 1, rep_stride, rowidx, count);
+        hipLaunchKernelGGL(ls_bwd_kernel<decltype(nv)::value>, dim3((M + CP_ROWS - 1) / CP_ROWS), dim3(256), 0, s, dx, ls.gamma, ls.rowscale,
+                           ls.dy, ls.dbias, M, C, ls.tokens, nrep > 0 ? nrep : 1, rep_stride, rowidx, count);
     });
+    return uvit_check_launch();
+}
+int uvit_ls_dgamma_from_wgrad_launch(const LsDgVec* v, int nvec, int C, int nrep, size_t rep_stride, float* loss, hipStream_t s) {
+    if (!v || nvec < 1 || nvec > LSDG_MAX_VEC || C < 1 || nrep < 1 || !loss) return UVIT_ERR_ARG;
+    LsDgArgs a;
+    for (int i = 0; i < nvec; ++i) {
+        a.v[i] = v[i];
+        if (!v[i].gamma || !v[i].dgamma || v[i].nterm < 1 || v[i].nterm > LSDG_MAX_TERM) return UVIT_ERR_ARG;
+        for (int t = 0; t < v[i].nterm; ++t) {
+            const LsDgTerm& q = v[i].t[t];
+            if (!q.W || !q.dW || !q.b || !q.db) return UVIT_ERR_ARG;
+            if (q.K < 8 || (q.K % 8) || ((uintptr_t)q.W % 16) || ((uintptr_t)q.dW % 16)) return UVIT_ERR_SHAPE;
+        }
+    }
+    hipLaunchKernelGGL(ls_dgamma_from_wgrad_kernel, dim3(C, nvec), dim3(256), 0, s, a, nrep, rep_stride, loss);
     return uvit_check_launch();
 }
 __global__ void rows_guard_kernel(const int* __restrict__ count, int limit, float* __restrict__ loss) {
diff --git a/uncertainty-vit_amd/csrc/engine.hip b/uncertainty-vit_amd/csrc/engine.hip
--- a/uncertainty-vit_amd/csrc/engine.hip
+++ b/uncertainty-vit_amd/csrc/engine.hip
@@ -108,7 +108,7 @@
 }
 
 struct LayerActs {
-    bf16 *ln1, *qkv, *attn, *projout, *ln2, *h, *a, *mlpout;
+    bf16 *ln1, *qkv, *attn, *ln2, *h, *a;
     float *mean1, *rstd1, *mean2, *rstd2, *lse;
 };
 
@@ -188,8 +188,7 @@
     const size_t Mp = e->rows_alloc(), C = e->C, Hd = e->Hd, BPp = e->BPpad;
     auto acts = [&](LayerActs& a) {
         a.ln1 = b.take<bf16>(Mp * C); a.qkv = b.take<bf16>(Mp * 3 * C); a.attn = b.take<bf16>(Mp * C);
-        a.projout = b.take<bf16>(Mp * C); a.ln2 = b.take<bf16>(Mp * C); a.h = b.take<bf16>(Mp * Hd);
-        a.a = b.take<bf16>(Mp * Hd); a.mlpout = b.take<bf16>(Mp * C);
+        a.ln2 = b.take<bf16>(Mp * C); a.h = b.take<bf16>(Mp * Hd); a.a = b.take<bf16>(Mp * Hd);
         a.mean1 = b.take<float>(Mp); a.rstd1 = b.take<float>(Mp); a.mean2 = b.take<float>(Mp); a.rstd2 = b.take<float>(Mp);
         a.lse = b.take<float>((size_t)e->B * e->H * e->N);
     };
@@ -601,7 +600,7 @@
     };
     auto prof_end = [&](bool on) { if (on) { (void)hipEventRecord(e->prof_ev[e->prof_used + 1], s); e->prof_used += 2; } };
     for (int st = 0; st < S; ++st) {
-        GemmEpi p; p.out = x_mid + st * Mp * C; p.out2 = save ? a.projout + st * Mp * C : nullptr; p.bias = w.f + off_projb(o, st);
+        GemmEpi p; p.out = x_mid + st * Mp * C; p.bias = w.f + off_projb(o, st);
         p.gamma = w.f + o.g1; p.resid = x_in + st * Mp * C; p.rowscale = dp_ptr(e, dp_on, l, st, 0, Bc); p.ldo = C; p.tokens = e->N;
         p.rowmap = at.rowmap[st]; p.rowcount = at.rowcnt[st];
         const bool pp = prof_begin(UVIT_PROF_PROJ, at.n[st]);
@@ -626,7 +625,7 @@
     CHECK(GEMM_NT(save ? EPI_GELU_DG : EPI_GELU, a.ln2, w.b + o.fc1w, ml.rows, Hd, C, C, C, &f1, s));
     prof_end(prof);
     for (int st = 0; st < S; ++st) {
-        GemmEpi f2; f2.out = x_out + st * Mp * C; f2.out2 = save ? a.mlpout + st * Mp * C : nullptr; f2.bias = w.f + o.fc2b;
+        GemmEpi f2; f2.out = x_out + st * Mp * C; f2.bias = w.f + o.fc2b;
         f2.gamma = w.f + o.g2; f2.resid = x_mid + st * Mp * C; f2.rowscale = dp_ptr(e, dp_on, l, st, 1, Bc); f2.ldo = C; f2.tokens = e->N;
         f2.rowmap = ml.rowmap[st]; f2.rowcount = ml.rowcnt[st];
         const bool pf2 = prof_begin(UVIT_PROF_FC2, ml.n[st]);
@@ -897,8 +896,8 @@
     }
     auto mlp_rider = [&](int layer, int st, const BranchRows& br, bf16* dY) {
         const LayerOff& L = e->lo.L[layer];
-        LsNext n; n.y = e->acts[layer].mlpout + st * Mp * C; n.gamma = pf + L.g2; n.rowscale = dp_ptr(e, dp_on, layer, st, 1, e->B);
-        n.dy = dY + br.off[st] * C; n.dgamma = RP(L.g2); n.dbias = RP(L.fc2b); n.tokens = e->N;
+        LsNext n; n.gamma = pf + L.g2; n.rowscale = dp_ptr(e, dp_on, layer, st, 1, e->B);
+        n.dy = dY + br.off[st] * C; n.dbias = RP(L.fc2b); n.tokens = e->N;
         return n;
     };
     if (l == e->cfg.depth - 1)
@@ -915,8 +914,8 @@
         LnBwd b; b.dy = e->dLN + ml.off[st] * C; b.x = e->XM[l] + eo; b.mean = a.mean2 + ml.off[st]; b.rstd = a.rstd2 + ml.off[st]; b.w = pf + o.n2w;
         b.dres = e->dXa + eo; b.dx = e->dXb + eo; b.dw = RP(o.n2w); b.db = RP(o.n2b); b.C = C; b.nrep = NREP; b.rep_stride = e->n_nd;
         LsNext& n = b.next;
-        n.y = a.projout + eo; n.gamma = pf + o.g1; n.rowscale = dp_ptr(e, dp_on, l, st, 0, e->B); n.dy = dY2 + at.off[st] * C;
-        n.dgamma = RP(o.g1); n.dbias = RP(off_projb(o, st)); n.tokens = e->N; n.pos = at.d[st].pos;
+        n.gamma = pf + o.g1; n.rowscale = dp_ptr(e, dp_on, l, st, 0, e->B); n.dy = dY2 + at.off[st] * C;
+        n.dbias = RP(off_projb(o, st)); n.tokens = e->N; n.pos = at.d[st].pos;
         if (ln2_samples) { b.M = M; b.pos = ml.d[st].pos; n.cnt = at.d[st].cnt; if (at.mode == ROWS_LIST) { n.pad2 = dqkv; n.pad2_cols = 3 * C; } }
         else { b.M = ml.n[st]; b.rowidx = ml.rowmap[st]; b.count = ml.rowcnt[st]; }
         CHECK(uvit_ln_bwd_launch(b, s));
@@ -948,6 +947,19 @@
     e->slab_started = true;
     if (e->dual) { HIPCHECK(hipEventRecord(e->ev_x, s)); HIPCHECK(hipStreamWaitEvent(ws, e->ev_x, 0)); }
     CHECK(wgrad(e, wg, nwg, ws));
+    {
+        LsDgVec v[2];
+        v[0].gamma = pf + o.g1; v[0].dgamma = g + o.g1; v[0].nterm = S;
+        for (int st = 0; st < S; ++st) {
+            LsDgTerm& t = v[0].t[st];
+            t.W = (const bf16*)e->buf.params_bf16 + off_projw(o, st); t.dW = g + off_projw(o, st); t.b = pf + off_projb(o, st);
+            t.db = RP(off_projb(o, st)); t.K = C;
+        }
+        v[1].gamma = pf + o.g2; v[1].dgamma = g + o.g2; v[1].nterm = 1;
+        LsDgTerm& t = v[1].t[0];
+        t.W = (const bf16*)e->buf.params_bf16 + o.fc2w; t.dW = g + o.fc2w; t.b = pf + o.fc2b; t.db = RP(o.fc2b); t.K = Hd;
+        CHECK(uvit_ls_dgamma_from_wgrad_launch(v, 2, C, NREP, e->n_nd, e->loss, ws));
+    }
     if (e->dual) HIPCHECK(hipEventRecord(e->ev_wdone[l], ws));
     GemmEpi d4; d4.out = e->dLN; d4.ldo = C;
     CHECK(GEMM_NT(EPI_BF16, dqkv, wt + o.qkvw, at.rows, C, 3 * C, 3 * C, 3 * C, &d4, s));
@@ -1161,6 +1173,12 @@
     LnBwd p; p.dy = (const bf16*)dy; p.x = x; p.mean = mean; p.rstd = rstd; p.w = w; p.dres = dres; p.dx = dx; p.dw = dw; p.db = db; p.M = M; p.C = C;
     return uvit_ln_bwd_launch(p, S(st));
 }
+extern "C" int uvit_op_ls_dgamma_from_wgrad(const void* W, const float* dW, const float* b, const float* db, const float* gamma,
+                                            float* dgamma, int C, int K, float* loss, uvit_stream st) {
+    LsDgVec v; v.nterm = 1; v.gamma = gamma; v.dgamma = dgamma;
+    v.t[0].W = (const bf16*)W; v.t[0].dW = dW; v.t[0].b = b; v.t[0].db = db; v.t[0].K = K;
+    return uvit_ls_dgamma_from_wgrad_launch(&v, 1, C, 1, 0, loss, S(st));
+}
 extern "C" int uvit_op_ema(float* ema, const float* p, void* eb, int64_t n, float d, uvit_stream st) {
     return uvit_ema_launch(ema, p, eb, (size_t)n, d, S(st));
 }
diff --git a/uncertainty-vit_amd/csrc/norm.hip b/uncertainty-vit_amd/csrc/norm.hip
--- a/uncertainty-vit_amd/csrc/norm.hip
+++ b/uncertainty-vit_amd/csrc/norm.hip
@@ -43,7 +43,7 @@
 template <int NV, bool LS>
 struct LnbRow {
     float4 x[NV], dres[NV];
-    bf16x4 dy[NV], y[LS ? NV : 1];
+    bf16x4 dy[NV];
     float mean, rstd, dp;
     int xr;
     int ar;
@@ -83,7 +83,6 @@
                 r.dy[k] = ((const bf16x4*)(dy + (size_t)r.ar * C))[i];
             }
             r.dres[k] = WALK == WALK_SAMPLES || dres ? ((const float4*)(dres + (size_t)r.xr * C))[i] : make_float4(0.f, 0.f, 0.f, 0.f);
-            if constexpr (LS) if (WALK == WALK_ROWS || r.yr >= 0) r.y[k] = ((const bf16x4*)(ls.y + (size_t)r.xr * C))[i];
         }
     }
 }
@@ -112,7 +111,7 @@
     if constexpr (WALK == WALK_SAMPLES && LS) { if (ls.cnt && blockIdx.x == gridDim.x - 1) lnb_pad_fill<NV>(ls, C, nv, lane, wave); }
     float4 ww[NV], gm[LS ? NV : 1];
     RowVec<NV> aw, ab;
-    RowVec<LS ? NV : 1> ag, ay;
+    RowVec<LS ? NV : 1> ay;
 #pragma unroll
     for (int k = 0; k < NV; ++k) {
         aw.v[k] = make_float4(0.f, 0.f, 0.f, 0.f); ab.v[k] = aw.v[k];
@@ -120,7 +119,7 @@
     }
 #pragma unroll
     for (int k = 0; k < (LS ? NV : 1); ++k) {
-        ag.v[k] = make_float4(0.f, 0.f, 0.f, 0.f); ay.v[k] = ag.v[k]; gm[k] = ag.v[k];
+        ay.v[k] = make_float4(0.f, 0.f, 0.f, 0.f); gm[k] = ay.v[k];
         if constexpr (LS) { if (lane + 64 * k < nv) gm[k] = ((const float4*)ls.gamma)[lane + 64 * k]; }
     }
     const int row_end = min((int)(blockIdx.x + 1) * rows_per_block, n_valid);
@@ -161,7 +160,7 @@
                                          o.z + rstd * (g[k].z - s1 - h[k].z * s2), o.w + rstd * (g[k].w - s1 - h[k].w * s2));
                 ((float4*)(dx + (size_t)cur.xr * C))[i] = o;
                 if constexpr (LS) if (cur.yr >= 0)
-                    ls_apply(o, cur.dp, cur.y[k], gm[k], (bf16x4*)(ls.dy + (size_t)cur.yr * C) + i, ag.v[k], ay.v[k]);
+                    ls_apply(o, cur.dp, gm[k], (bf16x4*)(ls.dy + (size_t)cur.yr * C) + i, ay.v[k]);
             }
         }
         if (more) cur = nxt;
@@ -185,7 +184,7 @@
         if (64 * k < nv) {
             fold(aw.v[k], dw, k);
             fold(ab.v[k], db, k);
-            if constexpr (LS) { fold(ag.v[k], ls.dgamma, k); fold(ay.v[k], ls.dbias, k); }
+            if constexpr (LS) fold(ay.v[k], ls.dbias, k);
         }
     }
 }
diff --git a/uncertainty-vit_amd/csrc/rowwise.h b/uncertainty-vit_amd/csrc/rowwise.h
--- a/uncertainty-vit_amd/csrc/rowwise.h
+++ b/uncertainty-vit_amd/csrc/rowwise.h
@@ -80,9 +80,8 @@
         if (lane + 64 * k < nv) ((bf16x4*)y)[lane + 64 * k] = bf16x4_zero();
 }
 
-__device__ __forceinline__ void ls_apply(const float4& d, float dp, const bf16x4& y, const float4& gamma, bf16x4* dy, float4& ag, float4& ab) {
+__device__ __forceinline__ void ls_apply(const float4& d, float dp, const float4& gamma, bf16x4* dy, float4& ab) {
     const float e0 = d.x * dp, e1 = d.y * dp, e2 = d.z * dp, e3 = d.w * dp;
-    ag.x += e0 * bf2f(y[0]); ag.y += e1 * bf2f(y[1]); ag.z += e2 * bf2f(y[2]); ag.w += e3 * bf2f(y[3]);
     const bf16x4 o = {f2bf(e0 * gamma.x), f2bf(e1 * gamma.y), f2bf(e2 * gamma.z), f2bf(e3 * gamma.w)};
     *dy = o;
     ab.x += bf2f(o[0]); ab.y += bf2f(o[1]); ab.z += bf2f(o[2]); ab.w += bf2f(o[3]);
diff --git a/uncertainty-vit_amd/csrc/uvit_internal.h b/uncertainty-vit_amd/csrc/uvit_internal.h
--- a/uncertainty-vit_amd/csrc/uvit_internal.h
+++ b/uncertainty-vit_amd/csrc/uvit_internal.h
@@ -93,11 +93,9 @@
 int uvit_ln_fwd_launch(const LnFwd& p, hipStream_t s);
 
 struct LsNext {
-    const bf16* y = nullptr;
     const float* gamma = nullptr;
     const float* rowscale = nullptr;
     bf16* dy = nullptr;
-    float* dgamma = nullptr;
     float* dbias = nullptr;
     int tokens = 0;
     const int* pos = nullptr;
@@ -147,6 +145,17 @@
                                hipStream_t s);
 int uvit_ls_bwd_launch(const float* dx, const LsNext& ls, int M, int C, int nrep, size_t rep_stride, hipStream_t s,
                        const int* rowidx = nullptr, const int* count = nullptr);
+#define LSDG_MAX_VEC 2
+#define LSDG_MAX_TERM 2
+struct LsDgTerm {
+    const bf16* W = nullptr;
+    const float* dW = nullptr;
+    const float* b = nullptr;
+    const float* db = nullptr;
+    int K = 0;
+};
+struct LsDgVec { LsDgTerm t[LSDG_MAX_TERM]; int nterm = 0; const float* gamma = nullptr; float* dgamma = nullptr; };
+int uvit_ls_dgamma_from_wgrad_launch(const LsDgVec* v, int nvec, int C, int nrep, size_t rep_stride, float* loss, hipStream_t s);
 int uvit_rows_guard_launch(const int* count, int limit, float* loss, hipStream_t s);
 int uvit_colsum_launch(const void* y_bf16, int ld, int col0, int ncols, int M, float* out, int nrep, size_t rep_stride,
                        hipStream_t s);
diff --git a/uncertainty-vit_amd/native.py b/uncertainty-vit_amd/native.py
--- a/uncertainty-vit_amd/native.py
+++ b/uncertainty-vit_amd/native.py
@@ -133,6 +133,7 @@
     "uvit_op_relpos_scatter": (_i, [_vp, _i, _vp, _vp, _i, _i, _i, _vp]),
     "uvit_op_ln_fwd": (_i, [_vp, _vp, _vp, _vp, _vp, _vp, _i, _i, _f, _vp]),
     "uvit_op_ln_bwd": (_i, [_vp, _vp, _vp, _vp, _vp, _vp, _vp, _vp, _vp, _i, _i, _vp]),
+    "uvit_op_ls_dgamma_from_wgrad": (_i, [_vp, _vp, _vp, _vp, _vp, _vp, _i, _i, _vp, _vp]),
     "uvit_op_ema": (_i, [_vp, _vp, _vp, _i64, _f, _vp]),
     "uvit_op_sumsq": (_i, [_vp, _i64, _vp, _vp]),
     "uvit_op_adamw": (_i, [_vp, _vp, _vp, _vp, _vp, _i64, _i64, _f, _f, _f, _f, _f, _i, _vp, _f, _f, _vp, _vp]),
```

New measurement: 5550, median of 6. No clear change (+0.5%).
